# DrorT/demucs

Measured on AMD Instinct MI355X. Metric: real-time factor (audio-sec/wall-sec) htdemucs 4-stem 44.1kHz stereo, 1/8 GPU, higher is better.
Workload: dtype f32

## Files before the change

### demucs_amd/_lib.py

```python
from __future__ import annotations

import ctypes as C
import os
import threading

_HERE = os.path.dirname(os.path.abspath(__file__))
LIB_PATH = os.environ.get("DEMUCS_AMD_LIB") or os.path.join(_HERE, "libdemucs_amd.so")

MI_OK = 0


class MiTensorDesc(C.Structure):
    _fields_ = [("name", C.c_char_p), ("data", C.c_void_p), ("numel", C.c_int64)]


class MiConfig(C.Structure):
    _fields_ = [("n_sources", C.c_int32), ("segment_length", C.c_int32), ("max_batch", C.c_int32),
                ("dtype", C.c_int32)]


class MiProfileRow(C.Structure):
    _fields_ = [("name", C.c_char * 48), ("launches", C.c_int64), ("ms", C.c_double), ("flops", C.c_double),
                ("bytes", C.c_double)]

# ... 16 lines not shown
        ("xh", C.c_void_p), ("xh_n", C.c_int64), ("yh", C.c_void_p), ("yh_n", C.c_int64),
        ("wtap", C.c_void_p), ("ntaps", C.c_int32), ("tap_k2", C.c_int32), ("tap_pad1", C.c_int32), ("tap_pad2", C.c_int32),
        ("tap_dil1", C.c_int32), ("tap_dil2", C.c_int32), ("yh_pq", C.c_int64),
        ("dma_rows", C.c_int32), ("dma_rows_pad", C.c_int32),
    ]


SIGNATURES = {
    "mi_model_create": (C.c_int, [C.POINTER(MiConfig), C.POINTER(MiTensorDesc), C.c_size_t, C.POINTER(C.c_void_p)]),
    "mi_model_destroy": (None, [C.c_void_p]),
    "mi_model_forward": (C.c_int, [C.c_void_p, C.c_void_p, C.c_void_p, C.c_int32, C.c_void_p]),
    "mi_model_forward_core": (C.c_int, [C.c_void_p, C.c_void_p, C.c_void_p, C.c_void_p, C.c_void_p, C.c_int32, C.c_void_p]),
    "mi_model_tap": (C.c_int, [C.c_void_p, C.c_char_p, C.c_void_p, C.c_int32, C.POINTER(C.c_int64), C.c_void_p]),
    "mi_hmodel_create": (C.c_int, [C.POINTER(MiConfig), C.POINTER(MiTensorDesc), C.c_size_t, C.POINTER(C.c_void_p)]),
    "mi_hmodel_destroy": (None, [C.c_void_p]),
    "mi_hmodel_forward": (C.c_int, [C.c_void_p, C.c_void_p, C.c_void_p, C.c_int32, C.c_int32, C.c_void_p]),
    "mi_hmodel_tap": (C.c_int, [C.c_void_p, C.c_char_p, C.c_void_p, C.c_int32, C.POINTER(C.c_int64), C.c_void_p]),
    "mi_hmodel_device_bytes": (C.c_int64, [C.c_void_p]),
    "mi_hmodel_status": (C.c_int, [C.c_void_p, C.c_void_p]),
    "mi_set_two_streams": (C.c_int, [C.c_int32]),
    "mi_set_split_bf16": (C.c_int, [C.c_int32]),
    "mi_set_istft_fused": (C.c_int, [C.c_int32]),
    "mi_set_transpose_tiles": (C.c_int, [C.c_int32]),
    "mi_profile_begin": (C.c_int, [C.c_void_p]),
    "mi_profile_end": (C.c_int, [C.c_void_p, C.POINTER(MiProfileRow), C.c_int32, C.POINTER(C.c_int32), C.c_void_p]),
    "mi_model_device_bytes": (C.c_int64, [C.c_void_p]),
    "mi_segments_gather": (C.c_int, [C.c_void_p, C.c_int64, C.c_int32, C.c_void_p, C.c_int32, C.c_int32, C.c_void_p,
                                     C.c_int64, C.c_void_p]),
    "mi_ola_accumulate": (C.c_int, [C.c_void_p, C.c_int64, C.c_int32, C.c_void_p, C.c_int32, C.c_int64, C.c_void_p, C.c_void_p,
                                    C.c_void_p, C.c_int32, C.c_int64, C.c_int64, C.c_void_p, C.c_int32, C.c_void_p]),
    "mi_ola_finish": (C.c_int, [C.c_void_p, C.c_int64, C.c_int32, C.c_int64, C.c_void_p, C.c_void_p, C.c_int32,
                                C.c_int32, C.c_void_p, C.c_void_p]),
    "mi_segments_gather_packed": (C.c_int, [C.c_void_p, C.c_int64, C.c_int32, C.c_void_p, C.c_int32, C.c_int32, C.c_void_p,
                                            C.c_int64, C.c_void_p]),
    "mi_ola_accumulate_packed": (C.c_int, [C.c_void_p, C.c_int64, C.c_int32, C.c_void_p, C.c_int32, C.c_int64, C.c_void_p, C.c_int32,
                                           C.c_void_p, C.c_int32, C.c_void_p, C.c_int64, C.c_void_p]),
    "mi_ola_finish_packed": (C.c_int, [C.c_void_p, C.c_int64, C.c_int32, C.c_void_p, C.c_int32, C.c_void_p, C.c_int32, C.c_void_p,
                                       C.c_int64, C.c_void_p]),
    "mi_stream_emit": (C.c_int, [C.c_void_p, C.c_int64, C.c_int32, C.c_int32, C.c_void_p, C.c_int32, C.c_void_p, C.c_int32,
                                 C.c_void_p, C.c_int64, C.c_void_p, C.c_int32, C.c_int32, C.c_int32, C.c_void_p, C.c_int64,
                                 C.c_void_p, C.c_int64, C.c_void_p]),
    "mi_streams_emit": (C.c_int, [C.c_void_p, C.c_int64, C.c_int32, C.c_int32, C.c_void_p, C.c_int32, C.c_int64, C.c_void_p,
                                  C.c_int32, C.c_void_p, C.c_int32, C.c_void_p, C.c_int64, C.c_void_p, C.c_int32, C.c_int32,
                                  C.c_int32, C.c_void_p, C.c_int32, C.c_void_p, C.c_int64, C.c_void_p]),
    "mi_streams_append": (C.c_int, [C.c_void_p, C.c_int64, C.c_int32, C.c_void_p, C.c_int32, C.c_int64, C.c_void_p, C.c_int32,
                                    C.c_void_p]),
    "mi_streams_convert_append": (C.c_int, [C.c_void_p, C.c_int64, C.c_int32, C.c_void_p, C.c_int32, C.c_int64, C.c_void_p, C.c_int64,
                                            C.c_void_p, C.c_int64, C.c_void_p, C.c_int32, C.c_int32, C.c_void_p]),
    "mi_streams_compact": (C.c_int, [C.c_void_p, C.c_int64, C.c_void_p, C.c_int64, C.c_void_p, C.c_int32, C.c_int64, C.c_void_p]),
    "mi_mono_stats_scratch_bytes": (C.c_int32, []),
    "mi_mono_stats": (C.c_int, [C.c_void_p, C.c_int32, C.c_int64, C.c_void_p, C.c_void_p, C.c_void_p]),
    "mi_track_affine": (C.c_int, [C.c_void_p, C.c_int64, C.c_void_p, C.c_int32, C.c_void_p]),
    "mi_prevent_clip": (C.c_int, [C.c_void_p, C.c_int64, C.c_int32, C.c_void_p, C.c_void_p, C.c_void_p]),
    "mi_two_stems": (C.c_int, [C.c_void_p, C.c_int32, C.c_int32, C.c_void_p, C.c_int32, C.c_int64, C.c_void_p, C.c_void_p]),
    "mi_stft_cac": (C.c_int, [C.c_void_p, C.c_int32, C.c_int32, C.c_void_p, C.c_void_p]),
    "mi_istft_cac": (C.c_int, [C.c_void_p, C.c_int32, C.c_int32, C.c_int32, C.c_void_p, C.c_void_p]),
    "mi_conv_forward": (C.c_int, [C.POINTER(MiConvDesc), C.c_void_p]),
    "mi_resample_frac": (C.c_int, [C.c_void_p, C.c_int32, C.c_int64, C.c_void_p, C.c_int32, C.c_int32, C.c_int32, C.c_void_p, C.c_int64,
                                   C.c_void_p]),
    "mi_conv_pack_split": (C.c_int, [C.c_void_p, C.c_int32, C.c_int32, C.c_int32, C.c_void_p, C.c_void_p]),
    "mi_conv_pack_half": (C.c_int, [C.c_void_p, C.c_int32, C.c_int32, C.c_int32, C.c_void_p, C.c_void_p]),
    "mi_f32_to_image": (C.c_int, [C.c_void_p, C.c_int32, C.c_int32, C.c_int64, C.c_int32, C.c_void_p, C.c_void_p]),
    "mi_conv_pack_tap": (C.c_int, [C.c_void_p, C.c_int32, C.c_int32, C.c_int32, C.c_int32, C.c_void_p, C.c_void_p]),
    "mi_attention": (C.c_int, [C.c_void_p, C.c_void_p, C.c_void_p, C.c_void_p, C.c_int32, C.c_int32, C.c_int32,
                               C.c_int32, C.c_int64, C.c_int64, C.c_int64, C.c_int32, C.c_void_p]),
    "mi_attention_split": (C.c_int, [C.c_void_p, C.c_void_p, C.c_void_p, C.c_void_p, C.c_int32, C.c_int32, C.c_int32,
                                     C.c_int32, C.c_int64, C.c_int64, C.c_int64, C.c_void_p]),
    "mi_attention_heads": (C.c_int, [C.c_void_p, C.c_void_p, C.c_void_p, C.c_void_p, C.c_int32, C.c_int32, C.c_int32, C.c_int32,
                                     C.c_int32, C.c_int32, C.c_int32, C.c_void_p]),
    "mi_attention_image": (C.c_int, [C.c_void_p, C.c_void_p, C.c_void_p, C.c_void_p, C.c_int64, C.c_int32, C.c_int32, C.c_int32,
                                     C.c_int32, C.c_int64, C.c_int64, C.c_int32, C.c_void_p]),
    "mi_lstm_seq": (C.c_int, [C.c_void_p, C.c_void_p, C.c_int32, C.c_int32, C.c_int32, C.c_void_p, C.c_int32, C.c_void_p]),
    "mi_gn_gelu": (C.c_int, [C.c_void_p, C.c_int32, C.c_int32, C.c_int32, C.c_int32, C.c_int32, C.c_int32, C.c_void_p, C.c_void_p,
                             C.c_void_p, C.c_void_p]),
    "mi_gram_order": (C.c_int32, [C.c_int32]),
    "mi_gn_gelu_gram": (C.c_int, [C.c_void_p, C.c_int32, C.c_int32, C.c_int32, C.c_int32, C.c_int32, C.c_int32, C.c_int32, C.c_void_p,
                                  C.c_void_p, C.c_void_p, C.c_void_p, C.c_int32, C.c_void_p]),
    "mi_dconv_gn_gelu_gram": (C.c_int, [C.c_void_p, C.c_int32, C.c_int32, C.c_int32, C.c_int32, C.c_int32, C.c_int32, C.c_int32,
                                        C.c_void_p, C.c_void_p, C.c_void_p, C.c_void_p, C.c_int32, C.c_void_p]),
    "mi_gram_finalize": (C.c_int, [C.c_void_p, C.c_int32, C.c_int32, C.c_int32, C.c_void_p, C.c_void_p, C.c_double, C.c_double,
                                   C.c_double, C.c_double, C.c_float, C.c_void_p, C.c_void_p]),
    "mi_layernorm_cf": (C.c_int, [C.c_void_p, C.c_int32, C.c_int32, C.c_int32, C.c_void_p, C.c_void_p, C.c_void_p,
                                  C.c_void_p, C.c_void_p]),
    "mi_debug_set_post_launch_hook": (None, [C.c_void_p]),
    "mi_debug_last_conv_route": (C.c_int, []),
    "mi_last_error": (C.c_char_p, []),
    "mi_version": (C.c_char_p, []),
}

_lib = None
_lock = threading.Lock()


class EngineError(RuntimeError):
    """A libdemucs_amd call returned a non-zero status (the reference convention for this path
    is "exceptions propagate", demucs/apply.py:289-293)."""


def load() -> C.CDLL:
    global _lib
    with _lock:
        if _lib is None:
            if not os.path.exists(LIB_PATH):
                raise EngineError(
                    f"{LIB_PATH} not found: build it with `python -c 'import __graft_entry__ as g; g.build()'` "
                    "(hipcc --offload-arch=gfx950).  demucs_amd has no CPU / eager fallback.")
            lib = C.CDLL(LIB_PATH)
            for name, (res, args) in SIGNATURES.items():
                fn = getattr(lib, name)
                fn.restype = res
                fn.argtypes = args
            _lib = lib
    return _lib


def check(status: int, what: str) -> None:
    if status != MI_OK:
        msg = load().mi_last_error().decode(errors="replace")
        raise EngineError(f"{what} failed ({status}): {msg}")


def current_stream_ptr() -> int:
    import torch
    return torch.cuda.current_stream().cuda_stream
```

### demucs_amd/csrc/api.hip

```cpp
#include <new>

#include "common.h"
#include "gemm_conv.h"
#include "kernels.h"
#include "hmodel.h"
#include "model.h"

namespace mi {

post_launch_hook_t g_post_launch_hook = nullptr;
int g_last_conv_route = -1;

char *last_error_buf() {
    static thread_local char buf[1024] = "";
    return buf;
}

int set_error(int code, const char *fmt, ...) {
    va_list ap;
    va_start(ap, fmt);
    vsnprintf(last_error_buf(), 1024, fmt, ap);
    va_end(ap);
    return code;
}
// ... 414 lines not shown
                       void *stream) {
    MI_REQUIRE(q_dev && k_dev && v_dev && img_dev && B > 0 && heads > 0 && Tq > 0 && Tk > 0, "mi_attention_image: bad argument");
    MI_REQUIRE(dtype == MI_DTYPE_BF16 || dtype == MI_DTYPE_F16, "mi_attention_image: dtype %d is not a half mode", dtype);
    return launch_attention(q_dev, k_dev, v_dev, nullptr, B, heads, Tq, Tk, q_batch_stride, kv_batch_stride, 0, dtype,
                            (hipStream_t)stream, img_dev, n_img);
}

int mi_gn_gelu(float *x_dev, int32_t B, int32_t C, int32_t C_alloc, int32_t D1, int32_t D2, int32_t row_mode, const float *stats_dev,
               const float *w_dev, const float *b_dev, void *stream) {
    MI_REQUIRE(x_dev && stats_dev && w_dev && b_dev && B > 0 && C > 0 && D1 > 0 && D2 > 0, "mi_gn_gelu: bad argument");
    MI_REQUIRE(C_alloc >= C, "mi_gn_gelu: C_alloc < C");
    return launch_gn_gelu(x_dev, B, C, C_alloc, D1, D2, row_mode, (const float2 *)stats_dev, w_dev, b_dev, (hipStream_t)stream);
}

int32_t mi_gram_order(int32_t h) { return gram_hp(h); }

int mi_lstm_seq(const float *gx_dev, const float *whh_host, int32_t N, int32_t H, int32_t W, float *out_dev, int32_t mode, void *stream) {
    MI_REQUIRE(gx_dev && whh_host && out_dev && N > 0 && W > 0 && (H == 192 || H == 384), "mi_lstm_seq: bad argument (H must be 192 or 384)");
    MI_REQUIRE(mode == 0 || mode == 1, "mi_lstm_seq: mode 0 (one launch per step) or 1 (persistent kernel)");
    hipStream_t st = (hipStream_t)stream;
    std::vector<float> packed((size_t)2 * 4 * H * H);
    pack_lstm_whh(whh_host, H, packed.data());
    float *wd = nullptr, *state = nullptr;
    void *scratch = nullptr;
    unsigned *flag = nullptr;
    int r = MI_OK;
    auto fail = [&](hipError_t e, const char *what) { if (e != hipSuccess && r == MI_OK) r = set_error(MI_EHIP, "mi_lstm_seq: %s: %s", what, hipGetErrorString(e)); };
    fail(hipMalloc((void **)&wd, packed.size() * sizeof(float)), "hipMalloc");
    fail(hipMalloc((void **)&state, (size_t)6 * N * H * sizeof(float)), "hipMalloc");
    fail(hipMalloc(&scratch, lstm_persist_scratch_bytes()), "hipMalloc");
    fail(hipHostMalloc((void **)&flag, 64, hipHostMallocMapped), "hipHostMalloc");
    if (r == MI_OK) {
        *flag = 0;
        fail(hipMemcpyAsync(wd, packed.data(), packed.size() * sizeof(float), hipMemcpyHostToDevice, st), "hipMemcpyAsync");
        if (r == MI_OK) r = mode ? launch_lstm_persist(gx_dev, wd, N, H, W, out_dev, scratch, flag, st) : launch_lstm_seq(gx_dev, wd, N, H, W, out_dev, state, st);
        fail(hipStreamSynchronize(st), "hipStreamSynchronize");
        if (r == MI_OK && *(volatile unsigned *)flag) r = set_error(MI_EHIP, "mi_lstm_seq: the persistent kernel timed out waiting for its hidden-state exchange");
        if (r == MI_OK && mode && getenv("MI_LSTM_DEBUG")) {
                        unsigned dbg[16] = {};
            (void)hipMemcpy(dbg, (char *)scratch + lstm_persist_ctl_offset(), sizeof(dbg), hipMemcpyDeviceToHost);
            fprintf(stderr, "[lstm] H %d N %d W %d: block 0 / wave 1 spent %.1f us gathering h in %u poll passes (%.2f us, %.2f passes per step); "
                    "%s stores\n", H, N, W, dbg[2] * 0.01, dbg[3], dbg[2] * 0.01 / std::max(1, W - 1), (double)dbg[3] / std::max(1, W - 1),
                    dbg[4] ? "same-XCD plain" : "write-through");
            fprintf(stderr, "[lstm]   shader cycles per step: gather %.0f, issue + products %.0f, LDS write + barrier %.0f, gate stage %.0f; whole step %.0f\n",
                    (double)dbg[8] / W, (double)dbg[9] / W, (double)dbg[10] / W, (double)dbg[11] / W, (double)dbg[12] / W);
        }
    }
    if (wd) (void)hipFree(wd);
    if (state) (void)hipFree(state);
    if (scratch) (void)hipFree(scratch);
    if (flag) (void)hipHostFree(flag);
    return r;
}

int mi_gn_gelu_gram(float *x_dev, int32_t B, int32_t h, int32_t C_alloc, int32_t D1, int32_t D2, int32_t pitch, int32_t row_mode,
                    const float *stats_dev, const float *w_dev, const float *b_dev, double *gram_dev, int32_t slots, void *stream) {
    MI_REQUIRE(x_dev && stats_dev && w_dev && b_dev && gram_dev && B > 0 && h > 0 && D1 > 0 && D2 > 0 && slots > 0, "mi_gn_gelu_gram: bad argument");
    MI_REQUIRE(C_alloc >= h && pitch >= D2, "mi_gn_gelu_gram: C_alloc < h or pitch < D2");
    return launch_gn_gelu_gram(x_dev, B, h, C_alloc, D1, D2, pitch, row_mode, (const float2 *)stats_dev, w_dev, b_dev, gram_dev, slots,
                               false, (hipStream_t)stream);
}

int mi_dconv_gn_gelu_gram(float *x_dev, int32_t B, int32_t h, int32_t C_alloc, int32_t D1, int32_t D2, int32_t pitch, int32_t row_mode,
                          const float *stats_dev, const float *w_dev, const float *b_dev, double *gram_dev, int32_t slots, void *stream) {
    MI_REQUIRE(x_dev && stats_dev && w_dev && b_dev && gram_dev && B > 0 && h > 0 && D1 > 0 && D2 > 0 && slots > 0, "mi_dconv_gn_gelu_gram: bad argument");
    MI_REQUIRE(C_alloc >= h && C_alloc <= gram_hp(h) && pitch >= D2, "mi_dconv_gn_gelu_gram: C_alloc outside [h, mi_gram_order(h)] or pitch < D2");
    return launch_gn_gelu_gram(x_dev, B, h, C_alloc, D1, D2, pitch, row_mode, (const float2 *)stats_dev, w_dev, b_dev, gram_dev, slots,
                               true, (hipStream_t)stream);
}

int mi_gram_finalize(double *gram_dev, int32_t rows, int32_t h, int32_t slots, const double *wt_dev, const double *ct_dev, double sum_b,
                     double sum_bsq, double cols, double count, float eps, float *stats_out_dev, void *stream) {
    MI_REQUIRE(gram_dev && wt_dev && ct_dev && stats_out_dev && rows > 0 && h > 0 && slots > 0 && count > 0.0, "mi_gram_finalize: bad argument");
    return launch_gram_finalize(gram_dev, rows, h, slots, wt_dev, ct_dev, sum_b, sum_bsq, cols, count, eps, (float2 *)stats_out_dev,
                                (hipStream_t)stream);
}

int mi_layernorm_cf(const float *x_dev, int32_t B, int32_t C, int32_t T, const float *w_dev, const float *b_dev,
                    const float *add_dev, float *y_dev, void *stream) {
    MI_REQUIRE(x_dev && w_dev && b_dev && y_dev, "mi_layernorm_cf: null argument");
    return launch_layernorm_cf(x_dev, B, C, T, w_dev, b_dev, add_dev, y_dev, nullptr, (hipStream_t)stream);
}

}
```

### demucs_amd/csrc/attention_x6.hip

```cpp
#include "common.h"
#include "kernels.h"
#include "split_bf16.h"

namespace mi {

namespace {

typedef float f32x16 __attribute__((ext_vector_type(16)));
typedef unsigned u32x4 __attribute__((ext_vector_type(4)));
constexpr int HD = 64;
constexpr int KT = 64;

__device__ __forceinline__ f32x16 mfma6(const u32x4 (&a)[3], const u32x4 (&b)[3], f32x16 acc) {
    constexpr int PA[6] = {2, 0, 1, 1, 0, 0}, PB[6] = {0, 2, 1, 0, 1, 0};
#pragma unroll
    for (int q = 0; q < 6; ++q)
        acc = __builtin_amdgcn_mfma_f32_32x32x16_bf16(__builtin_bit_cast(bf16x8, a[PA[q]]), __builtin_bit_cast(bf16x8, b[PB[q]]), acc, 0,
                                                      0, 0);
    return acc;
}

__device__ __forceinline__ void split8(const float (&x)[8], u32x4 (&out)[3]) {
    unsigned h[4], m[4], l[4];
#pragma unroll
    for (int j = 0; j < 4; ++j) split3(x[2 * j], x[2 * j + 1], h[j], m[j], l[j]);
    out[0] = u32x4{h[0], h[1], h[2], h[3]};
    out[1] = u32x4{m[0], m[1], m[2], m[3]};
    out[2] = u32x4{l[0], l[1], l[2], l[3]};
}

}

__global__ __launch_bounds__(256, 2) void attention_x6_kernel(const float *__restrict__ q, const float *__restrict__ k,
                                                              const float *__restrict__ v, float *__restrict__ o, int Tq, int Tk,
                                                              int64_t q_bs, int64_t kv_bs, int64_t o_bs, int planes, int heads) {
    __shared__ u32x4 Kx[3 * 8 * KT];
    __shared__ u32x4 Vx[3 * 8 * HD];
    {
        float agpr_anchor = 0.f;
        asm volatile("; accumulators in AGPRs %0" : "+a"(agpr_anchor));
    }
    const int tid = threadIdx.x, lane = tid & 63;
    const int wave = __builtin_amdgcn_readfirstlane(tid >> 6);
    const int li = lane & 31, lh = lane >> 5;
    const int nqb = (Tq + 127) / 128;
    const int xj = blockIdx.x >> 3;
    const int pl = (xj / nqb) * 8 + (blockIdx.x & 7);
    if (pl >= planes) return;
    const int head = pl % heads, b = pl / heads;
    const int q0 = (xj % nqb) * 128 + wave * 32;
    const float *qp = q + (size_t)b * q_bs + (size_t)head * HD * Tq;
    const float *kp = k + (size_t)b * kv_bs + (size_t)head * HD * Tk;
    const float *vp = v + (size_t)b * kv_bs + (size_t)head * HD * Tk;

    const int qi = q0 + li;
    const bool qok = qi < Tq;
    const int qic = qok ? qi : Tq - 1;
    u32x4 qx[4][3];
#pragma unroll
    for (int t = 0; t < 4; ++t) {
        float x[8];
#pragma unroll
        for (int j = 0; j < 8; ++j) {
            const float qv = qp[(size_t)(16 * t + 8 * lh + j) * Tq + qic];
            x[j] = qok ? qv * 0.125f : 0.f;
        }
        split8(x, qx[t]);
    }

    f32x16 oacc[2];
#pragma unroll
    for (int r = 0; r < 16; ++r) { oacc[0][r] = 0.f; oacc[1][r] = 0.f; }
    float mrun = -INFINITY, lrun = 0.f;

    const int ve = lane >> 3, vd = (lane & 7) + 8 * wave, vc = 16 * (ve >> 1) + 4 * (ve & 1);
    float kst[2][8];
    float4 vst[2][2];
    auto stage_load = [&](int k0) {
        const bool kok = k0 + lane < Tk;
        const int kc = kok ? k0 + lane : Tk - 1;
#pragma unroll
        for (int i = 0; i < 2; ++i)
#pragma unroll
            for (int j = 0; j < 8; ++j) kst[i][j] = kp[(size_t)(8 * (wave + 4 * i) + j) * Tk + kc];
#pragma unroll
        for (int i = 0; i < 2; ++i)
#pragma unroll
            for (int c = 0; c < 2; ++c) {
                const int key = k0 + vc + 8 * c;
                vst[i][c] = *reinterpret_cast<const float4 *>(vp + (size_t)(vd + 32 * i) * Tk + (key < Tk ? key : Tk - 4));
            }
    };
    auto stage_mask = [&](int k0) {
        if (k0 + KT <= Tk) return;
        if (k0 + lane >= Tk) {
#pragma unroll
            for (int i = 0; i < 2; ++i)
#pragma unroll
                for (int j = 0; j < 8; ++j) kst[i][j] = 0.f;
        }
#pragma unroll
        for (int c = 0; c < 2; ++c)
            if (k0 + vc + 8 * c >= Tk)
#pragma unroll
                for (int i = 0; i < 2; ++i) vst[i][c] = make_float4(0.f, 0.f, 0.f, 0.f);
    };
    auto stage_store = [&]() {
#pragma unroll
        for (int i = 0; i < 2; ++i) {
            u32x4 t[3];
            split8(kst[i], t);
#pragma unroll
            for (int p = 0; p < 3; ++p) Kx[(p * 8 + wave + 4 * i) * KT + lane] = t[p];
        }
#pragma unroll
        for (int i = 0; i < 2; ++i) {
            const float x[8] = {vst[i][0].x, vst[i][0].y, vst[i][0].z, vst[i][0].w, vst[i][1].x, vst[i][1].y, vst[i][1].z, vst[i][1].w};
            u32x4 t[3];
            split8(x, t);
#pragma unroll
            for (int p = 0; p < 3; ++p) Vx[(p * 8 + ve) * HD + vd + 32 * i] = t[p];
        }
    };

    stage_load(0);
    for (int k0 = 0; k0 < Tk; k0 += KT) {
        __syncthreads();
        stage_mask(k0);
        stage_store();
        __syncthreads();
        if (k0 + KT < Tk) stage_load(k0 + KT);
#pragma unroll
        for (int sub = 0; sub < 2; ++sub) {
            const int kb = sub * 32;
            if (k0 + kb >= Tk) break;
            f32x16 sacc;
#pragma unroll
            for (int r = 0; r < 16; ++r) sacc[r] = 0.f;
#pragma unroll
            for (int t = 0; t < 4; ++t) {
                u32x4 kf[3];
#pragma unroll
                for (int p = 0; p < 3; ++p) kf[p] = Kx[(p * 8 + 2 * t + lh) * KT + kb + li];
                sacc = mfma6(kf, qx[t], sacc);
            }
            float s[16];
#pragma unroll
            for (int r = 0; r < 16; ++r) s[r] = sacc[r];
            float mloc = -INFINITY;
            if (k0 + kb + 32 > Tk) {
#pragma unroll
                for (int r = 0; r < 16; ++r)
                    if (k0 + kb + (r & 3) + 8 * (r >> 2) + 4 * lh >= Tk) s[r] = -INFINITY;
            }
#pragma unroll
            for (int r = 0; r < 16; ++r) mloc = fmaxf(mloc, s[r]);
            mloc = fmaxf(mloc, __shfl_xor(mloc, 32));
            const float mnew = fmaxf(mrun, mloc);
            float psum = 0.f;
#pragma unroll
            for (int r = 0; r < 16; ++r) {
                const float p = __expf(s[r] - mnew);
                s[r] = p;
                psum += p;
            }
            if (__any(mnew != mrun)) {
                const float alpha = __expf(mrun - mnew);
                lrun *= alpha;
#pragma unroll
                for (int r = 0; r < 16; ++r) { oacc[0][r] *= alpha; oacc[1][r] *= alpha; }
                mrun = mnew;
            }
            lrun += psum;
#pragma unroll
            for (int m = 0; m < 2; ++m) {
                float x[8];
#pragma unroll
                for (int j = 0; j < 8; ++j) x[j] = s[8 * m + j];
                u32x4 px[3];
                split8(x, px);
#pragma unroll
                for (int dt = 0; dt < 2; ++dt) {
                    u32x4 vf[3];
#pragma unroll
                    for (int p = 0; p < 3; ++p) vf[p] = Vx[(p * 8 + 2 * (2 * sub + m) + lh) * HD + dt * 32 + li];
                    oacc[dt] = mfma6(vf, px, oacc[dt]);
                }
            }
        }
    }
    const float ltot = lrun + __shfl_xor(lrun, 32);
    const float inv = 1.0f / ltot;
    if (qok) {
        float *op = o + (size_t)b * o_bs + (size_t)head * HD * Tq + qi;
#pragma unroll
        for (int dt = 0; dt < 2; ++dt)
#pragma unroll
            for (int r = 0; r < 16; ++r) {
                const int dd = dt * 32 + (r & 3) + 8 * (r >> 2) + 4 * lh;
                op[(size_t)dd * Tq] = oacc[dt][r] * inv;
            }
    }
}

int launch_attention_x6(const float *q, const float *k, const float *v, float *o, int B, int heads, int Tq, int Tk, int64_t q_bs,
                        int64_t kv_bs, int64_t o_bs, hipStream_t st) {
    MI_REQUIRE(Tk % 4 == 0, "attention x6: Tk %% 4 != 0 (%d)", Tk);
    MI_REQUIRE(((uintptr_t)k & 15) == 0 && ((uintptr_t)v & 15) == 0 && kv_bs % 4 == 0, "attention x6: k/v must be 16-byte aligned");
    const int planes = B * heads;
    hipLaunchKernelGGL(attention_x6_kernel, dim3((unsigned)(ceil_div(Tq, 128) * ((planes + 7) / 8) * 8)), dim3(256), 0, st, q, k, v, o,
                       Tq, Tk, q_bs, kv_bs, o_bs, planes, heads);
    MI_CHECK_LAUNCH();
    return MI_OK;
}

}
```

### demucs_amd/csrc/gemm_conv.hip

```cpp
#include <vector>

#include "gemm_tile.h"

namespace mi {

template <int WM, int WN, int TM, int TN, int EPI, int LFLAGS, bool PLAIN>
__global__ __launch_bounds__(256, (TM * TN == 4 ? 3 : 4)) void conv_gemm_kernel(const mi_conv_desc d, const int N, const int MT, const int Gm) {
    constexpr int BM = WM * TM * 32;
    static_assert(WN * TN * 32 == BN, "block N tile is 128");
    static_assert(WM * WN == 4, "4 waves");
    __shared__ float As[2][BK][BM];
    __shared__ float Bs[2][BK][BN];

    const int tid = threadIdx.x;
    const int lane = tid & 63;
    const int wave = __builtin_amdgcn_readfirstlane(tid >> 6);
    const int wm = wave / WN, wn = wave % WN;
    int mt, nt;
    if (!tile_of_block(MT, Gm, N, mt, nt)) return;
    const int m0 = mt * BM, n0 = nt * BN;
    const int P = d.O1 * d.O2;

    constexpr int A_F4 = BK * BM / 4, A_FULL = A_F4 / 256, A_REM = A_F4 % 256;
    constexpr int A_SLOTS = A_FULL + (A_REM ? 1 : 0);
// ... 562 lines not shown
            atomicMax(&rec->maxdiff_bits, __float_as_uint(dlt == dlt ? dlt : 3.0e38f));
            const int bb = (int)(i / ybs), m = (int)((i % ybs) / ycs), p = (int)(i % ycs);
            atomicMin(&rec->bmin, bb); atomicMax(&rec->bmax, bb);
            atomicMin(&rec->mmin, m); atomicMax(&rec->mmax, m);
            atomicMin(&rec->pmin, p); atomicMax(&rec->pmax, p);
        }
    }
}

static void x6_verify_dump() {
    if (!g_vlog || g_vinfo.empty()) return;
    (void)hipDeviceSynchronize();
    std::vector<X6VerifyRec> h(g_vinfo.size());
    if (hipMemcpy(h.data(), g_vlog, h.size() * sizeof(X6VerifyRec), hipMemcpyDeviceToHost) != hipSuccess) return;
    size_t nbad = 0;
    for (size_t i = 0; i < h.size(); ++i) {
        if (!h[i].bad) continue;
        const X6VerifyInfo &f = g_vinfo[i];
        if (++nbad <= 40)
            fprintf(stderr, "[x6 verify] launch %zu: M %d K %d N %d epi %d flags %d tile %d plain %d B %d O1 %d O2 %d o2v %d | %u bad, max %.3e, "
                    "b %d-%d  m %d-%d  p %d-%d (col tiles %d-%d)\n", i, f.M, f.K, f.N, f.epi, f.flags, f.tile, f.plain, f.B, f.O1, f.O2, f.o2v,
                    h[i].bad, __builtin_bit_cast(float, h[i].maxdiff_bits), h[i].bmin, h[i].bmax, h[i].mmin, h[i].mmax, h[i].pmin, h[i].pmax,
                    h[i].pmin / BN, h[i].pmax / BN);
    }
    fprintf(stderr, "[x6 verify] %zu launches checked, %zu with mismatches\n", h.size(), nbad);
}

static int launch_conv_fp32_only(const mi_conv_desc &d, hipStream_t st);

static int x6_verified_launch(const mi_conv_desc &d, int tile, bool plain, hipStream_t st, int loader = 0) {
    auto launch_x6 = [&]() {
        return loader == 1 ? launch_conv_tap_x6(d, tile, st) : loader == 2 ? launch_conv_rows_x6(d, tile, st) : launch_conv_x6(d, tile, plain, st);
    };
    const bool checkable = d.epi != MI_EPI_STATS_ONLY && d.epi != MI_EPI_BIAS_STATS && d.res != d.y && (int)g_vinfo.size() < kVerifyMax;
    if (!checkable) return launch_x6();
    if (!g_vlog) {
        MI_HIP(hipMalloc((void **)&g_vlog, kVerifyMax * sizeof(X6VerifyRec)));
        std::vector<X6VerifyRec> init(kVerifyMax, X6VerifyRec{0, 0, 1 << 30, -1, 1 << 30, -1, 1 << 30, -1});
        MI_HIP(hipMemcpy(g_vlog, init.data(), init.size() * sizeof(X6VerifyRec), hipMemcpyHostToDevice));
        atexit(x6_verify_dump);
    }
    const size_t elems = (size_t)d.B * (size_t)d.y_bstride;
    if (elems > g_vscratch_elems) {
        MI_HIP(hipStreamSynchronize(st));
        if (g_vscratch) (void)hipFree(g_vscratch);
        MI_HIP(hipMalloc((void **)&g_vscratch, elems * sizeof(float)));
        g_vscratch_elems = elems;
    }
    MI_HIP(hipMemcpyAsync(g_vscratch, d.y, elems * sizeof(float), hipMemcpyDeviceToDevice, st));
    MI_TRY(launch_x6());
    mi_conv_desc e = d;
    e.wx = nullptr; e.y = g_vscratch;
    MI_TRY(launch_conv_fp32_only(e, st));
    const int id = (int)g_vinfo.size();
    g_vinfo.push_back(X6VerifyInfo{d.M, d.K, d.B * d.O1 * d.O2, d.epi, d.flags, tile, plain ? 1 : 0, d.B, d.O1, d.O2, d.o2_valid, d.y_bstride, d.y_cstride});
    hipLaunchKernelGGL(x6_verify_kernel, dim3(1024), dim3(256), 0, st, d.y, g_vscratch, (long long)elems, (long long)d.y_bstride, (long long)d.y_cstride, g_vlog + id);
    MI_CHECK_LAUNCH();
    return MI_OK;
}

int g_split_bf16 = 1;

int launch_conv(const mi_conv_desc &din, hipStream_t st) {
    mi_conv_desc d = din;
    if (!d.sink) d.sink = conv_sink();
    MI_REQUIRE(d.sink, "conv: could not allocate the store sink");
    MI_REQUIRE((int64_t)d.Mpad * d.y_cstride < (1ll << 31), "conv: output channel stride too large for 32-bit row offsets");
    MI_REQUIRE(d.Kpad % BK == 0 && d.Kpad >= BK, "conv: Kpad %d must be a positive multiple of %d", d.Kpad, BK);
    MI_REQUIRE(d.Mpad % 4 == 0, "conv: Mpad %d must be a multiple of 4", d.Mpad);
    MI_REQUIRE(d.O2 >= 32 || d.row_mode == 0 || (d.epi != MI_EPI_BIAS_STATS && d.epi != MI_EPI_STATS_ONLY),
               "conv: statistics epilogue needs O2 >= 32");
    const int tile = d.tile_m ? d.tile_m : conv_pick_tile(d.M);
    MI_REQUIRE(d.pro == 0, "conv: the fused GroupNorm+GELU prologue was replaced by launch_gn_gelu");
    MI_REQUIRE(!(d.flags & MI_FLAG_IMG4) || (d.epi == MI_EPI_GLU && d.half && d.yh && d.yh_pq > 0 && d.yh_n >= (int64_t)d.B * d.yh_pq && d.M % 32 == 0 &&
                                             ((uintptr_t)d.yh & 15) == 0),
               "conv: MI_FLAG_IMG4 needs a half-mode GLU layer with M %% 32 == 0 and an aligned phase image of >= B * yh_pq positions per plane");
    MI_REQUIRE(!(d.flags & MI_FLAG_STATS) || (d.epi == MI_EPI_LINEAR && d.stats && d.O2 >= 32 && d.row_mode == 0),
               "conv: MI_FLAG_STATS needs a LINEAR layer, a statistics buffer and O2 >= 32");
    if (!g_split_bf16) d.wx = nullptr;
    MI_REQUIRE(!(d.flags & MI_FLAG_LN) || (d.pro_stats && d.scale && d.epi == MI_EPI_LINEAR), "conv: MI_FLAG_LN needs pro_stats and scale");
    const int64_t P = (int64_t)d.O1 * d.O2;
    const bool plain = d.plain && d.K == d.Kpad && P % 4 == 0 && d.x_bstride % 4 == 0 && ((uintptr_t)d.x & 15) == 0 &&
                       d.S1 == 1 && d.S2 == 1 && d.D1 == d.O1 && (d.x_ld ? d.x_ld : d.D2) == d.O2;
    MI_REQUIRE(!(d.flags & MI_FLAG_IMG) || d.epi == MI_EPI_CONVTR ||
               (d.half && d.yh && d.epi == MI_EPI_LINEAR && d.M % 8 == 0 && d.yh_n >= (int64_t)d.B * P && ((uintptr_t)d.yh & 15) == 0) ||
               (d.half && d.yh && d.epi == MI_EPI_GLU && d.M % 32 == 0 && !(d.flags & (MI_FLAG_IMG4 | MI_FLAG_EMB)) && d.yh_n >= (int64_t)d.B * P &&
                ((uintptr_t)d.yh & 15) == 0),
               "conv: MI_FLAG_IMG needs a half-precision LINEAR layer with M %% 8 == 0 (or GLU layer with M %% 32 == 0) and an aligned "
               "output image of >= B * P columns");
    MI_REQUIRE(d.epi != MI_EPI_CONVTR || ((int64_t)d.Mpad * d.y_cstride < (1ll << 30) && (d.tr_stride == 0 || d.tr_stride == 2 || d.tr_stride == 4) &&
                                          d.M % (d.tr_stride == 2 ? 2 : 4) == 0),
               "conv: transposed conv needs stride 2 or 4, M a multiple of it and 30-bit output offsets per item");
    {
        const int f = d.flags & (MI_FLAG_GELU | MI_FLAG_RES | MI_FLAG_IMG);
        MI_REQUIRE(d.epi != MI_EPI_CONVTR || f == 0 || (d.tr_stride != 2 && (f == (MI_FLAG_GELU | MI_FLAG_RES) || f == (MI_FLAG_GELU | MI_FLAG_RES | MI_FLAG_IMG))),
                   "conv: transposed conv epilogue supports no flags, GELU|RES or GELU|RES|IMG (stride 2: no flags), got %d", d.flags);
    }
    MI_REQUIRE(!(d.flags & MI_FLAG_IMG) || d.epi != MI_EPI_CONVTR ||
               (d.half && d.yh && d.yh_n >= (int64_t)d.B * d.y_cstride && ((uintptr_t)d.yh & 15) == 0),
               "conv: MI_FLAG_IMG on a transposed conv needs a half mode and an output image of >= B * y_cstride positions");
    if (d.wtap) { MI_REQUIRE(d.half && d.xh, "conv: tap-ordered weights need a half mode and an operand-image input"); g_last_conv_route = 6; return launch_conv_tap(d, tile, st); }
    MI_REQUIRE(!(d.flags & MI_FLAG_HEADS) || (d.half && d.yh && d.epi == MI_EPI_LINEAR && d.M % 512 == 0 && d.O1 == 1 && d.yh_n >= d.O2 &&
                                              ((uintptr_t)d.yh & 15) == 0 && !(d.flags & MI_FLAG_IMG)),
               "conv: MI_FLAG_HEADS needs a half-precision LINEAR layer on tokens (O1 = 1) with M %% 512 == 0 and an aligned output");
    MI_REQUIRE(!d.xh || d.half, "conv: an operand-image input needs a half-precision layer");
    if (d.half) { g_last_conv_route = 5; return launch_conv_half(d, tile, plain, st); }
    static const int x6_mode = getenv("MI_X6_MODE") ? atoi(getenv("MI_X6_MODE")) : 0;
    static const int x6_class = getenv("MI_X6_CLASS") ? atoi(getenv("MI_X6_CLASS")) : -1;
    const bool x6_class_ok = x6_class < 0 || x6_class == d.epi * 8 + (tile == 32 ? 0 : tile == 64 ? 1 : tile == 96 ? 2 : 3) * 2 + (plain ? 1 : 0);
    static const bool x6_verify = getenv("MI_X6_VERIFY") != nullptr;
    if (!plain && x6_mode == 0 && x6_class_ok && dmatap_eligible(d, tile, true))
        return x6_verify ? x6_verified_launch(d, tile, false, st, 1) : launch_conv_tap_x6(d, tile, st);
    if (x6_mode == 0 && x6_class_ok && dmarow_eligible(d, tile, plain, true))
        return x6_verify ? x6_verified_launch(d, tile, false, st, 2) : launch_conv_rows_x6(d, tile, st);
    static const int small_tile = getenv("MI_SMALL_TILE") ? atoi(getenv("MI_SMALL_TILE")) : 1;
    int ktile = tile;
    if (small_tile && !plain && d.epi == MI_EPI_GLU && tile == 128 && d.Mpad % 96 == 0 &&
        (int64_t)(d.Mpad / 128) * ceil_div((int64_t)d.B * d.O1 * d.O2, BN) < 200)
        ktile = 96;
    if (!plain && dmatap_eligible(d, ktile))
        return d.epi == MI_EPI_GLU ? launch_dmatap<MI_EPI_GLU>(d, ktile, st) : launch_dmatap<MI_EPI_BIAS_STATS>(d, ktile, st);
    if (dmarow_eligible(d, tile, plain)) {
        switch (d.epi) {
            case MI_EPI_LINEAR: return launch_dmarow<MI_EPI_LINEAR, MI_FLAG_GELU>(d, tile, st);
            case MI_EPI_CONVTR: return launch_dmarow<MI_EPI_CONVTR, 0>(d, tile, st);
            case MI_EPI_GLU: return launch_dmarow<MI_EPI_GLU, 0>(d, tile, st);
            case MI_EPI_GN_GLU: return launch_dmarow<MI_EPI_GN_GLU, 0>(d, tile, st);
        }
    }
    if (!x6_class_ok) d.wx = nullptr;
    if (d.wx && conv_x6_supported(tile) && x6_mode == 3) return launch_conv_x6(d, tile, false, st);
    if (d.wx && conv_x6_supported(tile) && (x6_mode == 0 || (x6_mode == 1) == plain))
        return x6_verify ? x6_verified_launch(d, tile, plain, st) : launch_conv_x6(d, tile, plain, st);
#define MI_DISPATCH(E)                                              \
    case E: return plain ? launch_tile<E, 0, true>(d, tile, st) : launch_tile<E, 0, false>(d, tile, st)
#define MI_LINEAR(F)                                                \
    case F: return plain ? launch_tile<MI_EPI_LINEAR, F, true>(d, tile, st) : launch_tile<MI_EPI_LINEAR, F, false>(d, tile, st)
    if (d.epi == MI_EPI_LINEAR) {
        switch (d.flags & (MI_FLAG_GELU | MI_FLAG_SCALE | MI_FLAG_RES | MI_FLAG_LN | MI_FLAG_STATS)) {
            MI_LINEAR(0);
            MI_LINEAR(MI_FLAG_GELU);
            MI_LINEAR(MI_FLAG_RES);
            MI_LINEAR(MI_FLAG_SCALE | MI_FLAG_RES);
            MI_LINEAR(MI_FLAG_SCALE | MI_FLAG_RES | MI_FLAG_STATS);
            MI_LINEAR(MI_FLAG_LN);
            MI_LINEAR(MI_FLAG_LN | MI_FLAG_GELU);
        }
        return set_error(MI_EINVAL, "conv: unsupported LINEAR flag combination %d", d.flags);
    }
#undef MI_LINEAR
    switch (d.epi) {
        MI_DISPATCH(MI_EPI_GLU);
        MI_DISPATCH(MI_EPI_BIAS_STATS);
        MI_DISPATCH(MI_EPI_STATS_ONLY);
        MI_DISPATCH(MI_EPI_GN_GLU);
        MI_DISPATCH(MI_EPI_CONVTR);
    }
#undef MI_DISPATCH
    return set_error(MI_EINVAL, "conv: unsupported epilogue %d", d.epi);
}

static int launch_conv_fp32_only(const mi_conv_desc &d, hipStream_t st) {
    mi_conv_desc e = d;
    e.wx = nullptr;
    return launch_conv(e, st);
}

}
```

### demucs_amd/csrc/gemm_tile.h

```cpp
#pragma once
#include "common.h"
#include "gemm_conv.h"
#include "kernels.h"

namespace mi {

typedef float f32x16 __attribute__((ext_vector_type(16)));

constexpr int BK = 16;
constexpr int BN = 128;

struct ColInfo {
    int b, o1, o2, p;
    bool valid;
};

__device__ __forceinline__ ColInfo decompose(int n, int N, int P, int O2, int o2v) {
    ColInfo c;
    c.valid = n < N;
    const int nn = c.valid ? n : 0;
    c.b = nn / P;
    c.p = nn - c.b * P;
    c.o1 = c.p / O2;
    c.o2 = c.p - c.o1 * O2;
    c.valid = c.valid && c.o2 < o2v;
    return c;
}

__device__ __forceinline__ void load_rows16(const float *p, int mbase, float (&out)[16]) {
#pragma unroll
    for (int g = 0; g < 4; ++g) {
        const float4 v = *reinterpret_cast<const float4 *>(p + mbase + 8 * g);
        out[4 * g] = v.x; out[4 * g + 1] = v.y; out[4 * g + 2] = v.z; out[4 * g + 3] = v.w;
    }
}

__device__ __forceinline__ float gather_b(const mi_conv_desc &d, const mi_ktab_entry e, const float *xcol, int i1b, int i2b,
                                          bool colvalid, bool &ok) {
    const int i1 = i1b + e.d1, i2 = i2b + e.d2;
    ok = colvalid && (unsigned)i1 < (unsigned)d.D1 && (unsigned)i2 < (unsigned)d.D2;
    const float *p = ok ? xcol + e.off : d.x;
    return *p;
}

struct TrCol {
    int po[4];
    size_t colbase;
    size_t imgbase;
};
constexpr int kTrBad = -(1 << 30);

template <int LG>
__device__ __forceinline__ TrCol convtr_column(const mi_conv_desc &d, const ColInfo &c) {
    const bool trf = d.flags & MI_FLAG_TR_FREQ;
    const int tpad = d.tr_stride ? d.tr_pad : 2, ostep = trf ? d.O2 : 1;
    const int oq = ((trf ? c.o1 : c.o2) << LG) - tpad;
    TrCol t;
#pragma unroll
    for (int ph = 0; ph < (1 << LG); ++ph) {
        const int o = oq + ph;
        t.po[ph] = (c.valid && (unsigned)o < (unsigned)d.out_len) ? o * ostep : kTrBad;
    }
    const int o2 = trf ? c.o2 : 0;
    t.colbase = c.valid ? (size_t)c.b * d.y_bstride + o2 : 0;
    t.imgbase = ((size_t)c.b * d.y_cstride + o2) * 8;
    return t;
}

template <int LG, int F>
__device__ __forceinline__ void convtr_tile(const mi_conv_desc &d, const f32x16 &acc, const float (&biasr)[16], const TrCol &t, int mbase,
                                            float *sink) {
    const int cs = (int)d.y_cstride;
    constexpr bool gelu = F & MI_FLAG_GELU, resf = F & MI_FLAG_RES, imgf = F & MI_FLAG_IMG;
    const int co0 = mbase >> LG, cout = d.M >> LG;
    float *const ycol = d.y + t.colbase;
    const float *const rcol = d.res + t.colbase;
    unsigned short *const yimg = reinterpret_cast<unsigned short *>(d.yh) + t.imgbase;
#pragma unroll
    for (int h = 0; h < 2; ++h) {
        int off[8];
        float resv[8];
#pragma unroll
        for (int q = 0; q < 8; ++q) {
            const int r = 8 * h + q, j = (r & 3) + 8 * (r >> 2), co = co0 + (j >> LG);
            const int rowoff = co < cout ? co * cs : kTrBad;
            off[q] = rowoff + t.po[j & ((1 << LG) - 1)];
        }
        if (resf) {
#pragma unroll
            for (int q = 0; q < 8; ++q) resv[q] = rcol[max(off[q], 0)];
        }
#pragma unroll
        for (int q = 0; q < 8; ++q) {
            const int r = 8 * h + q;
            float v = acc[r] + biasr[r];
            if (gelu) v = gelu_exact(v);
            if (resf) v += resv[q];
            if (imgf) {
                const int j = (r & 3) + 8 * (r >> 2), co = co0 + (j >> LG);
                const size_t chan = (size_t)(co >> 3) * d.yh_n * 8 + (co & 7);
                const int pos8 = (off[q] - co * cs) * 8;
                if (off[q] >= 0) yimg[chan + pos8] = (unsigned short)(pack_half2(d.half, v, 0.f) & 0xffffu);
            } else {
                *(off[q] >= 0 ? ycol + off[q] : sink) = v;
            }
        }
        __builtin_amdgcn_sched_barrier(0);
    }
}

template <int TM, int TN, int EPI, int LFLAGS>
__device__ __forceinline__ void conv_epilogue(const mi_conv_desc &d, f32x16 (&acc)[TM][TN], int m0, int n0, int wm, int wn, int N,
                                              int P, int o2v) {
    const int tid = threadIdx.x, lane = tid & 63, li = lane & 31, lh = lane >> 5;
    const int slot = blockIdx.x % kStatSlots;
    float *const sink = d.sink + tid;
#pragma unroll
    for (int b = 0; b < TN; ++b) {
        const int n = n0 + (wn * TN + b) * 32 + li;
        const ColInfo c = decompose(n, N, P, d.O2, o2v);
        const int row = d.row_mode ? c.b * d.O1 + c.o1 : c.b;
        float s1 = 0.f, s2 = 0.f;
        float2 lnstat = make_float2(0.f, 1.f);
        if (EPI == MI_EPI_LINEAR && (LFLAGS & MI_FLAG_LN))
            lnstat = reinterpret_cast<const float2 *>(d.pro_stats)[c.valid ? n : 0];
        float gmean = 0.f, grstd = 0.f;
        if (EPI == MI_EPI_GN_GLU) {
            const float2 st = reinterpret_cast<const float2 *>(d.gn_stats)[row];
            gmean = st.x; grstd = st.y;
        }
        const int tr_lg = d.tr_stride == 2 ? 1 : 2;
        TrCol trc;
        if (EPI == MI_EPI_CONVTR) trc = tr_lg == 2 ? convtr_column<2>(d, c) : convtr_column<1>(d, c);
#pragma unroll
        for (int a = 0; a < TM; ++a) {
            __builtin_amdgcn_sched_barrier(0);
            int mbase = m0 + (wm * TM + a) * 32 + 4 * lh;
            asm volatile("" : "+v"(mbase));
            const f32x16 &tacc = acc[a][b];
            float biasr[16], auxr[16], aux2r[16];
            load_rows16(d.bias, mbase, biasr);
            if (EPI == MI_EPI_LINEAR && (LFLAGS & (MI_FLAG_SCALE | MI_FLAG_LN))) load_rows16(d.scale, mbase, auxr);
            if (EPI == MI_EPI_GN_GLU) { load_rows16(d.gn_w, mbase, auxr); load_rows16(d.gn_b, mbase, aux2r); }
            if (EPI == MI_EPI_LINEAR) {
                const size_t colbase = c.valid ? (size_t)c.b * d.y_bstride + c.p : 0;
                float *const ycol = d.y + colbase;
                const int cs = (int)d.y_cstride;
                float resv[16], vq[4];
                if (LFLAGS & MI_FLAG_RES) {
                    const float *const rcol = d.res + colbase;
#pragma unroll
                    for (int r = 0; r < 16; ++r) {
                        const int m = mbase + (r & 3) + 8 * (r >> 2);
                        resv[r] = rcol[(c.valid && m < d.M) ? m * cs : 0];
                    }
                }
#pragma unroll
                for (int r = 0; r < 16; ++r) {
                    const int m = mbase + (r & 3) + 8 * (r >> 2);
                    float v;
                    if (LFLAGS & MI_FLAG_LN) v = lnstat.y * (tacc[r] - lnstat.x * auxr[r]) + biasr[r];
                    else v = tacc[r] + biasr[r];
                    if (LFLAGS & MI_FLAG_GELU) v = gelu_exact(v);
                    if (LFLAGS & MI_FLAG_SCALE) v *= auxr[r];
                    if (LFLAGS & MI_FLAG_RES) v += resv[r];
                    if (LFLAGS & MI_FLAG_STATS) { const bool ok = c.valid && m < d.M; s1 += ok ? v : 0.f; s2 += ok ? v * v : 0.f; }
                    if (LFLAGS & MI_FLAG_HEADS) {
                        vq[r & 3] = v;
                        if ((r & 3) == 3) {
                            const int mo = mbase + 8 * (r >> 2);
                            const size_t plane = ((size_t)(mo >> 9) * d.B + c.b) * 8 + ((mo >> 6) & 7);
                            uint2 *dst = reinterpret_cast<uint2 *>(d.yh) + ((plane * d.yh_n + c.p) * 64 + (mo & 63)) / 4;
                            if (c.valid && mo < d.M) *dst = make_uint2(pack_half2(d.half, vq[0], vq[1]), pack_half2(d.half, vq[2], vq[3]));
                        }
                        continue;
                    }
                    if (LFLAGS & MI_FLAG_IMG) {
                        vq[r & 3] = v;
                        if ((r & 3) == 3) {
                            const int mo = mbase + 8 * (r >> 2);
                            uint2 *dst = reinterpret_cast<uint2 *>(d.yh) + ((size_t)(mo >> 3) * d.yh_n + n) * 2 + lh;
                            if (c.valid && mo < d.M) *dst = make_uint2(pack_half2(d.half, vq[0], vq[1]), pack_half2(d.half, vq[2], vq[3]));
                        }
                        continue;
                    }
                    *((c.valid && m < d.M) ? ycol + m * cs : sink) = v;
                }
            } else if (EPI == MI_EPI_GLU || EPI == MI_EPI_GN_GLU) {
                const size_t colbase = c.valid ? (size_t)c.b * d.y_bstride + c.p : 0;
                float *const ycol = d.y + colbase;
                const int cs = (int)d.y_cstride;
                const bool emb = EPI == MI_EPI_GLU && (d.flags & MI_FLAG_EMB);
                const bool imgp = EPI == MI_EPI_GLU && (d.flags & MI_FLAG_IMG);
                const bool img4 = (EPI == MI_EPI_GLU && (d.flags & MI_FLAG_IMG4)) || imgp;
                unsigned *img4p = nullptr;
                size_t oct_step = 0;
                if (imgp) {
                    img4p = reinterpret_cast<unsigned *>(d.yh) + (size_t)(c.valid ? n : 0) * 4;
                    oct_step = (size_t)4 * d.yh_n;
                } else if (img4) {
                    const bool trf = d.flags & MI_FLAG_TR_FREQ;
                    const int idx = trf ? c.o1 : c.o2, rho = idx & 3, q = (idx >> 2) + (rho >> 1);
                    const size_t pos = (size_t)c.b * d.yh_pq + (trf ? (size_t)q * d.O2 + c.o2 : (size_t)q);
                    img4p = reinterpret_cast<unsigned *>(d.yh) + ((size_t)rho * d.yh_n + pos) * 4;
                    oct_step = (size_t)16 * d.yh_n;
                }
                float resv[8], scv[8], vprev = 0.f;
                unsigned pk4[4] = {0u, 0u, 0u, 0u};
#pragma unroll
                for (int r = 0; r < 16; r += 2) {
                    const int m = mbase + (r & 3) + 8 * (r >> 2), ch = m >> 1;
                    const bool ok = c.valid && m < d.M;
                    if (EPI == MI_EPI_GN_GLU) { resv[r >> 1] = d.res[colbase + (ok ? ch * cs : 0)]; scv[r >> 1] = d.scale[ok ? ch : 0]; }
                    else if (emb) resv[r >> 1] = d.emb[ok ? ch * d.O1 + c.o1 : 0];
                }
#pragma unroll
                for (int r = 0; r < 16; r += 2) {
                    const int m = mbase + (r & 3) + 8 * (r >> 2);
                    float va = tacc[r] + biasr[r], vg = tacc[r + 1] + biasr[r + 1];
                    if (EPI == MI_EPI_GN_GLU) {
                        va = (va - gmean) * grstd * auxr[r] + aux2r[r];
                        vg = (vg - gmean) * grstd * auxr[r + 1] + aux2r[r + 1];
                    }
                    float v = va * sigmoid_f(vg);
                    if (EPI == MI_EPI_GN_GLU) v = resv[r >> 1] + scv[r >> 1] * v;
                    else if (emb) v += resv[r >> 1];
                    *((c.valid && m < d.M && !imgp) ? ycol + (m >> 1) * cs : sink) = v;
                    if (img4) {
                        if (r & 2) pk4[r >> 2] = pack_half2(d.half, vprev, v);
                        else vprev = v;
                    }
                }
                if (img4) {
                    typedef unsigned u2 __attribute__((ext_vector_type(2)));
                    const u2 s02 = __builtin_amdgcn_permlane32_swap(pk4[0], pk4[2], false, false);
                    const u2 s13 = __builtin_amdgcn_permlane32_swap(pk4[1], pk4[3], false, false);
                    const int oct = ((mbase - 4 * lh) >> 4) + lh;
                    if (c.valid && mbase - 4 * lh + 31 < d.M)
                        *reinterpret_cast<uint4 *>(img4p + (size_t)oct * oct_step) = make_uint4(s02[0], s02[1], s13[0], s13[1]);
                }
            } else if (EPI == MI_EPI_BIAS_STATS || EPI == MI_EPI_STATS_ONLY) {
#pragma unroll
                for (int r = 0; r < 16; ++r) {
                    const int m = mbase + (r & 3) + 8 * (r >> 2);
                    const float v = tacc[r] + biasr[r];
                    const bool ok = c.valid && m < d.M;
                    if (EPI == MI_EPI_BIAS_STATS)
                        *(ok ? d.y + ((size_t)c.b * d.y_bstride + (size_t)m * d.y_cstride + c.p) : sink) = v;
                    s1 += ok ? v : 0.f; s2 += ok ? v * v : 0.f;
                }
            } else if (EPI == MI_EPI_CONVTR) {
                if (tr_lg == 1) convtr_tile<1, 0>(d, tacc, biasr, trc, mbase, sink);
                else if (!(d.flags & MI_FLAG_GELU)) convtr_tile<2, 0>(d, tacc, biasr, trc, mbase, sink);
                else if (!(d.flags & MI_FLAG_IMG)) convtr_tile<2, MI_FLAG_GELU | MI_FLAG_RES>(d, tacc, biasr, trc, mbase, sink);
                else convtr_tile<2, MI_FLAG_GELU | MI_FLAG_RES | MI_FLAG_IMG>(d, tacc, biasr, trc, mbase, sink);
            }
        }
        if (EPI == MI_EPI_BIAS_STATS || EPI == MI_EPI_STATS_ONLY || (EPI == MI_EPI_LINEAR && (LFLAGS & MI_FLAG_STATS))) {
            double t1 = (double)s1, t2 = (double)s2;
// ... 40 lines not shown
```

### demucs_amd/csrc/gemm_x6.hip

```cpp
#include "gemm_tile.h"
#include "split_bf16.h"

namespace mi {

typedef __attribute__((address_space(1))) const void gvoid_t;
typedef __attribute__((address_space(3))) void lvoid_t;

__global__ void pack_split_kernel(const float *__restrict__ wt, int Kpad, int Mpad, int BM, __bf16 *__restrict__ wx) {
    const size_t idx = blockIdx.x * (size_t)blockDim.x + threadIdx.x;
    if (idx >= (size_t)Kpad * Mpad) return;
    const int k = (int)(idx / Mpad), m = (int)(idx % Mpad);
    const int mt = m / BM, mi = m % BM, kt = k / BK, h = (k % BK) / 8, j = k % 8, nk = Kpad / BK;
    const float x = wt[idx];
    const __bf16 a = (__bf16)x;
    const float r = x - (float)a;
    const __bf16 b = (__bf16)r;
    const __bf16 c = (__bf16)(r - (float)b);
    __bf16 *img = wx + ((size_t)mt * nk + kt) * ((size_t)BM * 48);
    img[((0 * 2 + h) * BM + mi) * 8 + j] = a;
    img[((1 * 2 + h) * BM + mi) * 8 + j] = b;
    img[((2 * 2 + h) * BM + mi) * 8 + j] = c;
}

int launch_pack_split(const float *wt, int Kpad, int Mpad, int tile_m, void *wx, hipStream_t st) {
    MI_REQUIRE(Kpad % BK == 0 && Mpad % tile_m == 0, "pack_split: Kpad %d / Mpad %d do not fit tile %d", Kpad, Mpad, tile_m);
    const size_t n = (size_t)Kpad * Mpad;
    hipLaunchKernelGGL(pack_split_kernel, dim3((unsigned)((n + 255) / 256)), dim3(256), 0, st, wt, Kpad, Mpad, tile_m, (__bf16 *)wx);
    MI_CHECK_LAUNCH();
    return MI_OK;
}

#ifndef MI_X6_ABL
#define MI_X6_ABL 0
#endif
constexpr int kRowTaps = -1;
template <int WM, int WN, int TM, int TN, int EPI, int LFLAGS, bool PLAIN, bool HALF_IMG, int NT>
__device__ __forceinline__ void conv_x6_body(const mi_conv_desc &d, const int N, const int MT, const int Gm) {
    constexpr int BM = WM * TM * 32;
    constexpr bool RAW = PLAIN || NT != 0;
    constexpr bool ROWS = NT == kRowTaps;
    static_assert(NT <= 0 || (!PLAIN && EPI == MI_EPI_GLU), "tap loader: GLU rewrite convs");
    static_assert(!ROWS || (!PLAIN && (EPI == MI_EPI_LINEAR || EPI == MI_EPI_CONVTR || EPI == MI_EPI_GLU)),
                  "row-tap loader: encoder / transposed convs, 1 x 1 + GLU rewrites");
    static_assert(NT >= kRowTaps, "NT: taps, 0 or kRowTaps");
    static_assert(WN * TN * 32 == BN, "block N tile is 128");
    static_assert(WM * WN == 4, "4 waves");
    constexpr int A_BYTES = BM * 96, B_BYTES = BN * 96, STAGE = A_BYTES + B_BYTES;
    constexpr int A_CHUNKS = A_BYTES / 1024;
    static_assert(!HALF_IMG || BM == 64, "HALF_IMG: 64-row tile of a 128-row image");
    constexpr int A_KSTEP = HALF_IMG ? 2 * A_BYTES : A_BYTES, A_CHUNK_STRIDE = HALF_IMG ? 2048 : 1024;
    __shared__ __attribute__((aligned(16))) unsigned char smem[2 * STAGE];
    __shared__ __attribute__((aligned(16))) float braw[RAW ? 2 * BK * BN : 4];

    {
        float agpr_anchor = 0.f;
        asm volatile("; accumulators in AGPRs %0" : "+a"(agpr_anchor));
    }
    const int tid = threadIdx.x, lane = tid & 63;
    const int wave = __builtin_amdgcn_readfirstlane(tid >> 6);
    const int wm = wave / WN, wn = wave % WN;
    int mt, nt;
    if (!tile_of_block(MT, Gm, N, mt, nt)) return;
    const int m0 = mt * BM, n0 = nt * BN;
    const int P = d.O1 * d.O2;
    const int o2v = d.o2_valid ? d.o2_valid : d.O2;
    const int nk = d.Kpad / BK;

    const unsigned char *aimg = reinterpret_cast<const unsigned char *>(d.wx) + (size_t)(HALF_IMG ? mt >> 1 : mt) * nk * A_KSTEP +
                                (HALF_IMG ? (mt & 1) * 1024 : 0) + lane * 16;
#define MI_A_DMA(kt, stage)                                                                                         \
    do {                                                                                                            \
        _Pragma("unroll") for (int c = 0; c < (A_CHUNKS + 3) / 4; ++c) {                                             \
            const int chunk = c * 4 + wave;                                                                         \
            if (chunk < A_CHUNKS)                                                                                   \
                __builtin_amdgcn_global_load_lds((gvoid_t *)(aimg + (size_t)(kt) * A_KSTEP + chunk * A_CHUNK_STRIDE), \
                                                 (lvoid_t *)(smem + (stage) * STAGE + chunk * 1024), 16, 0, 0);     \
        }                                                                                                           \
    } while (0)

    const int bn = tid & 127;
    const int bh = __builtin_amdgcn_readfirstlane(tid >> 7);
    const ColInfo lc = decompose(n0 + bn, N, P, d.O2, PLAIN ? d.O2 : o2v);
    const int i1b = lc.o1 * d.S1, i2b = lc.o2 * d.S2;
    const float *xcol = d.x + (size_t)lc.b * d.x_bstride + (PLAIN ? (size_t)lc.p : (size_t)i1b * (d.x_ld ? d.x_ld : d.D2) + i2b);
    const float *bp = lc.valid ? xcol + (size_t)(8 * bh) * P : d.sink + 256;
    const size_t b_row = lc.valid ? (size_t)P : 0, b_step = lc.valid ? (size_t)BK * P : 0;
    float breg[8];
    const int li = lane & 31, lh = lane >> 5;
    const int rc4 = li * 4, rrow = 4 * wave + lh;
    const ColInfo rcol = decompose(n0 + rc4, N, P, d.O2, NT ? o2v : d.O2);
    const int x_ld = d.x_ld ? d.x_ld : d.D2;
    const int ri1 = rcol.o1 * d.S1;
    const float *rsrc = !rcol.valid ? d.sink + 256
                        : d.x + (size_t)rcol.b * d.x_bstride +
                              (ROWS ? (size_t)ri1 * x_ld + rcol.o2 : (size_t)rcol.p + (NT ? 0 : (size_t)rrow * P));
    const size_t r_row2 = rcol.valid ? (size_t)2 * P : 0, r_step = rcol.valid ? (size_t)BK * P : 0;
    const int4 *ktab4 = reinterpret_cast<const int4 *>(d.ktab) + 4 * wave;
    typedef int v2i __attribute__((ext_vector_type(2)));
    v2i e0, e1, e2, e3;
#define MI_ROW_LOADS "s_load_dwordx2 %0, %4, 0x0\n\ts_load_dwordx2 %1, %4, 0x10\n\ts_load_dwordx2 %2, %4, 0x20\n\t" \
                     "s_load_dwordx2 %3, %4, 0x30\n\t"
#define MI_ROW_ENTRIES(kt)                                                                                          \
    asm volatile(MI_ROW_LOADS "s_waitcnt lgkmcnt(0)"                                                               \
                 : "=&s"(e0), "=&s"(e1), "=&s"(e2), "=&s"(e3) : "s"(ktab4 + (kt) * BK) : "memory")
    constexpr int K2 = 3;
    const int fix_l = (NT && rcol.valid && rcol.o2 == 0) ? 0 : -1;
    const int fr = d.D2 - 1 - rcol.o2;
    const int fix_r = (NT && rcol.valid && fr >= 0 && fr < 4) ? fr : -1;
#define MI_BRAW_DMA(kt, rs)                                                                                         \
    do {                                                                                                            \
        float *dst = braw + (rs) * (BK * BN) + (4 * wave) * BN;                                                     \
        if constexpr (ROWS) {                                                                                       \
            _Pragma("unroll") for (int i = 0; i < 2; ++i) {                                                         \
                const int off = i ? (lh ? e3.x : e2.x) : (lh ? e1.x : e0.x);                                        \
                const int dd1 = i ? (lh ? e3.y : e2.y) : (lh ? e1.y : e0.y);                                        \
                const bool ok = rcol.valid && (unsigned)(ri1 + dd1) < (unsigned)d.D1;                               \
                __builtin_amdgcn_global_load_lds((gvoid_t *)(ok ? rsrc + off : d.sink + 256), (lvoid_t *)(dst + 2 * i * BN), 16, 0, 0); \
            }                                                                                                       \
        } else if constexpr (NT > 0) {                                                                              \
            _Pragma("unroll") for (int i = 0; i < 2; ++i) {                                                         \
                const int k = (kt) * BK + rrow + 2 * i, ci = k / NT, tap = k - ci * NT, t1 = tap / K2, t2 = tap - t1 * K2; \
                const int i1 = rcol.o1 + t1 - d.tap_pad1;                                                           \
                const bool ok = rcol.valid && k < d.K && (unsigned)i1 < (unsigned)d.D1;                             \
                const float *g = rsrc + (int64_t)ci * P + (int64_t)(t1 - d.tap_pad1) * x_ld + (t2 - d.tap_pad2);    \
                __builtin_amdgcn_global_load_lds((gvoid_t *)(ok ? g : d.sink + 256), (lvoid_t *)(dst + 2 * i * BN), 16, 0, 0); \
            }                                                                                                       \
        } else {                                                                                                    \
            const float *g = rsrc + (size_t)(kt) * r_step;                                                          \
            __builtin_amdgcn_global_load_lds((gvoid_t *)g, (lvoid_t *)dst, 16, 0, 0);                               \
            __builtin_amdgcn_global_load_lds((gvoid_t *)(g + r_row2), (lvoid_t *)(dst + 2 * BN), 16, 0, 0);         \
        }                                                                                                           \
    } while (0)
#define MI_BRAW_FIX(kt, rs)                                                                                         \
    do {                                                                                                            \
        if constexpr (NT > 0) {                                                                                     \
            float *row = braw + (rs) * (BK * BN) + rrow * BN + rc4;                                                 \
            _Pragma("unroll") for (int i = 0; i < 2; ++i) {                                                         \
                const int k = (kt) * BK + rrow + 2 * i, dd2 = (k % NT) % K2 - d.tap_pad2;                           \
                if (dd2 < 0 && fix_l >= 0) row[2 * i * BN + fix_l] = 0.f;                                           \
                if (dd2 > 0 && fix_r >= 0) row[2 * i * BN + fix_r] = 0.f;                                           \
            }                                                                                                       \
        }                                                                                                           \
    } while (0)
#define MI_BRAW_READ(rs)                                                                                            \
    do {                                                                                                            \
        _Pragma("unroll") for (int j = 0; j < 8; ++j) breg[j] = braw[(rs) * (BK * BN) + (8 * bh + j) * BN + bn];     \
    } while (0)

#define MI_B_LOAD(kt)                                                                                               \
    do {                                                                                                            \
        if (PLAIN) {                                                                                                \
            _Pragma("unroll") for (int j = 0; j < 8; ++j) breg[j] = bp[(size_t)(kt) * b_step + j * b_row];           \
        } else {                                                                                                    \
            mi_ktab_entry ke[8];                                                                                    \
            _Pragma("unroll") for (int j = 0; j < 8; ++j) ke[j] = d.ktab[(kt) * BK + 8 * bh + j];                    \
            _Pragma("unroll") for (int j = 0; j < 8; ++j) {                                                          \
                bool ok;                                                                                            \
                const float v = gather_b(d, ke[j], xcol, i1b, i2b, lc.valid, ok);                                   \
                breg[j] = ok ? v : 0.f;                                                                             \
            }                                                                                                       \
        }                                                                                                           \
    } while (0)

#define MI_B_STORE(stage)                                                                                           \
    do {                                                                                                            \
        unsigned ph[4], pm[4], pl[4];                                                                               \
        _Pragma("unroll") for (int j = 0; j < 4; ++j) split3(breg[2 * j], breg[2 * j + 1], ph[j], pm[j], pl[j]);    \
        unsigned char *bs = smem + (stage) * STAGE + A_BYTES + (bh * BN + bn) * 16;                                 \
        *reinterpret_cast<uint4 *>(bs) = make_uint4(ph[0], ph[1], ph[2], ph[3]);                                    \
        *reinterpret_cast<uint4 *>(bs + 2 * BN * 16) = make_uint4(pm[0], pm[1], pm[2], pm[3]);                      \
        *reinterpret_cast<uint4 *>(bs + 4 * BN * 16) = make_uint4(pl[0], pl[1], pl[2], pl[3]);                      \
    } while (0)

    f32x16 acc[TM][TN];
#pragma unroll
    for (int a = 0; a < TM; ++a)
#pragma unroll
        for (int b = 0; b < TN; ++b)
#pragma unroll
            for (int r = 0; r < 16; ++r) acc[a][b][r] = 0.f;

    constexpr int PA[6] = {2, 0, 1, 1, 0, 0}, PB[6] = {0, 2, 1, 0, 1, 0};
    MI_A_DMA(0, 0);
    if constexpr (RAW) {
        if constexpr (ROWS) MI_ROW_ENTRIES(0);
        MI_BRAW_DMA(0, 0);
        if (nk > 1) {
            if constexpr (ROWS) MI_ROW_ENTRIES(1);
            MI_BRAW_DMA(1, 1);
        }
        if constexpr (ROWS) { if (nk > 2) MI_ROW_ENTRIES(2); }
        asm volatile("s_waitcnt vmcnt(0)" ::: "memory");
        MI_BRAW_FIX(0, 0);
        if (nk > 1) MI_BRAW_FIX(1, 1);
        __syncthreads();
        MI_BRAW_READ(0);
    } else {
        MI_B_LOAD(0);
    }
    MI_B_STORE(0);
    asm volatile("s_waitcnt vmcnt(0)" ::: "memory");
    __syncthreads();
    int cur = 0;
    bf16x8 keepa[TM][3], keepb[TN][3];
    for (int kt = 0; kt < nk; ++kt) {
        const unsigned char *As = smem + cur * STAGE, *Bs = As + A_BYTES;
        bf16x8 af[TM][3], bf[TN][3];
        if ((MI_X6_ABL & 128) && kt > 0) {
#pragma unroll
            for (int p = 0; p < 3; ++p) {
#pragma unroll
                for (int a = 0; a < TM; ++a) af[a][p] = keepa[a][p];
#pragma unroll
                for (int b = 0; b < TN; ++b) bf[b][p] = keepb[b][p];
            }
        } else
#pragma unroll
        for (int p = 0; p < 3; ++p) {
#pragma unroll
            for (int a = 0; a < TM; ++a)
                af[a][p] = *reinterpret_cast<const bf16x8 *>(As + (((p * 2 + lh) * BM) + (wm * TM + a) * 32 + li) * 16);
#pragma unroll
            for (int b = 0; b < TN; ++b)
                bf[b][p] = *reinterpret_cast<const bf16x8 *>(Bs + (((p * 2 + lh) * BN) + (wn * TN + b) * 32 + li) * 16);
        }
        if (MI_X6_ABL & 128) {
#pragma unroll
            for (int p = 0; p < 3; ++p) {
#pragma unroll
                for (int a = 0; a < TM; ++a) keepa[a][p] = af[a][p];
#pragma unroll
                for (int b = 0; b < TN; ++b) keepb[b][p] = bf[b][p];
            }
        }
        if (MI_X6_ABL & 64) {
            typedef unsigned u32x4 __attribute__((ext_vector_type(4)));
#pragma unroll
            for (int p = 0; p < 3; ++p) {
#pragma unroll
                for (int a = 0; a < TM; ++a) { u32x4 z = __builtin_bit_cast(u32x4, af[a][p]); asm volatile("" : "+v"(z)); af[a][p] = __builtin_bit_cast(bf16x8, z); }
#pragma unroll
                for (int b = 0; b < TN; ++b) { u32x4 z = __builtin_bit_cast(u32x4, bf[b][p]); asm volatile("" : "+v"(z)); bf[b][p] = __builtin_bit_cast(bf16x8, z); }
            }
        }
        if (MI_X6_ABL & 8) {
            typedef unsigned u32x4 __attribute__((ext_vector_type(4)));
#pragma unroll
            for (int p = 0; p < 3; ++p) {
#pragma unroll
                for (int a = 0; a < TM; ++a) { u32x4 z = {0u, 0u, 0u, 0u}; asm volatile("" : "+v"(z)); af[a][p] = __builtin_bit_cast(bf16x8, z); }
#pragma unroll
                for (int b = 0; b < TN; ++b) { u32x4 z = {0u, 0u, 0u, 0u}; asm volatile("" : "+v"(z)); bf[b][p] = __builtin_bit_cast(bf16x8, z); }
            }
        }
        __builtin_amdgcn_sched_barrier(0);
        if (kt + 1 < nk) {
            MI_A_DMA(kt + 1, cur ^ 1);
            if constexpr (RAW) {
                if (kt + 2 < nk) MI_BRAW_DMA(kt + 2, kt & 1);
            } else {
                MI_B_LOAD(kt + 1);
            }
        }
        if constexpr (RAW) {
            MI_BRAW_READ((kt + 1) & 1);
        }
        __builtin_amdgcn_sched_barrier(0);
#pragma unroll
        for (int q = 0; q < 6; ++q)
#pragma unroll
            for (int a = 0; a < TM; ++a)
#pragma unroll
                for (int b = 0; b < TN; ++b)
                    if (!(MI_X6_ABL & 1) || (q == 0 && a == 0 && b == 0)) {
                        acc[a][b] = __builtin_amdgcn_mfma_f32_32x32x16_bf16(af[a][PA[q]], bf[b][PB[q]], acc[a][b], 0, 0, 0);
                        if (MI_X6_ABL & 16) asm volatile("s_nop 15\n\ts_nop 15");
                        if ((MI_X6_ABL & 32) && a == TM - 1 && b == TN - 1) asm volatile("s_nop 15\n\ts_nop 15\n\ts_nop 15\n\ts_nop 15");
                    }
        if (RAW || kt + 1 < nk) MI_B_STORE(cur ^ 1);
        if constexpr (RAW) {
#pragma unroll
            for (int i = 0; i < 6 * TM * TN; ++i) {
                __builtin_amdgcn_sched_group_barrier(0x008, 1, 0);
                __builtin_amdgcn_sched_group_barrier(0x002, (72 + 6 * TM * TN - 1) / (6 * TM * TN), 0);
            }
        }
        if (ROWS && kt + 3 < nk)
            asm volatile(MI_ROW_LOADS "s_waitcnt vmcnt(0) lgkmcnt(0)"
                         : "=&s"(e0), "=&s"(e1), "=&s"(e2), "=&s"(e3) : "s"(ktab4 + (kt + 3) * BK) : "memory");
        else
            asm volatile("s_waitcnt vmcnt(0)" ::: "memory");
        if (kt + 2 < nk) MI_BRAW_FIX(kt + 2, kt & 1);
        __syncthreads();
        cur ^= 1;
    }
#undef MI_A_DMA
#undef MI_B_LOAD
#undef MI_BRAW_DMA
#undef MI_BRAW_FIX
#undef MI_BRAW_READ
#undef MI_ROW_ENTRIES
#undef MI_ROW_LOADS
#undef MI_B_STORE

    if (MI_X6_ABL & 4) {
        float s = 0.f;
        for (int a = 0; a < TM; ++a) for (int b = 0; b < TN; ++b) for (int r = 0; r < 16; ++r) s += acc[a][b][r];
        d.sink[threadIdx.x] = s;
        return;
    }
    conv_epilogue<TM, TN, EPI, LFLAGS>(d, acc, m0, n0, wm, wn, N, P, o2v);
}

template <int WM, int WN, int TM, int TN, int EPI, int LFLAGS, bool PLAIN, bool HALF_IMG = false>
__global__ __launch_bounds__(256, 2) void conv_gemm_x6_kernel(const mi_conv_desc d, const int N, const int MT, const int Gm) {
    conv_x6_body<WM, WN, TM, TN, EPI, LFLAGS, PLAIN, HALF_IMG, 0>(d, N, MT, Gm);
}

template <int WM, int WN, int TM, int TN, bool HALF_IMG, int NT>
__global__ __launch_bounds__(256, 2) void conv_tap_x6_kernel(const mi_conv_desc d, const int N, const int MT, const int Gm) {
    conv_x6_body<WM, WN, TM, TN, MI_EPI_GLU, 0, false, HALF_IMG, NT>(d, N, MT, Gm);
}

template <int WM, int WN, int TM, int TN, int EPI, int LFLAGS, bool HALF_IMG>
__global__ __launch_bounds__(256, 2) void conv_rows_x6_kernel(const mi_conv_desc d, const int N, const int MT, const int Gm) {
    conv_x6_body<WM, WN, TM, TN, EPI, LFLAGS, false, HALF_IMG, kRowTaps>(d, N, MT, Gm);
}

template <int WM, int WN, int TM, int TN, int EPI, int LFLAGS, bool PLAIN, bool HALF_IMG = false, int NTAPS = 0>
static int launch_cfg_x6(const mi_conv_desc &d, hipStream_t st) {
    constexpr int BM = WM * TM * 32;
    const int64_t N64 = (int64_t)d.B * d.O1 * d.O2;
    MI_REQUIRE(N64 < (1ll << 31) - 256, "conv: too many output positions (%lld)", (long long)N64);
    MI_REQUIRE(d.Mpad % (HALF_IMG ? 2 * BM : BM) == 0, "conv: Mpad %d not a multiple of the %d-row tile", d.Mpad, BM);
    const int N = (int)N64, MT = d.Mpad / BM, NT = ceil_div(N, BN);
    const int Gm = pick_m_groups(MT, (size_t)d.Kpad * d.Mpad * 6);
    const unsigned grid = grouped_grid(MT, NT, Gm);
    if constexpr (NTAPS > 0) hipLaunchKernelGGL((conv_tap_x6_kernel<WM, WN, TM, TN, HALF_IMG, NTAPS>), dim3(grid), dim3(256), 0, st, d, N, MT, Gm);
    else if constexpr (NTAPS == kRowTaps)
        hipLaunchKernelGGL((conv_rows_x6_kernel<WM, WN, TM, TN, EPI, LFLAGS, HALF_IMG>), dim3(grid), dim3(256), 0, st, d, N, MT, Gm);
    else hipLaunchKernelGGL((conv_gemm_x6_kernel<WM, WN, TM, TN, EPI, LFLAGS, PLAIN, HALF_IMG>), dim3(grid), dim3(256), 0, st, d, N, MT, Gm);
    MI_CHECK_LAUNCH();
    return MI_OK;
}

template <int EPI, int LFLAGS, bool PLAIN>
static int launch_tile_x6(const mi_conv_desc &d, int tile, hipStream_t st) {
    if constexpr (PLAIN && EPI == MI_EPI_LINEAR) {
        static const int small = getenv("MI_SMALL_TILE") ? atoi(getenv("MI_SMALL_TILE")) : 1;
        if (small && tile == 128 && (int64_t)(d.Mpad / 128) * ceil_div((int64_t)d.B * d.O1 * d.O2, BN) < 200)
            return launch_cfg_x6<1, 4, 2, 1, EPI, LFLAGS, PLAIN, true>(d, st);
    }
    switch (tile) {
        case 128: return launch_cfg_x6<2, 2, 2, 2, EPI, LFLAGS, PLAIN>(d, st);
        case 96: return launch_cfg_x6<1, 4, 3, 1, EPI, LFLAGS, PLAIN>(d, st);
        case 64: return launch_cfg_x6<1, 4, 2, 1, EPI, LFLAGS, PLAIN>(d, st);
    }
    return set_error(MI_EINVAL, "conv x6: unsupported tile_m %d", tile);
}

bool conv_x6_supported(int tile) { return tile == 128 || tile == 96 || tile == 64; }

template <int NT>
static int launch_tile_tap_x6(const mi_conv_desc &d, int tile, hipStream_t st) {
    static const int small = getenv("MI_SMALL_TILE") ? atoi(getenv("MI_SMALL_TILE")) : 1;
    if (small && tile == 128 && (int64_t)(d.Mpad / 128) * ceil_div((int64_t)d.B * d.O1 * d.O2, BN) < 200)
        return launch_cfg_x6<1, 4, 2, 1, MI_EPI_GLU, 0, false, true, NT>(d, st);
    if (tile == 128) return launch_cfg_x6<2, 2, 2, 2, MI_EPI_GLU, 0, false, false, NT>(d, st);
    return launch_cfg_x6<1, 4, 3, 1, MI_EPI_GLU, 0, false, false, NT>(d, st);
}

int launch_conv_tap_x6(const mi_conv_desc &d, int tile, hipStream_t st) {
    g_last_conv_route = 7;
    MI_REQUIRE(d.wx && ((uintptr_t)d.wx & 15) == 0, "conv tap x6: split weight image missing or misaligned");
    MI_REQUIRE(d.epi == MI_EPI_GLU && (tile == 96 || tile == 128) && (d.ntaps == 9 || d.ntaps == 3),
               "conv tap x6: GLU layer with 9 or 3 taps on a 96- or 128-row tile (epi %d, tile %d, ntaps %d)", d.epi, tile, d.ntaps);
    return d.ntaps == 9 ? launch_tile_tap_x6<9>(d, tile, st) : launch_tile_tap_x6<3>(d, tile, st);
}

template <int EPI, int LFLAGS>
static int launch_tile_rows_x6(const mi_conv_desc &d, int tile, hipStream_t st) {
    static const int small = getenv("MI_SMALL_TILE") ? atoi(getenv("MI_SMALL_TILE")) : 1;
    if (small && tile == 128 && (int64_t)(d.Mpad / 128) * ceil_div((int64_t)d.B * d.O1 * d.O2, BN) < 200)
        return launch_cfg_x6<1, 4, 2, 1, EPI, LFLAGS, false, true, kRowTaps>(d, st);
    if (tile == 128) return launch_cfg_x6<2, 2, 2, 2, EPI, LFLAGS, false, false, kRowTaps>(d, st);
    return launch_cfg_x6<1, 4, 3, 1, EPI, LFLAGS, false, false, kRowTaps>(d, st);
}

int launch_conv_rows_x6(const mi_conv_desc &d, int tile, hipStream_t st) {
    g_last_conv_route = 8;
    MI_REQUIRE(d.wx && ((uintptr_t)d.wx & 15) == 0, "conv rows x6: split weight image missing or misaligned");
    MI_REQUIRE(d.ktab && ((uintptr_t)d.ktab & 63) == 0, "conv rows x6: gather table missing or misaligned");
    MI_REQUIRE(tile == 96 || tile == 128, "conv rows x6: 96- or 128-row tile (tile %d)", tile);
    if (d.epi == MI_EPI_CONVTR) return launch_tile_rows_x6<MI_EPI_CONVTR, 0>(d, tile, st);
    if (d.epi == MI_EPI_GLU) {
        MI_REQUIRE(tile == 128, "conv rows x6: GLU on a 128-row tile (tile %d)", tile);
        return launch_tile_rows_x6<MI_EPI_GLU, 0>(d, tile, st);
    }
    MI_REQUIRE(d.epi == MI_EPI_LINEAR && (d.flags & (MI_FLAG_GELU | MI_FLAG_SCALE | MI_FLAG_RES | MI_FLAG_LN | MI_FLAG_STATS)) == MI_FLAG_GELU,
               "conv rows x6: LINEAR + GELU, CONVTR or GLU (epi %d, flags %d)", d.epi, d.flags);
    return launch_tile_rows_x6<MI_EPI_LINEAR, MI_FLAG_GELU>(d, tile, st);
}

int launch_conv_x6(const mi_conv_desc &d, int tile, bool plain, hipStream_t st) {
    g_last_conv_route = 4;
    MI_REQUIRE(d.wx && ((uintptr_t)d.wx & 15) == 0, "conv x6: split weight image missing or misaligned");
#define MI_DISPATCH(E)                                              \
    case E: return plain ? launch_tile_x6<E, 0, true>(d, tile, st) : launch_tile_x6<E, 0, false>(d, tile, st)
#define MI_LINEAR(F)                                                \
    case F: return plain ? launch_tile_x6<MI_EPI_LINEAR, F, true>(d, tile, st) : launch_tile_x6<MI_EPI_LINEAR, F, false>(d, tile, st)
    if (d.epi == MI_EPI_LINEAR) {
        switch (d.flags & (MI_FLAG_GELU | MI_FLAG_SCALE | MI_FLAG_RES | MI_FLAG_LN | MI_FLAG_STATS)) {
            MI_LINEAR(0);
            MI_LINEAR(MI_FLAG_GELU);
            MI_LINEAR(MI_FLAG_RES);
            MI_LINEAR(MI_FLAG_SCALE | MI_FLAG_RES);
            MI_LINEAR(MI_FLAG_SCALE | MI_FLAG_RES | MI_FLAG_STATS);
            MI_LINEAR(MI_FLAG_LN);
            MI_LINEAR(MI_FLAG_LN | MI_FLAG_GELU);
        }
        return set_error(MI_EINVAL, "conv: unsupported LINEAR flag combination %d", d.flags);
    }
#undef MI_LINEAR
    switch (d.epi) {
        MI_DISPATCH(MI_EPI_GLU);
        MI_DISPATCH(MI_EPI_BIAS_STATS);
        MI_DISPATCH(MI_EPI_STATS_ONLY);
        MI_DISPATCH(MI_EPI_GN_GLU);
        MI_DISPATCH(MI_EPI_CONVTR);
    }
#undef MI_DISPATCH
    return set_error(MI_EINVAL, "conv: unsupported epilogue %d", d.epi);
}

}
```

### demucs_amd/csrc/kernels.h

```cpp
#pragma once
#include <cmath>
#include <vector>
#include <hip/hip_runtime.h>
#include <stdint.h>

#include "gemm_conv.h"

namespace mi {

struct FftTables {
    const float *window;
    const float2 *twiddle;
    const float *envelope;
};
static inline std::vector<float2> fft_twiddle_table() {
    std::vector<float2> tw(2048);
    for (int i = 0; i < 2048; ++i) { const double a = -2.0 * M_PI * i / 4096.0; tw[i] = make_float2((float)cos(a), (float)sin(a)); }
    return tw;
}

int launch_stft_frames(const float *mix, int B, int L, const FftTables &tb, float *zt, double *stats, hipStream_t st);
int launch_cac_transpose(const float *zt, int B, int T, const float2 *norm, float *x, hipStream_t st, int x_pitch = 0 );
int launch_istft(const float *y, int B, int S, int L, const float2 *denorm, const float *xt, const float2 *denorm_t,
                 const FftTables &tb, float *yt, float *fr, float *out, hipStream_t st, int xt_pitch = 0 ,
// ... 5 lines not shown
int launch_row_stats(const float *x, int rows, int64_t count, int64_t row_stride, double *stats, hipStream_t st);
int launch_finalize_stats(double *stats, int rows, double count, float eps, int mode, float2 *out_a, float2 *out_b,
                          hipStream_t st);
int launch_row_affine(const float *x, int rows, int64_t count, const float2 *norm, float *y, hipStream_t st);
int launch_row_denorm(const float *x, int rows, int64_t count, const float2 *denorm, float *y, hipStream_t st);
int launch_layernorm_cf(const float *x, int B, int C, int T, const float *w, const float *b, const float *pe, float *y,
                        float2 *ostat, hipStream_t st, void *img = nullptr, int64_t img_n = 0, int img_dtype = 0);
int launch_token_stats(const float *x, int B, int C, int T, float2 *ostat, hipStream_t st, void *img = nullptr, int64_t img_n = 0,
                       int img_dtype = 0);
int launch_gn_apply_tokstats(const float *x, int B, int C, int T, const float2 *gstat, const float *w, const float *b, float *y,
                             float2 *ostat, hipStream_t st, void *img = nullptr, int64_t img_n = 0, int img_dtype = 0);

int gram_hp(int h);
int launch_gn_gelu_gram(float *x, int B, int h, int Cs, int D1, int D2 , int pitch, int row_mode, const float2 *stats, const float *w,
                        const float *b, double *gram , int slots, bool zero_pad, hipStream_t st);
int launch_gram_finalize(double *gram, int rows, int h, int slots, const double *wt , const double *ct , double sum_b,
                         double sum_bsq, double cols, double count, float eps, float2 *out, hipStream_t st);
int launch_gn_gelu(float *x, int B, int C, int Cs, int D1, int D2, int row_mode, const float2 *stats, const float *w, const float *b,
                   hipStream_t st);

struct DConvRowLayer {
    const float *w0;
    const float *b0;
    const float *g1w, *g1b;
    const float *w3;
    const float *b3, *g2w, *g2b;
    const float *ls;
};
struct DConvTimeLayer {
    DConvRowLayer w;
    const double *gram_a;
    const double *gram_v;
    const double *gram_c;
    const double *gram_e1, *gram_e2;
    double sum_b3, sum_b3sq;
};
struct DConvRowArgs {
    DConvTimeLayer l[2];
    const float *x;
    float *y;
    int Fr, T;
};
bool dconv_row_supported(int C, int T);
int launch_dconv_row(const DConvRowArgs &a, int C, int rows, hipStream_t st);

bool dconv_time_supported(int C, int Lp);
int launch_dconv_time_layer(const DConvTimeLayer &l, int C, int dil, int B, int Lv, int Lp, const float *x, float *y, float *hbuf,
                            double *stats, double *gram, float2 *st1, float2 *st2, hipStream_t st);

int launch_conv(const mi_conv_desc &d, hipStream_t st);
int conv_pick_tile(int M);
extern int g_split_bf16;
bool conv_x6_supported(int tile);
int launch_conv_x6(const mi_conv_desc &d, int tile, bool plain, hipStream_t st);
int launch_conv_tap_x6(const mi_conv_desc &d, int tile, hipStream_t st);
int launch_conv_rows_x6(const mi_conv_desc &d, int tile, hipStream_t st);
int launch_pack_split(const float *wt, int Kpad, int Mpad, int tile_m, void *wx, hipStream_t st);

int launch_conv_half(const mi_conv_desc &d, int tile, bool plain, hipStream_t st);
int launch_pack_half(const float *wt, int Kpad, int Mpad, int dtype, void *wh, hipStream_t st);
int conv_tap_pairs_pad(int Cin, int ntaps);
int launch_pack_tap(const float *wt, int Mpad, int Cin, int ntaps, int dtype, void *out, hipStream_t st);
int launch_conv_tap(const mi_conv_desc &d, int tile, hipStream_t st);
int launch_f32_to_image(const float *x, int B, int C, int64_t P, int dtype, void *img, hipStream_t st);

int launch_row_affine_pitch(const float *x, int B, int C, int L, int out_pitch, const float2 *norm, float *y, hipStream_t st);
int launch_gn_apply(const float *x, int B, int Cin, int G, int in_pitch, int off, const float2 *stats, const float *w, const float *bias,
                    int glu, int gelu, const float *scale, const float *res, int res_pitch, float *y, int Cout, int out_len,
                    int out_pitch, hipStream_t st, int chan_div = 1);
int launch_unfold_frames(const float *x, int B, int C, int T, int F, int W, int S, float *fr, hipStream_t st);
int launch_restitch_frames(const float *fr, int B, int C, int T, int F, int W, int S, const float *skip, float *y, hipStream_t st);
void pack_lstm_whh(const float *whh , int H, float *packed);
int launch_lstm_seq(const float *gx, const float *whh , int N, int H, int W, float *out, float *state , hipStream_t st);
size_t lstm_persist_scratch_bytes();
size_t lstm_persist_ctl_offset();
int launch_lstm_persist(const float *gx, const float *whh , int N, int H, int W, float *out, void *scratch, unsigned *ctl_host,
                        hipStream_t st);
int launch_lstm_small(const float *gx, const float *whh_natural , int N, int H, int W, float *out, hipStream_t st);
int launch_local_attn(const float *qkc, int B, int C, int T, int ld , float *out, int ld_o, hipStream_t st);

int launch_attention(const float *q, const float *k, const float *v, float *o, int B, int heads, int Tq, int Tk, int64_t q_bs,
                     int64_t kv_bs, int64_t o_bs, int dtype, hipStream_t st, void *oh = nullptr, int64_t oh_n = 0);
int launch_attention_x6(const float *q, const float *k, const float *v, float *o, int B, int heads, int Tq, int Tk, int64_t q_bs,
                        int64_t kv_bs, int64_t o_bs, hipStream_t st);

int launch_segments_gather(const float *track, int64_t track_len, int channels, const int64_t *starts_dev, int B, int valid,
                           float *seg, hipStream_t st);
int launch_ola_accumulate(float *acc, int64_t acc_len, int rows, const float *model_out, int valid, const int64_t *offs_dev,
                          const int32_t *lens_dev, const int32_t *trim_dev, int B, int64_t span_lo, int64_t span_hi,
                          const float *weight, int weight_len, hipStream_t st);
int launch_ola_finish(float *acc, int64_t acc_len, int rows, int64_t acc_off0, const int64_t *offs_dev, const int32_t *lens_dev,
                      int n_segments, int max_len, const float *weight, hipStream_t st);

int launch_segments_gather_packed(const float *tracks, int64_t tracks_cap, int channels, const int64_t *items_dev, int B, int valid,
                                  float *seg, hipStream_t st);
int launch_ola_accumulate_packed(float *acc, int64_t acc_cap, int rows, const float *model_out, int valid, const int64_t *items_dev,
                                 int B, const int64_t *tiles_dev, int n_tiles, const float *weights, int64_t weights_cap,
                                 hipStream_t st);
int launch_ola_finish_packed(float *acc, int64_t acc_cap, int rows, const int64_t *tiles_dev, int n_tiles, const int64_t *segs_dev,
                             int n_segs, const float *weights, int64_t weights_cap, hipStream_t st);

int launch_resample_frac(const float *x, int rows, int64_t L, const float *table, int old_sr, int new_sr, int width, float *y,
                         int64_t Lout, hipStream_t st);

int launch_streams_convert_append(float *win, int64_t win_cap, int channels, const int64_t *table, int n_streams, int64_t max_groups,
                                  const float *bank, int64_t bank_cap, float *hist, int64_t hist_cap, const float *stats, int n_stats,
                                  int lds_floats, hipStream_t st);

const void *conv_zero_page();
int launch_attention_heads(const void *q, const void *k, const void *v, const void *zero_page, int B, int heads, int Tq, int Tk, int Tq_pitch,
                           int Tk_pitch, int dtype, void *oh, int64_t oh_n, float *o, int64_t o_bs, hipStream_t st);

int post_stats_scratch_bytes();
int launch_mono_stats(const float *wav, int channels, int64_t length, double *scratch, float *stats, hipStream_t st);
int launch_stream_emit(const float *acc, int64_t acc_cap, int n_sources, int channels, const int64_t *passes, int n_passes,
                       const int64_t *segs, int n_segs, const float *weights, int64_t weights_cap, const float *scales, int n_members,
                       int shifts, int bag, const float *stats, int64_t n, float *out, hipStream_t st);
int launch_streams_emit(const float *acc, int64_t acc_cap, int n_sources, int channels, const int64_t *streams, int n_streams, int64_t max_n,
                        const int64_t *passes, int n_passes, const int64_t *segs, int n_segs, const float *weights, int64_t weights_cap,
                        const float *scales, int n_members, int shifts, int bag, const float *stats, int n_stats, float *out,
                        int64_t out_cap, hipStream_t st);
int launch_streams_append(float *win, int64_t win_cap, int channels, const int64_t *table, int n_streams, int64_t max_n,
                          const float *stats, int n_stats, hipStream_t st);
int launch_streams_compact(float *dst, int64_t dst_cap, const float *src, int64_t src_cap, const int64_t *table, int n_rows, int64_t max_len,
                           hipStream_t st);
int launch_track_affine(float *x, int64_t n, const float *stats, int mode, hipStream_t st);
int launch_prevent_clip(const float *x, int64_t n, int mode, unsigned *peak, float *y, hipStream_t st);
int launch_two_stems(const float *const *stems, int S, int sel, const float *origin, int mode, int64_t n, float *y, hipStream_t st);

}
```

### demucs_amd/csrc/model.hip

```cpp
#include <cmath>
#include <map>
#include <memory>
#include <mutex>
#include <string>
#include <vector>

#include "common.h"
#include "gemm_conv.h"
#include "kernels.h"
#include "model.h"
#include "model_internal.h"

namespace mi {

int Model::dev_alloc(void **p, size_t bytes) {
    bytes = (bytes + 255) & ~(size_t)255;
    hipError_t e = hipMalloc(p, bytes);
    if (e != hipSuccess) return set_error(MI_ENOMEM, "hipMalloc(%zu) failed: %s", bytes, hipGetErrorString(e));
    allocs.push_back(*p);
    device_bytes += (int64_t)bytes;
    return MI_OK;
}

template <typename T>
// ... 21 lines not shown
        int least = 0, greatest = 0;
        MI_HIP(hipDeviceGetStreamPriorityRange(&least, &greatest));
        MI_HIP(hipStreamCreateWithPriority(&side_st, hipStreamNonBlocking, prio[0] == 'l' ? least : greatest));
    } else
        MI_HIP(hipStreamCreateWithFlags(&side_st, hipStreamNonBlocking));
    MI_HIP(hipEventCreateWithFlags(&ev_main, hipEventDisableTiming));
    MI_HIP(hipEventCreateWithFlags(&ev_side, hipEventDisableTiming));
    return MI_OK;
}

hipEvent_t Profiler::get() {
    if (!pool.empty()) { hipEvent_t e = pool.back(); pool.pop_back(); return e; }
    hipEvent_t e;
    (void)hipEventCreate(&e);
    return e;
}
void Profiler::begin() {
    for (auto &r : rows) r = ProfRow();
    on = true;
}
int Profiler::end(hipStream_t st) {
    on = false;
    MI_HIP(hipStreamSynchronize(st));
    for (auto &p : pending) {
        float ms = 0.f;
        MI_HIP(hipEventElapsedTime(&ms, p.a, p.b));
        ProfRow &r = rows[p.cls];
        r.cls = p.cls; r.launches += p.launches; r.ms += ms; r.flops += p.flops; r.bytes += p.bytes;
        pool.push_back(p.a); pool.push_back(p.b);
    }
    pending.clear();
    return MI_OK;
}
Profiler::~Profiler() {
    for (auto &p : pending) { (void)hipEventDestroy(p.a); (void)hipEventDestroy(p.b); }
    for (auto e : pool) (void)hipEventDestroy(e);
}

static const char *kEpiNames[6] = {"linear", "glu", "bias_stats", "stats_only", "gn_glu", "convtr"};

static int conv_class(const mi_conv_desc &d, int tile) {
    const int ti = tile == 32 ? 0 : tile == 64 ? 1 : tile == 96 ? 2 : 3;
    const bool x6 = d.half || (d.wx && g_split_bf16 && conv_x6_supported(tile));
    return (x6 ? 48 : 0) + d.epi * 8 + ti * 2 + (d.plain ? 1 : 0);
}

int Model::conv(const mi_conv_desc &d, hipStream_t st) {
    if (!prof.on) return launch_conv(d, st);
    const int tile = d.tile_m ? d.tile_m : conv_pick_tile(d.M);
    const int cls = conv_class(d, tile);
    const double N = (double)d.B * d.O1 * d.O2;
    const double in_bytes = 4.0 * (double)d.B * (double)d.x_bstride;
    double out_rows = d.M;
    if (d.epi == MI_EPI_GLU || d.epi == MI_EPI_GN_GLU) out_rows = d.M / 2;
    if (d.epi == MI_EPI_CONVTR) out_rows = d.M;
    if (d.epi == MI_EPI_STATS_ONLY) out_rows = 0;
    double bytes = in_bytes + 4.0 * out_rows * N + 4.0 * (double)d.M * d.K;
    if (d.flags & MI_FLAG_RES || d.epi == MI_EPI_GN_GLU) bytes += 4.0 * out_rows * N;
    Profiler::Pending p{cls, prof.get(), prof.get(), 2.0 * d.M * (double)d.K * N, bytes};
    MI_HIP(hipEventRecord(p.a, st));
    const int r = launch_conv(d, st);
    MI_HIP(hipEventRecord(p.b, st));
    const bool tap_x6 = r == MI_OK && g_last_conv_route == 7, rows_x6 = r == MI_OK && g_last_conv_route == 8;
    if (tap_x6) p.cls = 105 + (d.ntaps == 9 ? 2 : 0) + (tile == 128 ? 1 : 0);
    if (rows_x6) p.cls = 109 + (d.epi == MI_EPI_CONVTR ? 4 : d.epi == MI_EPI_GLU ? 2 : 0) + (tile == 128 ? 1 : 0);
    prof.pending.push_back(p);
    ProfRow &row = prof.rows[p.cls];
    if (!row.name[0] && tap_x6)
        snprintf(row.name, sizeof(row.name), "conv_tap_x6<%s,tile%d,taps%d>", kEpiNames[d.epi], tile, d.ntaps);
    else if (!row.name[0] && rows_x6)
        snprintf(row.name, sizeof(row.name), "conv_rows_x6<%s,tile%d>", kEpiNames[d.epi], tile);
    else if (!row.name[0])
        snprintf(row.name, sizeof(row.name), "conv_gemm%s<%s,tile%d%s>", d.half == MI_DTYPE_BF16 ? "_bf16" : d.half == MI_DTYPE_F16 ? "_f16" : cls >= 48 ? "_x6" : "",
                 kEpiNames[d.epi], tile, d.plain ? ",1x1" : "");
    return r;
}

static int x6_scope() {
    static const char *env = getenv("MI_X6");
    static const int scope = env ? (atoi(env) != 0 ? 2 : 0) : 1;
    return scope;
}

int Model::attn(const float *q, const float *k, const float *v, float *o, int B, int Tq, int Tk, int64_t q_bs, int64_t kv_bs,
                int64_t o_bs, hipStream_t st, bool image) {
    void *oh = image ? (void *)o : nullptr;
    const int64_t oh_n = (int64_t)B * Tq;
    const bool x6 = cfg.dtype == MI_DTYPE_F32 && !image && g_split_bf16 && x6_scope() != 0;
    auto launch = [&]() {
        return x6 ? launch_attention_x6(q, k, v, o, B, 8, Tq, Tk, q_bs, kv_bs, o_bs, st)
                  : launch_attention(q, k, v, o, B, 8, Tq, Tk, q_bs, kv_bs, o_bs, cfg.dtype, st, oh, oh_n);
    };
    if (!prof.on) return launch();
    const int cls = x6 ? 104 : 100;
    Profiler::Pending p{cls, prof.get(), prof.get(), 4.0 * B * 8 * (double)Tq * Tk * 64.0,
                        4.0 * B * 512.0 * (2.0 * Tq + 2.0 * Tk)};
    MI_HIP(hipEventRecord(p.a, st));
    const int r = launch();
    MI_HIP(hipEventRecord(p.b, st));
    prof.pending.push_back(p);
    snprintf(prof.rows[cls].name, sizeof(prof.rows[cls].name), "attention%s_kernel",
             x6 ? "_x6" : cfg.dtype == MI_DTYPE_BF16 ? "_bf16" : cfg.dtype == MI_DTYPE_F16 ? "_f16" : "");
    return r;
}

int Model::attn_heads(const void *q, const void *k, const void *v, float *o, int B, int Tq, int Tk, hipStream_t st) {
    const int64_t oh_n = (int64_t)B * Tq;
    const void *zero = conv_zero_page();
    MI_REQUIRE(zero, "attention: could not allocate the zero page");
    if (!prof.on) return launch_attention_heads(q, k, v, zero, B, 8, Tq, Tk, Tq, Tk, cfg.dtype, o, oh_n, nullptr, 0, st);
    const int cls = 100;
    Profiler::Pending p{cls, prof.get(), prof.get(), 4.0 * B * 8 * (double)Tq * Tk * 64.0, 2.0 * B * 512.0 * (2.0 * Tq + 2.0 * Tk)};
    MI_HIP(hipEventRecord(p.a, st));
    const int r = launch_attention_heads(q, k, v, zero, B, 8, Tq, Tk, Tq, Tk, cfg.dtype, o, oh_n, nullptr, 0, st);
    MI_HIP(hipEventRecord(p.b, st));
    prof.pending.push_back(p);
    snprintf(prof.rows[cls].name, sizeof(prof.rows[cls].name), "attention_heads%s_kernel", cfg.dtype == MI_DTYPE_BF16 ? "_bf16" : "_f16");
    return r;
}

int Model::pack_split(PackedConv *pc) {
    const int scope = x6_scope();
    static const bool no_rows = getenv("MI_NO_DMA_ROWS") != nullptr;
    const bool want = scope == 2 || (scope == 1 && (split_linears || split_taps || (split_rows && !no_rows)) && cfg.dtype == MI_DTYPE_F32);
    if (!want || !conv_x6_supported(pc->tile)) return MI_OK;
    MI_TRY(dev_alloc(&pc->wx, (size_t)6 * pc->Kpad * pc->Mpad));
    MI_TRY(launch_pack_split(pc->wt, pc->Kpad, pc->Mpad, pc->tile, pc->wx, nullptr));
    MI_HIP(hipStreamSynchronize(nullptr));
    return MI_OK;
}

int Model::pack_half(PackedConv *pc) {
    if (cfg.dtype == MI_DTYPE_F32) return MI_OK;
    const int Kh = round_up(pc->Kpad, 32);
    MI_TRY(dev_alloc(&pc->wh, (size_t)2 * Kh * pc->Mpad));
    pc->half = cfg.dtype;
    MI_TRY(launch_pack_half(pc->wt, pc->Kpad, pc->Mpad, cfg.dtype, pc->wh, nullptr));
    MI_HIP(hipStreamSynchronize(nullptr));
    return MI_OK;
}

int Model::pack_tap(PackedConv *pc, int ntaps) {
    static const bool no_tap = getenv("MI_NO_TAP_IMAGE") != nullptr;
    if (cfg.dtype == MI_DTYPE_F32 || no_tap || ntaps < 2 || pc->K % ntaps || (pc->K / ntaps) % 8) return MI_OK;
    const int Cin = pc->K / ntaps;
    MI_TRY(dev_alloc(&pc->wtap, (size_t)16 * conv_tap_pairs_pad(Cin, ntaps) * pc->Mpad));
    pc->ntaps = ntaps;
    MI_TRY(launch_pack_tap(pc->wt, pc->Mpad, Cin, ntaps, cfg.dtype, pc->wtap, nullptr));
    MI_HIP(hipStreamSynchronize(nullptr));
    return MI_OK;
}

int Model::pack_enc_tap(const float *W , int Cin, PackedConv *pc) {
    static const bool off = getenv("MI_NO_ENC_IMAGE") != nullptr || getenv("MI_NO_TAP_IMAGE") != nullptr;
    if (cfg.dtype == MI_DTYPE_F32 || off || Cin % 8) return MI_OK;
    const int M = pc->M, K = 8 * Cin;
    std::vector<float> wt((size_t)K * pc->Mpad, 0.f);
    for (int m = 0; m < M; ++m)
        for (int ci = 0; ci < Cin; ++ci)
            for (int rho = 0; rho < 4; ++rho)
                for (int j = 0; j < 2; ++j) {
                    const int tau = 4 * (j - (rho >= 2)) + rho + 2, ce = ((ci >> 3) * 4 + rho) * 8 + (ci & 7);
                    wt[(size_t)(ce * 2 + j) * pc->Mpad + m] = W[((size_t)m * Cin + ci) * 8 + tau];
                }
    float *tmp = nullptr;
    MI_HIP(hipMalloc((void **)&tmp, wt.size() * sizeof(float)));
    MI_HIP(hipMemcpy(tmp, wt.data(), wt.size() * sizeof(float), hipMemcpyHostToDevice));
    int r = dev_alloc(&pc->wtap, (size_t)16 * conv_tap_pairs_pad(4 * Cin, 2) * pc->Mpad);
    if (r == MI_OK) r = launch_pack_tap(tmp, pc->Mpad, 4 * Cin, 2, cfg.dtype, pc->wtap, nullptr);
    (void)hipStreamSynchronize(nullptr);
    (void)hipFree(tmp);
    if (r == MI_OK) pc->ntaps = 2;
    return r;
// ... 348 lines not shown
                pe1[(size_t)(256 + i) * Tt + t2] = sinf(ph);
            }
        }
        MI_TRY(upload(pe2, &pos_emb[0])); MI_TRY(upload(pe1, &pos_emb[1]));
    }
    MI_TRY(alloc_workspace());
    MI_HIP(hipDeviceSynchronize());
    return MI_OK;
}

int Workspace::alloc(void **p, size_t n) {
    n = (n + 255) & ~(size_t)255;
    hipError_t e = hipMalloc(p, n);
    if (e != hipSuccess) return set_error(MI_ENOMEM, "hipMalloc(%zu) failed: %s", n, hipGetErrorString(e));
    allocs.push_back(*p);
    bytes += (int64_t)n;
    return MI_OK;
}
Workspace::~Workspace() {
    for (void *p : allocs) (void)hipFree(p);
}

static std::mutex g_ws_mutex;
static std::map<std::string, std::weak_ptr<Workspace>> g_ws;

int Model::alloc_workspace() {
    int dev = 0;
    MI_HIP(hipGetDevice(&dev));
    char key[128];
    snprintf(key, sizeof(key), "htdemucs dev%d S%d SL%d B%d %s", dev, S, SL, cfg.max_batch, cfg.dtype == MI_DTYPE_F32 ? "f32" : "half");
    std::lock_guard<std::mutex> lock(g_ws_mutex);
    auto it = g_ws.find(key);
    if (it != g_ws.end()) ws = it->second.lock();
    if (!ws) {
        auto w = std::make_shared<Workspace>();
        w->key = key;
        MI_TRY(fill_workspace(*w));
        g_ws[key] = w;
        ws = w;
    }
    static_cast<WorkspacePtrs &>(*this) = *ws;
    dconv_tap_dma = true;
    return MI_OK;
}

int Model::fill_workspace(Workspace &w) {
    const size_t B = cfg.max_batch;
    auto A = [&](float **p, size_t per_item) { return w.alloc((void **)p, per_item * B * sizeof(float)); };
    auto dev_alloc = [&](void **p, size_t n) { return w.alloc(p, n); };
    MI_TRY(A(&w.w_xt0, (size_t)2 * SL));
    MI_TRY(A(&w.w_zt, (size_t)4 * 2048 * T));
    MI_TRY(A(&w.w_x0, (size_t)4 * 2048 * T));
    size_t big = 0;
    for (int i = 0; i < 4; ++i) {
        const size_t nf = (size_t)kCh[i] * kFr[i + 1] * T, nt = (size_t)kCh[i] * Lp[i + 1];
        MI_TRY(A(&w.w_skip[i], nf)); MI_TRY(A(&w.w_skip_t[i], nt));
        big = std::max(big, std::max(nf, nt));
    }
    if (cfg.dtype != MI_DTYPE_F32)
        for (int i = 0; i < 3; ++i) {
            const size_t pqf = (size_t)(kFr[i + 1] / 4 + 1) * T, pqt = round_up(ceil_div(Lt[i + 1], 4) + 1, 4);
            float *pf = nullptr, *pt = nullptr;
            MI_TRY(A(&pf, 2 * kCh[i] * pqf)); MI_TRY(A(&pt, 2 * kCh[i] * pqt));
            MI_HIP(hipMemset(pf, 0, 2 * kCh[i] * pqf * B * sizeof(float)));
            MI_HIP(hipMemset(pt, 0, 2 * kCh[i] * pqt * B * sizeof(float)));
            w.w_eimg[0][i] = pf; w.w_eimg[1][i] = pt;
        }
    MI_TRY(A(&w.w_h, big / 2)); MI_TRY(A(&w.w_th, big / 2));
    for (float **p : {&w.w_a, &w.w_b, &w.w_ta, &w.w_tb, &w.w_c, &w.w_tc}) {
        MI_TRY(w.alloc((void **)p, (big * B + 64) * sizeof(float)));
        *p += 32;
    }
    MI_HIP(hipMemset(w.w_h, 0, (big / 2) * B * sizeof(float)));
    MI_HIP(hipMemset(w.w_th, 0, (big / 2) * B * sizeof(float)));
    const size_t Tf = 8 * (size_t)T, Tt = Lt[4];
    for (int br = 0; br < 2; ++br) {
        const size_t P = br ? Tt : Tf;
        MI_TRY(A(&w.w_tr_x[br][0], 512 * P)); MI_TRY(A(&w.w_tr_x[br][1], 512 * P));
        if (cfg.dtype != MI_DTYPE_F32) {
            MI_TRY(A(&w.w_tr_ximg[br][0], 256 * P)); MI_TRY(A(&w.w_tr_ximg[br][1], 256 * P)); MI_TRY(A(&w.w_tr_x1img[br], 256 * P));
        }
        for (int q = 0; q < 2; ++q) MI_TRY(dev_alloc((void **)&w.w_tr_stat[br][q], B * P * sizeof(float2)));
        MI_TRY(dev_alloc((void **)&w.w_tr_stat1[br], B * P * sizeof(float2)));
        MI_TRY(A(&w.w_tr_qkv[br], 1536 * Tf)) ; MI_TRY(A(&w.w_tr_att[br], 512 * P));
        MI_TRY(A(&w.w_tr_x1[br], 512 * P)); MI_TRY(A(&w.w_tr_x2[br], 512 * P)); MI_TRY(A(&w.w_tr_ffh[br], 2048 * P));
    }
    MI_TRY(A(&w.w_yspec, (size_t)4 * S * 2048 * T));
    MI_TRY(A(&w.w_ytime, (size_t)2 * S * SL));
    MI_TRY(A(&w.w_yt, (size_t)4 * S * 2048 * T));
    MI_TRY(A(&w.w_fr, (size_t)S * T * 2 * 4096));
    const size_t max_rows = B * 512;
    w.stats_bytes = max_rows * kStatSlots * 2 * sizeof(double);
    MI_TRY(dev_alloc((void **)&w.w_stats, w.stats_bytes));
    MI_TRY(dev_alloc((void **)&w.w_stats_t, w.stats_bytes));
    w.gram_bytes = B * kStatSlots * 96 * sizeof(double);
    MI_TRY(dev_alloc((void **)&w.w_gram, w.gram_bytes));
    MI_HIP(hipMemset(w.w_gram, 0, w.gram_bytes));
    w.gram2_bytes = B * ((size_t)4 << 20);
    MI_TRY(dev_alloc((void **)&w.w_gram2, w.gram2_bytes));
    MI_HIP(hipMemset(w.w_gram2, 0, w.gram2_bytes));
    w.gram2t_bytes = B * ((size_t)1 << 20);
    MI_TRY(dev_alloc((void **)&w.w_gram2_t, w.gram2t_bytes));
    MI_HIP(hipMemset(w.w_gram2_t, 0, w.gram2t_bytes));
    MI_HIP(hipMemset(w.w_stats, 0, w.stats_bytes));
    MI_HIP(hipMemset(w.w_stats_t, 0, w.stats_bytes));
    MI_TRY(dev_alloc((void **)&w.w_st1, max_rows * sizeof(float2)));
    MI_TRY(dev_alloc((void **)&w.w_st2, max_rows * sizeof(float2)));
    MI_TRY(dev_alloc((void **)&w.w_st1_t, max_rows * sizeof(float2)));
    MI_TRY(dev_alloc((void **)&w.w_st2_t, max_rows * sizeof(float2)));
    MI_TRY(dev_alloc((void **)&w.w_norm_f, B * sizeof(float2))); MI_TRY(dev_alloc((void **)&w.w_denorm_f, B * sizeof(float2)));
    MI_TRY(dev_alloc((void **)&w.w_norm_t, B * sizeof(float2))); MI_TRY(dev_alloc((void **)&w.w_denorm_t, B * sizeof(float2)));
    return MI_OK;
}

static bool debug_sync() {
    static const bool on = getenv("MI_DEBUG_SYNC") != nullptr;
    return on;
}
#define MI_STAGE(name)                                                                        \
    do {                                                                                      \
        if (debug_sync()) {                                                                   \
            hipError_t _e = hipStreamSynchronize(st);                                         \
            fprintf(stderr, "[mi] reached %s (%s)\n", name, hipGetErrorString(_e));          \
            fflush(stderr);                                                                   \
            if (_e != hipSuccess) return set_error(MI_EHIP, "stage before %s failed: %s", name, hipGetErrorString(_e)); \
        }                                                                                     \
    } while (0)

int Model::run_dconv(const DConvW &w, int C, const Geo &g, float *x, float *tmp, float *hidden, double *stats, float2 *st1,
                     float2 *st2, hipStream_t st, double *gram2, size_t gram2_cap) {
    if (!gram2) { gram2 = w_gram2; gram2_cap = gram2_bytes; }
    const int h = w.h, hp = round_up(h, 16);
    const int64_t P = (int64_t)g.D1 * g.pitch();
    const int rows = g.row_mode ? g.B * g.D1 : g.B;
    if (w.has_row && g.row_mode == 1) {
        DConvRowArgs a{{w.tl[0], w.tl[1]}, x, x, g.D1, g.D2};
        if (prof.on) {
            Profiler::Pending p{101, prof.get(), prof.get(), 2.0 * 2.0 * (3.0 * C * h + 2.0 * 2 * C * h) * (double)rows * g.D2,
                                2.0 * 4.0 * C * (double)rows * g.D2};
            MI_HIP(hipEventRecord(p.a, st));
            const int r = launch_dconv_row(a, C, rows, st);
            MI_HIP(hipEventRecord(p.b, st));
            prof.pending.push_back(p);
            snprintf(prof.rows[101].name, sizeof(prof.rows[101].name), "dconv_row_kernel");
            return r;
        }
        return launch_dconv_row(a, C, rows, st);
    }
    if (w.has_time && g.row_mode == 0 && g.D1 == 1) {
        const bool timed = prof.on;
        Profiler::Pending p{102, nullptr, nullptr, 2.0 * 2.0 * (3.0 * C * h + 2.0 * C * h) * (double)g.B * g.D2,
                            2.0 * 4.0 * C * (double)g.B * g.D2};
        if (timed) { p.a = prof.get(); p.b = prof.get(); MI_HIP(hipEventRecord(p.a, st)); }
        float *s = x, *dd = tmp;
        for (int dlayer = 0; dlayer < 2; ++dlayer) {
            MI_TRY(launch_dconv_time_layer(w.tl[dlayer], C, 1 << dlayer, g.B, g.D2, g.pitch(), s, dd, hidden, stats, w_gram, st1, st2, st));
            std::swap(s, dd);
        }
        if (timed) {
            MI_HIP(hipEventRecord(p.b, st));
            prof.pending.push_back(p);
            snprintf(prof.rows[102].name, sizeof(prof.rows[102].name), "dconv_time_kernels");
        }
        return MI_OK;
    }
    const double cnt_row = g.row_mode ? (double)g.D2 : (double)g.D1 * g.D2;
    float *src = x, *dst = tmp;
    for (int dlayer = 0; dlayer < 2; ++dlayer) {
        const DConvLayerW &l = w.l[dlayer];
        mi_conv_desc d = base_desc(l.conv3, l.ktab3, src, (int64_t)C * P, g);
        d.epi = MI_EPI_BIAS_STATS; d.y = hidden; d.y_bstride = (int64_t)hp * P; d.y_cstride = P; d.stats = stats;
        if (dconv_tap_dma) {
            d.ntaps = 3; d.tap_k2 = 3; d.tap_pad1 = 0; d.tap_pad2 = 1 << dlayer; d.tap_dil2 = 1 << dlayer;
        }
        MI_TRY(conv(d, st));
        MI_TRY(launch_finalize_stats(stats, rows, cnt_row * h, 1e-5f, 0, st1, nullptr, st));
        const int gslots = g.row_mode ? 1 : 8, HP = gram_hp(h);
        MI_REQUIRE((size_t)rows * gslots * HP * HP * sizeof(double) <= gram2_cap, "dconv: Gram accumulators need %zu bytes, workspace has %zu",
                   (size_t)rows * gslots * HP * HP * sizeof(double), gram2_cap);
        MI_TRY(launch_gn_gelu_gram(hidden, g.B, h, hp, g.D1, g.D2, g.pitch(), g.row_mode, st1, l.gn1_w, l.gn1_b, gram2, gslots, true, st));
        MI_TRY(launch_gram_finalize(gram2, rows, h, gslots, l.gram_wt, l.gram_ct, l.sum_b, l.sum_bsq, cnt_row, cnt_row * 2 * C, 1e-5f, st2, st));
        mi_conv_desc e = base_desc(l.conv1, l.ktab1, hidden, (int64_t)hp * P, g);
        e.plain = 1;
        e.epi = MI_EPI_GN_GLU; e.stats = nullptr; e.gn_stats = (const float *)st2; e.gn_w = l.gn2_w; e.gn_b = l.gn2_b;
        e.scale = l.ls; e.res = src; e.y = dst; e.y_bstride = (int64_t)C * P; e.y_cstride = P;
        MI_TRY(conv(e, st));
        std::swap(src, dst);
    }
    return MI_OK;
}

int Model::run_tr_layer(int br, int k, int B, const float *x, const float2 *xstat, const float *other, const float2 *ostat,
                        float *out, float2 *outstat, hipStream_t st, const void *ximg, const void *oimg, void *outimg) {
    const TrLayerW &l = tr[br][k];
    const bool cross = k & 1;
    const int Tf = 8 * T, Tt = Lt[4];
    const int Tq = br ? Tt : Tf, Tk = cross ? (br ? Tf : Tt) : Tq;
    const Geo gq{B, 1, Tq, 0}, gk{B, 1, Tk, 0};
    float *qkv = w_tr_qkv[br], *att = w_tr_att[br], *x1 = w_tr_x1[br], *x2 = w_tr_x2[br], *ffh = w_tr_ffh[br];
    double *stats = br ? w_stats_t : w_stats;
    float2 *st1 = br ? w_st1_t : w_st1;
    static const bool lin2_stats = getenv("MI_NO_LIN2_STATS") == nullptr;
    static const bool no_img = getenv("MI_NO_FFN_IMAGE") != nullptr;
    const bool img = cfg.dtype != MI_DTYPE_F32 && !no_img;
    static const bool no_heads = getenv("MI_NO_QKV_HEADS") != nullptr;
    const bool heads = img && !no_heads;
    unsigned short *qh = reinterpret_cast<unsigned short *>(qkv);
    const size_t plane_q = (size_t)B * 512 * Tq, plane_k = (size_t)B * 512 * Tk;
    if (!cross) {
        mi_conv_desc d = base_desc(l.qkv_proj, tr_ktab512[br], x, (int64_t)512 * Tq, gq);
        d.plain = 1; d.epi = MI_EPI_LINEAR; d.flags = MI_FLAG_LN; d.scale = l.qkv_c1; d.pro_stats = (const float *)xstat;
        d.y = qkv; d.y_bstride = (int64_t)1536 * Tq; d.y_cstride = Tq;
        if (heads) { d.flags |= MI_FLAG_HEADS; d.yh = qh; d.yh_n = Tq; }
        if (heads && ximg) { d.xh = ximg; d.xh_n = (int64_t)B * Tq; }
        MI_TRY(conv(d, st));
        if (heads) MI_TRY(attn_heads(qh, qh + plane_q, qh + 2 * plane_q, att, B, Tq, Tq, st));
        else MI_TRY(attn(qkv, qkv + (size_t)512 * Tq, qkv + (size_t)1024 * Tq, att, B, Tq, Tq, (int64_t)1536 * Tq, (int64_t)1536 * Tq,
                         (int64_t)512 * Tq, st, img));
    } else {
        mi_conv_desc d = base_desc(l.q_proj, tr_ktab512[br], x, (int64_t)512 * Tq, gq);
        d.plain = 1; d.epi = MI_EPI_LINEAR; d.flags = MI_FLAG_LN; d.scale = l.q_c1; d.pro_stats = (const float *)xstat;
        d.y = qkv; d.y_bstride = (int64_t)512 * Tq; d.y_cstride = Tq;
        if (heads) { d.flags |= MI_FLAG_HEADS; d.yh = qh; d.yh_n = Tq; }
        if (heads && ximg) { d.xh = ximg; d.xh_n = (int64_t)B * Tq; }
        MI_TRY(conv(d, st));
        float *kv = qkv + (size_t)B * 512 * Tq;
        unsigned short *kvh = qh + plane_q;
        mi_conv_desc e = base_desc(l.kv_proj, tr_ktab512[1 - br], other, (int64_t)512 * Tk, gk);
        e.plain = 1; e.epi = MI_EPI_LINEAR; e.flags = MI_FLAG_LN; e.scale = l.kv_c1; e.pro_stats = (const float *)ostat;
        e.y = kv; e.y_bstride = (int64_t)1024 * Tk; e.y_cstride = Tk;
        if (heads) { e.flags |= MI_FLAG_HEADS; e.yh = kvh; e.yh_n = Tk; }
        if (heads && oimg) { e.xh = oimg; e.xh_n = (int64_t)B * Tk; }
        MI_TRY(conv(e, st));
        if (heads) MI_TRY(attn_heads(qh, kvh, kvh + plane_k, att, B, Tq, Tk, st));
        else MI_TRY(attn(qkv, kv, kv + (size_t)512 * Tk, att, B, Tq, Tk, (int64_t)512 * Tq, (int64_t)1024 * Tk, (int64_t)512 * Tq, st, img));
    }
    {
        mi_conv_desc d = base_desc(l.out_proj, tr_ktab512[br], att, (int64_t)512 * Tq, gq);
        d.plain = 1; d.epi = MI_EPI_LINEAR; d.flags = MI_FLAG_SCALE | MI_FLAG_RES; d.scale = l.gamma1; d.res = x;
        d.y = x1; d.y_bstride = (int64_t)512 * Tq; d.y_cstride = Tq;
        if (img) { d.xh = att; d.xh_n = (int64_t)B * Tq; }
        MI_TRY(conv(d, st));
    }
    const bool in_img = heads && ximg != nullptr;
    MI_TRY(launch_token_stats(x1, B, 512, Tq, w_tr_stat1[br], st, in_img ? w_tr_x1img[br] : nullptr, (int64_t)B * Tq, cfg.dtype));
    {
        mi_conv_desc d = base_desc(l.lin1, tr_ktab512[br], x1, (int64_t)512 * Tq, gq);
        d.plain = 1; d.epi = MI_EPI_LINEAR; d.flags = MI_FLAG_LN | MI_FLAG_GELU; d.scale = l.lin1_c1;
        d.pro_stats = (const float *)w_tr_stat1[br];
        d.y = ffh; d.y_bstride = (int64_t)2048 * Tq; d.y_cstride = Tq;
        if (img) { d.flags |= MI_FLAG_IMG; d.yh = ffh; d.yh_n = (int64_t)B * Tq; }
        if (img && in_img) { d.xh = w_tr_x1img[br]; d.xh_n = (int64_t)B * Tq; }
        MI_TRY(conv(d, st));
        mi_conv_desc e = base_desc(l.lin2, tr_ktab2048[br], ffh, (int64_t)2048 * Tq, gq);
        if (img) { e.xh = ffh; e.xh_n = (int64_t)B * Tq; }
        e.plain = 1; e.epi = MI_EPI_LINEAR; e.flags = MI_FLAG_SCALE | MI_FLAG_RES; e.scale = l.gamma2; e.res = x1;
        if (lin2_stats) { e.flags |= MI_FLAG_STATS; e.stats = stats; }
        e.y = x2; e.y_bstride = (int64_t)512 * Tq; e.y_cstride = Tq;
        MI_TRY(conv(e, st));
    }
    if (!lin2_stats) MI_TRY(launch_row_stats(x2, B, (int64_t)512 * Tq, (int64_t)512 * Tq, stats, st));
    MI_TRY(launch_finalize_stats(stats, B, (double)512 * Tq, 1e-5f, 0, st1, nullptr, st));
    MI_TRY(launch_gn_apply_tokstats(x2, B, 512, Tq, st1, l.norm_w[3], l.norm_b[3], out, outstat, st, in_img ? outimg : nullptr,
                                    (int64_t)B * Tq, cfg.dtype));
    return MI_OK;
}

int Model::run_core(const float *mix, const float *mag, int B, hipStream_t st) {
    if (ws->dirty) {
        MI_HIP(hipMemsetAsync(w_stats, 0, ws->stats_bytes, st));
        MI_HIP(hipMemsetAsync(w_stats_t, 0, ws->stats_bytes, st));
        MI_HIP(hipMemsetAsync(w_gram, 0, ws->gram_bytes, st));
        MI_HIP(hipMemsetAsync(w_gram2, 0, gram2_bytes, st));
        MI_HIP(hipMemsetAsync(w_gram2_t, 0, gram2t_bytes, st));
        ws->dirty = false;
    }
    const int r = run_core_impl(mix, mag, B, st);
    if (r != MI_OK) {
        ws->dirty = true;
        if (side_st) (void)hipStreamSynchronize(side_st);
    }
    return r;
}

int Model::forward(const float *mix, float *out, int B, hipStream_t st) {
    MI_REQUIRE(mix && out, "forward: null buffer");
    MI_TRY(run_core(mix, nullptr, B, st));
    MI_TRY(launch_istft(w_yspec, B, S, SL, w_denorm_f, w_ytime, w_denorm_t, fft, w_yt, w_fr, out, st));
    MI_STAGE("istft done");
    return MI_OK;
}

int Model::forward_core(const float *mix, const float *mag, float *spec_out, float *time_out, int B, hipStream_t st) {
    MI_REQUIRE(mix && spec_out && time_out, "forward_core: null buffer");
    MI_TRY(run_core(mix, mag, B, st));
    MI_TRY(launch_row_denorm(w_yspec, B, (int64_t)4 * S * 2048 * T, w_denorm_f, spec_out, st));
    MI_TRY(launch_row_denorm(w_ytime, B, (int64_t)2 * S * SL, w_denorm_t, time_out, st));
    return MI_OK;
}

int Model::run_core_impl(const float *mix, const float *mag, int B, hipStream_t st) {
    MI_REQUIRE(B >= 1 && B <= cfg.max_batch, "forward: batch %d outside [1, %d]", B, cfg.max_batch);
    const int Tf = 8 * T, Tt = Lt[4];
    static const bool one_stream = getenv("MI_ONE_STREAM") != nullptr;
    const bool two = !one_stream && g_two_streams && !debug_sync() && side_streams() == MI_OK;
    hipStream_t stt = two ? side_st : st;
    auto fork = [&]() -> int {
        if (!two) return MI_OK;
        MI_HIP(hipEventRecord(ev_main, st));
        MI_HIP(hipStreamWaitEvent(side_st, ev_main, 0));
        return MI_OK;
    };
    auto join = [&]() -> int {
        if (!two) return MI_OK;
        MI_HIP(hipEventRecord(ev_side, side_st));
        MI_HIP(hipStreamWaitEvent(st, ev_side, 0));
        return MI_OK;
    };
    MI_TRY(fork());
    MI_TRY(launch_row_stats(mix, B, (int64_t)2 * SL, (int64_t)2 * SL, w_stats_t, stt));
    MI_TRY(launch_finalize_stats(w_stats_t, B, 2.0 * SL, 1e-5f, 1, w_norm_t, w_denorm_t, stt));
    MI_TRY(launch_row_affine(mix, B, (int64_t)2 * SL, w_norm_t, w_xt0, stt));
    MI_STAGE("time normalisation done");
    if (mag) {
        const int64_t cnt = (int64_t)4 * 2048 * T;
        MI_TRY(launch_row_stats(mag, B, cnt, cnt, w_stats, st));
        MI_TRY(launch_finalize_stats(w_stats, B, (double)cnt, 1e-5f, 1, w_norm_f, w_denorm_f, st));
        MI_TRY(launch_row_affine(mag, B, cnt, w_norm_f, w_x0, st));
    } else {
        MI_TRY(launch_stft_frames(mix, B, SL, fft, w_zt, w_stats, st));
        MI_TRY(launch_finalize_stats(w_stats, B, 4.0 * 2048 * T, 1e-5f, 1, w_norm_f, w_denorm_f, st));
        MI_TRY(launch_cac_transpose(w_zt, B, T, w_norm_f, w_x0, st));
    }
    MI_STAGE("stft done");

    const float *xf = w_x0, *xt = w_xt0;
    for (int i = 0; i < 4; ++i) {
        const int Cin = i ? kCh[i - 1] : 4, Cint = i ? kCh[i - 1] : 2, C = kCh[i];
        {
            const Geo gin{B, kFr[i], T, 1}, go{B, kFr[i + 1], T, 1};
            const int64_t Pin = (int64_t)kFr[i] * T, P = (int64_t)kFr[i + 1] * T;
            mi_conv_desc d = base_desc(enc[i].conv, enc[i].ktab_conv, xf, Cin * Pin, gin);
            d.O1 = kFr[i + 1]; d.S1 = 4; d.epi = MI_EPI_LINEAR; d.flags = MI_FLAG_GELU;
            d.y = w_a; d.y_bstride = C * P; d.y_cstride = P;
            d.dma_rows = 1;
            if (i && enc[i].conv.wtap && w_eimg[0][i - 1]) {
                const int Q = kFr[i] / 4 + 1;
                d.xh = w_eimg[0][i - 1]; d.xh_n = (int64_t)cfg.max_batch * Q * T; d.wtap = enc[i].conv.wtap; d.ntaps = 2; d.tap_k2 = 1;
                d.D1 = Q; d.S1 = 1;
            }
            MI_TRY(conv(d, st));
            MI_STAGE("enc conv done");
            MI_TRY(run_dconv(enc[i].dconv, C, go, w_a, w_b, w_h, w_stats, w_st1, w_st2, st));
            MI_STAGE("enc dconv done");
            mi_conv_desc r = base_desc(enc[i].rewrite, enc[i].ktab_rw, w_a, C * P, go);
            r.plain = 1; r.epi = MI_EPI_GLU; r.y = w_skip[i]; r.y_bstride = C * P; r.y_cstride = P;
            if (i == 0) { r.flags = MI_FLAG_EMB; r.emb = freq_emb; }
            if (i < 3 && enc[i + 1].conv.wtap && w_eimg[0][i]) {
                const int64_t pq = (int64_t)(kFr[i + 1] / 4 + 1) * T;
                r.flags |= MI_FLAG_IMG4 | MI_FLAG_TR_FREQ; r.yh = w_eimg[0][i]; r.yh_pq = pq; r.yh_n = (int64_t)cfg.max_batch * pq;
            }
            MI_TRY(conv(r, st));
            xf = w_skip[i];
            MI_STAGE("enc rewrite done");
        }
        {
            const Geo gin{B, 1, Lt[i], 0, Lp[i]}, go{B, 1, Lt[i + 1], 0, Lp[i + 1]};
            const int64_t P = Lp[i + 1];
            mi_conv_desc d = base_desc(tenc[i].conv, tenc[i].ktab_conv, xt, (int64_t)Cint * Lp[i], gin);
            d.O2 = Lp[i + 1]; d.o2_valid = Lt[i + 1]; d.S2 = 4; d.epi = MI_EPI_LINEAR; d.flags = MI_FLAG_GELU;
            d.y = w_ta; d.y_bstride = C * P; d.y_cstride = P;
            if (i && tenc[i].conv.wtap && w_eimg[1][i - 1]) {
                const int Qp = round_up(ceil_div(Lt[i], 4) + 1, 4);
                d.xh = w_eimg[1][i - 1]; d.xh_n = (int64_t)cfg.max_batch * Qp; d.wtap = tenc[i].conv.wtap; d.ntaps = 2; d.tap_k2 = 2;
                d.D2 = Qp; d.x_ld = Qp; d.S2 = 1;
            }
            MI_TRY(conv(d, stt));
            MI_TRY(run_dconv(tenc[i].dconv, C, go, w_ta, w_tb, w_th, w_stats_t, w_st1_t, w_st2_t, stt, w_gram2_t, gram2t_bytes));
            mi_conv_desc r = base_desc(tenc[i].rewrite, tenc[i].ktab_rw, w_ta, C * P, go);
            r.plain = 1; r.epi = MI_EPI_GLU; r.y = w_skip_t[i]; r.y_bstride = C * P; r.y_cstride = P;
            if (i < 3 && tenc[i + 1].conv.wtap && w_eimg[1][i]) {
                const int64_t pq = round_up(ceil_div(Lt[i + 1], 4) + 1, 4);
                r.flags |= MI_FLAG_IMG4; r.yh = w_eimg[1][i]; r.yh_pq = pq; r.yh_n = (int64_t)cfg.max_batch * pq;
            }
            MI_TRY(conv(r, stt));
            xt = w_skip_t[i];
            MI_STAGE("tenc layer done");
        }
    }
    int cur[2] = {0, 0};
    static const bool no_in_img = getenv("MI_NO_INPUT_IMAGE") != nullptr || getenv("MI_NO_QKV_HEADS") != nullptr || getenv("MI_NO_FFN_IMAGE") != nullptr;
    const bool in_img = cfg.dtype != MI_DTYPE_F32 && !no_in_img;
    for (int br = 0; br < 2; ++br) {
        const int P = br ? Tt : Tf;
        const Geo g{B, 1, P, 0};
        hipStream_t sb = br ? stt : st;
        mi_conv_desc d = base_desc(chan[br], chan_ktab[br], br ? xt : xf, (int64_t)384 * P, g);
        d.plain = 1; d.epi = MI_EPI_LINEAR; d.y = w_tr_x1[br]; d.y_bstride = (int64_t)512 * P; d.y_cstride = P;
        MI_TRY(conv(d, sb));
        MI_TRY(launch_layernorm_cf(w_tr_x1[br], B, 512, P, norm_in_w[br], norm_in_b[br], pos_emb[br], w_tr_x[br][0],
                                   w_tr_stat[br][0], sb, in_img ? w_tr_ximg[br][0] : nullptr, (int64_t)B * P, cfg.dtype));
    }
    MI_STAGE("upsample + norm_in done");
    for (int k = 0; k < 5; ++k) {
        const float *f_in = w_tr_x[0][cur[0]], *t_in = w_tr_x[1][cur[1]];
        const float2 *f_st = w_tr_stat[0][cur[0]], *t_st = w_tr_stat[1][cur[1]];
        const void *f_img = in_img ? w_tr_ximg[0][cur[0]] : nullptr, *t_img = in_img ? w_tr_ximg[1][cur[1]] : nullptr;
        MI_TRY(join());
        MI_TRY(fork());
        MI_TRY(run_tr_layer(0, k, B, f_in, f_st, t_in, t_st, w_tr_x[0][cur[0] ^ 1], w_tr_stat[0][cur[0] ^ 1], st, f_img, t_img,
                            w_tr_ximg[0][cur[0] ^ 1]));
        MI_TRY(run_tr_layer(1, k, B, t_in, t_st, f_in, f_st, w_tr_x[1][cur[1] ^ 1], w_tr_stat[1][cur[1] ^ 1], stt, t_img, f_img,
                            w_tr_ximg[1][cur[1] ^ 1]));
        cur[0] ^= 1; cur[1] ^= 1;
        MI_STAGE("transformer layer done");
    }
    float *din = w_c, *dtin = w_tc;
    const bool tapimg = cfg.dtype != MI_DTYPE_F32 && dec[0].rewrite.wtap && tdec[0].rewrite.wtap;
    for (int br = 0; br < 2; ++br) {
        const int P = br ? Tt : Tf;
        const Geo g{B, 1, P, 0};
        mi_conv_desc d = base_desc(chan[2 + br], chan_ktab[2 + br], w_tr_x[br][cur[br]], (int64_t)512 * P, g);
        d.plain = 1; d.epi = MI_EPI_LINEAR; d.flags = MI_FLAG_RES; d.res = br ? w_skip_t[3] : w_skip[3];
        d.y = br ? dtin : din; d.y_bstride = (int64_t)384 * P; d.y_cstride = P;
        if (tapimg) { d.flags |= MI_FLAG_IMG; d.yh = br ? dtin : din; d.yh_n = (int64_t)B * P; }
        MI_TRY(conv(d, br ? stt : st));
    }
    for (int j = 0; j < 4; ++j) {
        const int C = kCh[3 - j], Fr = kFr[4 - j];
        const bool last = j == 3;
        {
            const Geo g{B, Fr, T, 1};
            const int64_t P = (int64_t)Fr * T;
            mi_conv_desc r = base_desc(dec[j].rewrite, dec[j].ktab_rw, din, C * P, g);
            r.epi = MI_EPI_GLU; r.y = w_a; r.y_bstride = C * P; r.y_cstride = P;
            r.ntaps = 9; r.tap_k2 = 3; r.tap_pad1 = 1; r.tap_pad2 = 1;
            if (tapimg) { r.xh = din; r.xh_n = (int64_t)B * P; r.wtap = dec[j].rewrite.wtap; }
            MI_TRY(conv(r, st));
            MI_TRY(run_dconv(dec[j].dconv, C, g, w_a, w_b, w_h, w_stats, w_st1, w_st2, st));
            const int Cout = last ? 4 * S : kCh[2 - j];
            mi_conv_desc t = base_desc(dec[j].convtr, dec[j].ktab_tr, w_a, C * P, g);
            t.O1 = Fr + 1; t.epi = MI_EPI_CONVTR; t.flags = MI_FLAG_TR_FREQ; t.out_len = 4 * Fr;
            t.y_cstride = (int64_t)4 * Fr * T; t.y_bstride = Cout * t.y_cstride;
            t.dma_rows = 1;
            if (last) t.y = w_yspec;
            else { t.flags |= MI_FLAG_GELU | MI_FLAG_RES; t.res = w_skip[2 - j]; t.y = din; }
            if (!last && tapimg) { t.flags |= MI_FLAG_IMG; t.yh = din; t.yh_n = (int64_t)B * t.y_cstride; }
            if (tapimg && dec[j].convtr.wtap && !last) {
                MI_TRY(launch_f32_to_image(w_a, B, C, P, cfg.dtype, w_b, st));
                t.xh = w_b; t.xh_n = (int64_t)B * P; t.wtap = dec[j].convtr.wtap; t.ntaps = 2; t.tap_k2 = 1; t.tap_dil1 = -1;
            }
            MI_TRY(conv(t, st));
            MI_STAGE("dec freq layer done");
        }
        {
            const int Lv = Lt[4 - j], L = Lp[4 - j], Lout = Lt[3 - j], Lpo = Lp[3 - j];
            const Geo g{B, 1, Lv, 0, L};
            mi_conv_desc r = base_desc(tdec[j].rewrite, tdec[j].ktab_rw, dtin, (int64_t)C * L, g);
            r.epi = MI_EPI_GLU; r.y = w_ta; r.y_bstride = (int64_t)C * L; r.y_cstride = L;
            r.ntaps = 3; r.tap_k2 = 3; r.tap_pad1 = 0; r.tap_pad2 = 1;
            if (tapimg) { r.xh = dtin; r.xh_n = (int64_t)B * L; r.wtap = tdec[j].rewrite.wtap; }
            MI_TRY(conv(r, stt));
            MI_TRY(run_dconv(tdec[j].dconv, C, g, w_ta, w_tb, w_th, w_stats_t, w_st1_t, w_st2_t, stt, w_gram2_t, gram2t_bytes));
            const int Cout = last ? 2 * S : kCh[2 - j];
            mi_conv_desc t = base_desc(tdec[j].convtr, tdec[j].ktab_tr, w_ta, (int64_t)C * L, g);
            t.O2 = Lv + 1; t.o2_valid = 0; t.epi = MI_EPI_CONVTR; t.out_len = Lout;
            t.y_cstride = Lpo; t.y_bstride = (int64_t)Cout * Lpo;
            if (last) t.y = w_ytime;
            else { t.flags |= MI_FLAG_GELU | MI_FLAG_RES; t.res = w_skip_t[2 - j]; t.y = dtin; }
            if (!last && tapimg) { t.flags |= MI_FLAG_IMG; t.yh = dtin; t.yh_n = (int64_t)B * t.y_cstride; }
            if (tapimg && tdec[j].convtr.wtap && !last) {
                MI_TRY(launch_f32_to_image(w_ta, B, C, L, cfg.dtype, w_tb, stt));
                t.xh = w_tb; t.xh_n = (int64_t)B * L; t.wtap = tdec[j].convtr.wtap; t.ntaps = 2; t.tap_k2 = 2; t.tap_dil2 = -1;
            }
            MI_TRY(conv(t, stt));
        }
    }
    MI_TRY(join());
    MI_STAGE("decoders done");
    return MI_OK;
}

}
```

### demucs_amd/csrc/norms.hip

```cpp
#include "common.h"
#include "kernels.h"

namespace mi {

__device__ __forceinline__ double wave_sum(double v) {
#pragma unroll
    for (int off = 32; off > 0; off >>= 1) v += __shfl_xor(v, off);
    return v;
}

__device__ __forceinline__ void block_sum2(double &a, double &b, double *red ) {
    a = wave_sum(a); b = wave_sum(b);
    const int w = threadIdx.x >> 6;
    if ((threadIdx.x & 63) == 0) { red[2 * w] = a; red[2 * w + 1] = b; }
    __syncthreads();
    if (threadIdx.x == 0) { a = red[0] + red[2] + red[4] + red[6]; b = red[1] + red[3] + red[5] + red[7]; }
}

__global__ __launch_bounds__(256) void row_stats_kernel(const float *__restrict__ x, int64_t count, int64_t row_stride,
                                                        double *__restrict__ stats) {
    __shared__ double red[8];
    const float *p = x + (size_t)blockIdx.y * row_stride;
    const int64_t per = (count + gridDim.x - 1) / gridDim.x;
    const int64_t lo = (int64_t)blockIdx.x * per, hi = min(count, lo + per);
    double s1 = 0.0, s2 = 0.0;
    for (int64_t base = lo; base < hi; base += 256 * 16) {
        float a = 0.f, q = 0.f;
#pragma unroll
        for (int j = 0; j < 16; ++j) {
            const int64_t i = base + threadIdx.x + 256 * j;
            if (i < hi) { const float v = p[i]; a += v; q += v * v; }
        }
        s1 += a; s2 += q;
    }
    block_sum2(s1, s2, red);
    if (threadIdx.x == 0) {
        double *dst = stats + ((size_t)blockIdx.y * kStatSlots + (blockIdx.x % kStatSlots)) * 2;
        atomicAdd(dst, s1); atomicAdd(dst + 1, s2);
    }
}

__global__ void finalize_stats_kernel(double *__restrict__ stats, int rows, double count, float eps, int mode,
                                      float2 *__restrict__ out_a, float2 *__restrict__ out_b) {
    const int row = blockIdx.x * blockDim.x + threadIdx.x;
    if (row >= rows) return;
    double s1 = 0.0, s2 = 0.0;
    for (int s = 0; s < kStatSlots; ++s) {
        double *p = stats + ((size_t)row * kStatSlots + s) * 2;
        s1 += p[0]; s2 += p[1];
        p[0] = 0.0; p[1] = 0.0;
    }
    const double mean = s1 / count;
    double m2 = s2 - s1 * mean;
    if (m2 < 0.0) m2 = 0.0;
    if (mode == 0) {
        const float var = (float)(m2 / count);
        out_a[row] = make_float2((float)mean, 1.0f / sqrtf(var + eps));
    } else {
        const float sd = (float)sqrt(m2 / (count - 1.0));
        out_a[row] = make_float2((float)mean, 1.0f / (eps + sd));
        if (out_b) out_b[row] = make_float2((float)mean, sd);
    }
}

__global__ __launch_bounds__(256) void row_affine_kernel(const float *__restrict__ x, int64_t count, const float2 *__restrict__ norm,
                                                         float *__restrict__ y) {
    const float2 nm = norm[blockIdx.y];
    const size_t base = (size_t)blockIdx.y * count;
    for (int64_t i = (int64_t)blockIdx.x * 256 + threadIdx.x; i < count; i += (int64_t)gridDim.x * 256)
        y[base + i] = (x[base + i] - nm.x) * nm.y;
}

template <int MODE>
__global__ __launch_bounds__(256) void token_tile_kernel(const float *__restrict__ x, int C, int T, const float *__restrict__ w,
                                                         const float *__restrict__ bvec, const float *__restrict__ pe,
                                                         const float2 *__restrict__ gstat, float eps, float *__restrict__ y,
                                                         float2 *__restrict__ ostat, uint4 *__restrict__ img, int64_t img_n, int img_dtype) {
    __shared__ float red[4][64][2];
    const int lane = threadIdx.x & 63, wv = __builtin_amdgcn_readfirstlane(threadIdx.x >> 6);
    const int t = blockIdx.x * 64 + lane;
    const bool ok = t < T;
    const size_t base = (size_t)blockIdx.y * C * T + (ok ? t : 0);
    const int cw = C / 4, c0 = wv * cw;
    const float inv_c = 1.0f / (float)C;
    float mean = 0.f, rstd = 1.f;
    if (MODE == 0 || MODE == 1) {
        const float x0 = x[base];
        float s1 = 0.f, s2 = 0.f;
        if (MODE == 1 && img) {
            for (int c = c0; c < c0 + cw; c += 8) {
                float q[8];
#pragma unroll
                for (int e = 0; e < 8; ++e) {
                    q[e] = x[base + (size_t)(c + e) * T];
                    const float v = q[e] - x0;
                    s1 += v; s2 += v * v;
                }
                if (ok) img[(size_t)(c >> 3) * img_n + (size_t)blockIdx.y * T + t] =
                    make_uint4(pack_half2(img_dtype, q[0], q[1]), pack_half2(img_dtype, q[2], q[3]), pack_half2(img_dtype, q[4], q[5]),
                               pack_half2(img_dtype, q[6], q[7]));
            }
        } else
        for (int c = c0; c < c0 + cw; ++c) {
            const float v = x[base + (size_t)c * T] - x0;
            s1 += v; s2 += v * v;
        }
        red[wv][lane][0] = s1; red[wv][lane][1] = s2;
        __syncthreads();
        s1 = red[0][lane][0] + red[1][lane][0] + red[2][lane][0] + red[3][lane][0];
        s2 = red[0][lane][1] + red[1][lane][1] + red[2][lane][1] + red[3][lane][1];
        const float dm = s1 * inv_c;
        mean = x0 + dm;
        rstd = 1.0f / sqrtf(fmaxf(s2 * inv_c - dm * dm, 0.f) + eps);
        if (MODE == 1) {
            if (ok && wv == 0) ostat[(size_t)blockIdx.y * T + t] = make_float2(mean, rstd);
            return;
        }
        __syncthreads();
    } else {
        const float2 g = gstat[blockIdx.y];
        mean = g.x; rstd = g.y;
    }
    float y0;
    {
        float v = (x[base] - mean) * rstd * w[0] + bvec[0];
        if (MODE == 0 && pe) v += pe[ok ? t : 0];
        y0 = v;
    }
    float s1 = 0.f, s2 = 0.f;
    int c = c0;
    for (; c + 8 <= c0 + cw; c += 8) {
        float xv[8], pv[8], q8[8];
#pragma unroll
        for (int e = 0; e < 8; ++e) xv[e] = x[base + (size_t)(c + e) * T];
        if (MODE == 0 && pe) {
#pragma unroll
            for (int e = 0; e < 8; ++e) pv[e] = pe[(size_t)(c + e) * T + (ok ? t : 0)];
        }
#pragma unroll
        for (int e = 0; e < 8; ++e) {
            float v = (xv[e] - mean) * rstd * w[c + e] + bvec[c + e];
            if (MODE == 0 && pe) v += pv[e];
            if (ok) y[base + (size_t)(c + e) * T] = v;
            const float dv = v - y0;
            s1 += dv; s2 += dv * dv;
            q8[e] = v;
        }
        if (img && ok)
            img[(size_t)(c >> 3) * img_n + (size_t)blockIdx.y * T + t] =
                make_uint4(pack_half2(img_dtype, q8[0], q8[1]), pack_half2(img_dtype, q8[2], q8[3]), pack_half2(img_dtype, q8[4], q8[5]),
                           pack_half2(img_dtype, q8[6], q8[7]));
    }
    for (; c < c0 + cw; ++c) {
        float v = (x[base + (size_t)c * T] - mean) * rstd * w[c] + bvec[c];
        if (MODE == 0 && pe) v += pe[(size_t)c * T + (ok ? t : 0)];
        if (ok) y[base + (size_t)c * T] = v;
        const float dv = v - y0;
        s1 += dv; s2 += dv * dv;
    }
    if (!ostat) return;
    red[wv][lane][0] = s1; red[wv][lane][1] = s2;
    __syncthreads();
    if (ok && wv == 0) {
        s1 = red[0][lane][0] + red[1][lane][0] + red[2][lane][0] + red[3][lane][0];
        s2 = red[0][lane][1] + red[1][lane][1] + red[2][lane][1] + red[3][lane][1];
        const float dm = s1 * inv_c;
        ostat[(size_t)blockIdx.y * T + t] = make_float2(y0 + dm, 1.0f / sqrtf(fmaxf(s2 * inv_c - dm * dm, 0.f) + eps));
    }
}

__global__ __launch_bounds__(256) void gn_gelu_kernel(float *__restrict__ x, int C, int Cs, int D1, int D2, int row_mode,
                                                      const float2 *__restrict__ st, const float *__restrict__ w,
                                                      const float *__restrict__ bvec) {
    const int p = blockIdx.x * 256 + threadIdx.x;
    if (p >= D1 * D2) return;
    const int c = blockIdx.y, b = blockIdx.z;
    const float2 s = st[row_mode ? b * D1 + p / D2 : b];
    const size_t i = ((size_t)b * Cs + c) * D1 * D2 + p;
    x[i] = gelu_exact((x[i] - s.x) * s.y * w[c] + bvec[c]);
}

int launch_gn_gelu(float *x, int B, int C, int Cs, int D1, int D2, int row_mode, const float2 *stats, const float *w, const float *b,
                   hipStream_t st) {
    hipLaunchKernelGGL(gn_gelu_kernel, dim3(ceil_div((int64_t)D1 * D2, 256), C, B), dim3(256), 0, st, x, C, Cs, D1, D2, row_mode, stats, w, b);
    MI_CHECK_LAUNCH();
    return MI_OK;
}

typedef float gram_f32x16 __attribute__((ext_vector_type(16)));
template <int HP>
__global__ __launch_bounds__(256) void gn_gelu_gram_kernel(float *__restrict__ x, int h, int Cs, int D1, int D2, int pitch, int row_mode,
                                                           const float2 *__restrict__ st, const float *__restrict__ w,
                                                           const float *__restrict__ bvec, double *__restrict__ gram, int slots,
                                                           int zero_pad) {
    constexpr int CT = HP > 96 ? 64 : 128, CG = 256 / CT, LDG = CT + 1, NT = HP / 32;
    __shared__ float Gs[HP][LDG];
    const int tid = threadIdx.x, row = blockIdx.y, col = tid & (CT - 1), cg = tid / CT;
    const int b = row_mode ? row / D1 : row, d1 = row_mode ? row % D1 : 0;
    const int cols = row_mode ? D2 : D1 * D2;
    const int q = blockIdx.x * CT + col;
    const bool ok = q < cols;
    const float2 s = st[row];
    float *xp = x + (size_t)b * Cs * D1 * pitch + (size_t)d1 * pitch + q;
    float v[HP / CG];
#pragma unroll
    for (int k = 0; k < HP / CG; ++k) {
        const int c = cg + k * CG;
        v[k] = (c < h && ok) ? xp[(size_t)c * D1 * pitch] : 0.f;
    }
#pragma unroll
    for (int k = 0; k < HP / CG; ++k) {
        const int c = cg + k * CG;
        float g = 0.f;
        if (c < h && ok) {
            g = gelu_exact((v[k] - s.x) * s.y * w[c] + bvec[c]);
            xp[(size_t)c * D1 * pitch] = g;
        } else if (ok) {
            if (c == h) g = 1.f;
            if (zero_pad && c < Cs) xp[(size_t)c * D1 * pitch] = 0.f;
        }
        Gs[c][col] = g;
    }
    __syncthreads();
    const int lane = tid & 63, wave = tid >> 6, li = lane & 31, lh = lane >> 5;
    double *gout = gram + ((size_t)row * slots + blockIdx.x % slots) * HP * HP;
    int t = 0;
    for (int ti = 0; ti < NT; ++ti)
        for (int tj = ti; tj < NT; ++tj, ++t) {
            if (t % 4 != wave) continue;
            if (ti * 32 > h) continue;
            gram_f32x16 acc;
#pragma unroll
            for (int r = 0; r < 16; ++r) acc[r] = 0.f;
            const float *ga = &Gs[ti * 32 + li][lh], *gb = &Gs[tj * 32 + li][lh];
// ... 22 lines not shown
        for (int sl = 0; sl < 8; ++sl) v[sl] = sl < slots ? p[(size_t)sl * HP * HP] : 0.0;
#pragma unroll
        for (int sl = 0; sl < 8; ++sl)
            if (sl < slots) p[(size_t)sl * HP * HP] = 0.0;
        const double acc = ((v[0] + v[1]) + (v[2] + v[3])) + ((v[4] + v[5]) + (v[6] + v[7]));
        s2 += wt[e] * acc;
        if (j == h) s1 += ct[i] * acc;
    }
    for (int off = 32; off > 0; off >>= 1) { s1 += __shfl_down(s1, off); s2 += __shfl_down(s2, off); }
    if ((tid & 63) == 0) { red[0][tid >> 6] = s1; red[1][tid >> 6] = s2; }
    __syncthreads();
    if (tid == 0) {
        s1 = red[0][0] + red[0][1] + red[0][2] + red[0][3] + cols * sum_b;
        s2 = red[1][0] + red[1][1] + red[1][2] + red[1][3] + cols * sum_bsq;
        const double mean = s1 / count;
        double m2 = s2 - s1 * mean;
        if (m2 < 0.0) m2 = 0.0;
        out[row] = make_float2((float)mean, 1.0f / sqrtf((float)(m2 / count) + eps));
    }
}

int gram_hp(int h) { return (h + 1 + 31) / 32 * 32; }

int launch_gn_gelu_gram(float *x, int B, int h, int Cs, int D1, int D2, int pitch, int row_mode, const float2 *stats, const float *w,
                        const float *b, double *gram, int slots, bool zero_pad, hipStream_t st) {
    const int HP = gram_hp(h), rows = row_mode ? B * D1 : B, cols = row_mode ? D2 : D1 * D2;
    MI_REQUIRE(HP <= 128, "gn_gelu_gram: %d hidden channels not instantiated", h);
    MI_REQUIRE(!zero_pad || Cs <= HP, "gn_gelu_gram: %d allocated channels, the pass zeroes padding up to %d", Cs, HP);
    MI_REQUIRE(row_mode || D1 == 1 || pitch == D2, "gn_gelu_gram: a per-item row needs contiguous positions");
    const dim3 grid(ceil_div(cols, HP > 96 ? 64 : 128), rows);
    if (HP == 32) hipLaunchKernelGGL(gn_gelu_gram_kernel<32>, grid, dim3(256), 0, st, x, h, Cs, D1, D2, pitch, row_mode, stats, w, b, gram, slots, (int)zero_pad);
    else if (HP == 64) hipLaunchKernelGGL(gn_gelu_gram_kernel<64>, grid, dim3(256), 0, st, x, h, Cs, D1, D2, pitch, row_mode, stats, w, b, gram, slots, (int)zero_pad);
    else if (HP == 96) hipLaunchKernelGGL(gn_gelu_gram_kernel<96>, grid, dim3(256), 0, st, x, h, Cs, D1, D2, pitch, row_mode, stats, w, b, gram, slots, (int)zero_pad);
    else hipLaunchKernelGGL(gn_gelu_gram_kernel<128>, grid, dim3(256), 0, st, x, h, Cs, D1, D2, pitch, row_mode, stats, w, b, gram, slots, (int)zero_pad);
    MI_CHECK_LAUNCH();
    return MI_OK;
}

int launch_gram_finalize(double *gram, int rows, int h, int slots, const double *wt, const double *ct, double sum_b, double sum_bsq,
                         double cols, double count, float eps, float2 *out, hipStream_t st) {
    MI_REQUIRE(slots >= 1 && slots <= 8, "gram_finalize: %d accumulator slots (1..8)", slots);
    hipLaunchKernelGGL(gram_finalize_kernel, dim3(rows), dim3(256), 0, st, gram, gram_hp(h), slots, h, wt, ct, sum_b, sum_bsq, cols, count, eps, out);
    MI_CHECK_LAUNCH();
    return MI_OK;
}

int launch_row_stats(const float *x, int rows, int64_t count, int64_t row_stride, double *stats, hipStream_t st) {
    const int nblk = (int)std::min<int64_t>(256, (count + 4095) / 4096);
    hipLaunchKernelGGL(row_stats_kernel, dim3(nblk, rows), dim3(256), 0, st, x, count, row_stride, stats);
    MI_CHECK_LAUNCH();
    return MI_OK;
}

int launch_finalize_stats(double *stats, int rows, double count, float eps, int mode, float2 *out_a, float2 *out_b,
                          hipStream_t st) {
    hipLaunchKernelGGL(finalize_stats_kernel, dim3(ceil_div(rows, 64)), dim3(64), 0, st, stats, rows, count, eps, mode, out_a, out_b);
    MI_CHECK_LAUNCH();
    return MI_OK;
}

__global__ __launch_bounds__(256) void row_denorm_kernel(const float *__restrict__ x, int64_t count, const float2 *__restrict__ denorm,
                                                         float *__restrict__ y) {
    const float2 d = denorm[blockIdx.y];
    const size_t base = (size_t)blockIdx.y * count;
    for (int64_t i = (int64_t)blockIdx.x * 256 + threadIdx.x; i < count; i += (int64_t)gridDim.x * 256)
        y[base + i] = x[base + i] * d.y + d.x;
}

int launch_row_denorm(const float *x, int rows, int64_t count, const float2 *denorm, float *y, hipStream_t st) {
    const int nblk = (int)std::min<int64_t>(2048, (count + 255) / 256);
    hipLaunchKernelGGL(row_denorm_kernel, dim3(nblk, rows), dim3(256), 0, st, x, count, denorm, y);
    MI_CHECK_LAUNCH();
    return MI_OK;
}

int launch_row_affine(const float *x, int rows, int64_t count, const float2 *norm, float *y, hipStream_t st) {
    const int nblk = (int)std::min<int64_t>(1024, (count + 255) / 256);
    hipLaunchKernelGGL(row_affine_kernel, dim3(nblk, rows), dim3(256), 0, st, x, count, norm, y);
    MI_CHECK_LAUNCH();
    return MI_OK;
}

static int check_img(int C, const void *img, int64_t img_n, int B, int T, int dtype) {
    MI_REQUIRE(!img || (C % 32 == 0 && img_n >= (int64_t)B * T && ((uintptr_t)img & 15) == 0 && (dtype == MI_DTYPE_BF16 || dtype == MI_DTYPE_F16)),
               "token kernel: operand image needs C %% 32 == 0, >= B * T columns, 16-byte alignment and a half dtype");
    return MI_OK;
}

int launch_layernorm_cf(const float *x, int B, int C, int T, const float *w, const float *b, const float *pe, float *y,
                        float2 *ostat, hipStream_t st, void *img, int64_t img_n, int img_dtype) {
    MI_REQUIRE(C % 4 == 0, "layernorm: C %% 4 != 0");
    MI_TRY(check_img(C, img, img_n, B, T, img_dtype));
    hipLaunchKernelGGL(token_tile_kernel<0>, dim3(ceil_div(T, 64), B), dim3(256), 0, st, x, C, T, w, b, pe, nullptr, 1e-5f, y, ostat,
                       (uint4 *)img, img_n, img_dtype);
    MI_CHECK_LAUNCH();
    return MI_OK;
}

int launch_token_stats(const float *x, int B, int C, int T, float2 *ostat, hipStream_t st, void *img, int64_t img_n, int img_dtype) {
    MI_REQUIRE(C % 4 == 0, "token_stats: C %% 4 != 0");
    MI_TRY(check_img(C, img, img_n, B, T, img_dtype));
    hipLaunchKernelGGL(token_tile_kernel<1>, dim3(ceil_div(T, 64), B), dim3(256), 0, st, x, C, T, nullptr, nullptr, nullptr, nullptr,
                       1e-5f, nullptr, ostat, (uint4 *)img, img_n, img_dtype);
    MI_CHECK_LAUNCH();
    return MI_OK;
}

int launch_gn_apply_tokstats(const float *x, int B, int C, int T, const float2 *gstat, const float *w, const float *b, float *y,
                             float2 *ostat, hipStream_t st, void *img, int64_t img_n, int img_dtype) {
    MI_REQUIRE(C % 4 == 0, "gn_apply: C %% 4 != 0");
    MI_TRY(check_img(C, img, img_n, B, T, img_dtype));
    hipLaunchKernelGGL(token_tile_kernel<2>, dim3(ceil_div(T, 64), B), dim3(256), 0, st, x, C, T, w, b, nullptr, gstat, 1e-5f, y, ostat,
                       (uint4 *)img, img_n, img_dtype);
    MI_CHECK_LAUNCH();
    return MI_OK;
}

}
```

### include/demucs_amd.h

```cpp
#ifndef DEMUCS_AMD_H
#define DEMUCS_AMD_H

#include <stddef.h>
#include <stdint.h>

#ifdef __cplusplus
extern "C" {
#endif

#define MI_OK 0
#define MI_EINVAL (-1)
#define MI_EHIP (-2)
#define MI_ENOMEM (-3)
#define MI_EWEIGHT (-4)

typedef struct mi_tensor_desc {
    const char *name;
    const float *data;
    int64_t numel;
} mi_tensor_desc;

typedef struct mi_config {
    int32_t n_sources;
    int32_t segment_length;
// ... 123 lines not shown
#define MI_CVT_SRC_CH 1
#define MI_CVT_N_IN 2
#define MI_CVT_BEFORE 3
#define MI_CVT_HIST_LEN 4
#define MI_CVT_HIST_RD 5
#define MI_CVT_HIST_WR 6
#define MI_CVT_HIST_START 7
#define MI_CVT_HIST_NEXT 8
#define MI_CVT_OUT0 9
#define MI_CVT_N_OUT 10
#define MI_CVT_TOTAL 11
#define MI_CVT_OLD 12
#define MI_CVT_NEW 13
#define MI_CVT_WIDTH 14
#define MI_CVT_BANK_OFF 15
#define MI_CVT_DST_OFF 16
#define MI_CVT_DST_LEN 17
#define MI_CVT_COL 18
#define MI_CVT_STATS 19
#define MI_CVT_COLS 20
#define MI_CVT_LDS_FLOATS 16384
int mi_streams_convert_append(float *win_dev, int64_t win_capacity, int32_t channels, const int64_t *table_dev, int32_t n_streams,
                              int64_t max_groups, const float *bank_dev, int64_t bank_capacity, float *hist_dev, int64_t hist_capacity,
                              const float *stats_dev, int32_t n_stats, int32_t lds_floats, void *stream);

int mi_resample_frac(const float *x_dev, int32_t rows, int64_t length, const float *table_dev, int32_t old_sr, int32_t new_sr,
                     int32_t width, float *y_dev, int64_t out_length, void *stream);

int32_t mi_mono_stats_scratch_bytes(void);
int mi_mono_stats(const float *wav_dev, int32_t channels, int64_t length, void *scratch_dev, float *stats_dev, void *stream);
int mi_track_affine(float *x_dev, int64_t numel, const float *stats_dev, int32_t inverse, void *stream);

#define MI_CLIP_RESCALE 1
#define MI_CLIP_CLAMP 2
#define MI_CLIP_TANH 3
int mi_prevent_clip(const float *x_dev, int64_t numel, int32_t mode, void *peak_dev, float *y_dev, void *stream);
int mi_two_stems(const float *const *stems_dev, int32_t n_stems, int32_t selected, const float *origin_dev, int32_t minus, int64_t numel,
                 float *y_dev, void *stream);

int mi_stft_cac(const float *mix_dev, int32_t B, int32_t L, float *cac_dev, void *stream);
int mi_istft_cac(const float *x_dev, int32_t B, int32_t S, int32_t L, float *wav_dev, void *stream);

struct mi_conv_desc;
int mi_conv_forward(const struct mi_conv_desc *desc, void *stream);

int mi_conv_pack_split(const float *wt_dev, int32_t Kpad, int32_t Mpad, int32_t tile_m, void *wx_dev, void *stream);

int mi_conv_pack_tap(const float *wt_dev, int32_t Mpad, int32_t Cin, int32_t ntaps, int32_t dtype, void *wtap_dev, void *stream);
int mi_f32_to_image(const float *x_dev, int32_t B, int32_t C, int64_t P, int32_t dtype, void *img_dev, void *stream);

int mi_conv_pack_half(const float *wt_dev, int32_t Kpad, int32_t Mpad, int32_t dtype, void *wh_dev, void *stream);

int mi_attention(const float *q_dev, const float *k_dev, const float *v_dev, float *o_dev, int32_t B, int32_t heads,
                 int32_t Tq, int32_t Tk, int64_t q_batch_stride, int64_t kv_batch_stride, int64_t o_batch_stride,
                 int32_t dtype, void *stream);

int mi_attention_split(const float *q_dev, const float *k_dev, const float *v_dev, float *o_dev, int32_t B, int32_t heads,
                       int32_t Tq, int32_t Tk, int64_t q_batch_stride, int64_t kv_batch_stride, int64_t o_batch_stride,
                       void *stream);

int mi_attention_heads(const void *q_dev, const void *k_dev, const void *v_dev, float *o_dev, int32_t B, int32_t heads, int32_t Tq, int32_t Tk,
                       int32_t Tq_pitch, int32_t Tk_pitch, int32_t dtype, void *stream);

int mi_attention_image(const float *q_dev, const float *k_dev, const float *v_dev, void *img_dev, int64_t n_img, int32_t B,
                       int32_t heads, int32_t Tq, int32_t Tk, int64_t q_batch_stride, int64_t kv_batch_stride, int32_t dtype,
                       void *stream);

int mi_gn_gelu(float *x_dev, int32_t B, int32_t C, int32_t C_alloc, int32_t D1, int32_t D2, int32_t row_mode, const float *stats_dev,
               const float *w_dev, const float *b_dev, void *stream);

int32_t mi_gram_order(int32_t h);
int mi_gn_gelu_gram(float *x_dev, int32_t B, int32_t h, int32_t C_alloc, int32_t D1, int32_t D2, int32_t pitch, int32_t row_mode,
                    const float *stats_dev, const float *w_dev, const float *b_dev, double *gram_dev, int32_t slots, void *stream);
int mi_dconv_gn_gelu_gram(float *x_dev, int32_t B, int32_t h, int32_t C_alloc, int32_t D1, int32_t D2, int32_t pitch, int32_t row_mode,
                          const float *stats_dev, const float *w_dev, const float *b_dev, double *gram_dev, int32_t slots, void *stream);
int mi_gram_finalize(double *gram_dev, int32_t rows, int32_t h, int32_t slots, const double *wt_dev, const double *ct_dev, double sum_b,
                     double sum_bsq, double cols, double count, float eps, float *stats_out_dev, void *stream);

int mi_lstm_seq(const float *gx_dev, const float *whh_host, int32_t N, int32_t H, int32_t W, float *out_dev, int32_t mode, void *stream);

int mi_layernorm_cf(const float *x_dev, int32_t B, int32_t C, int32_t T, const float *w_dev, const float *b_dev,
                    const float *add_dev, float *y_dev, void *stream);

void mi_debug_set_post_launch_hook(void (*hook)(void *stream));

int mi_debug_last_conv_route(void);

const char *mi_last_error(void);
const char *mi_version(void);

#ifdef __cplusplus
}
#endif
#endif
```

Measured before the change: 2313.

## Emit pre-split bf16x3 activation images from producers for float32 transformer linears

Producers (layernorm/token kernels, attention output, linear epilogues) now write their float32 outputs directly as a three-plane split-bf16 operand image. The consuming x6 GEMM DMAs the B operand from that image straight into LDS instead of loading raw floats and splitting them in the main loop. This moves the hi/mid/lo split work out of the GEMM inner loop and lets both operands be fed by async global-to-LDS copies. In exchange it writes three bf16 planes per activation, which costs extra memory traffic, and it needs image buffers and gating through env-controlled scopes.

Measured after the change: 2236. 3.3% lower.

```diff
diff --git a/demucs_amd/_lib.py b/demucs_amd/_lib.py
--- a/demucs_amd/_lib.py
+++ b/demucs_amd/_lib.py
@@ -122,6 +122,10 @@
                                    C.c_double, C.c_double, C.c_float, C.c_void_p, C.c_void_p]),
     "mi_layernorm_cf": (C.c_int, [C.c_void_p, C.c_int32, C.c_int32, C.c_int32, C.c_void_p, C.c_void_p, C.c_void_p,
                                   C.c_void_p, C.c_void_p]),
+    "mi_token_tile": (C.c_int, [C.c_int32, C.c_void_p, C.c_int32, C.c_int32, C.c_int32, C.c_void_p, C.c_void_p, C.c_void_p, C.c_void_p,
+                                C.c_void_p, C.c_void_p, C.c_void_p, C.c_int64, C.c_int32, C.c_void_p]),
+    "mi_attention_split_image": (C.c_int, [C.c_void_p, C.c_void_p, C.c_void_p, C.c_void_p, C.c_int64, C.c_int32, C.c_int32, C.c_int32,
+                                           C.c_int32, C.c_int64, C.c_int64, C.c_void_p]),
     "mi_debug_set_post_launch_hook": (None, [C.c_void_p]),
     "mi_debug_last_conv_route": (C.c_int, []),
     "mi_last_error": (C.c_char_p, []),
diff --git a/demucs_amd/csrc/api.hip b/demucs_amd/csrc/api.hip
--- a/demucs_amd/csrc/api.hip
+++ b/demucs_amd/csrc/api.hip
@@ -520,4 +520,24 @@
     return launch_layernorm_cf(x_dev, B, C, T, w_dev, b_dev, add_dev, y_dev, nullptr, (hipStream_t)stream);
 }
 
-}
+int mi_token_tile(int32_t mode, const float *x_dev, int32_t B, int32_t C, int32_t T, const float *w_dev, const float *b_dev,
+                  const float *add_dev, const float *gstat_dev, float *y_dev, float *stat_dev, void *img_dev, int64_t n_img,
+                  int32_t img_dtype, void *stream) {
+    MI_REQUIRE(x_dev && stat_dev && B > 0 && C > 0 && T > 0 && mode >= 0 && mode <= 2, "mi_token_tile: bad argument");
+    MI_REQUIRE(mode == 1 || (w_dev && b_dev && y_dev), "mi_token_tile: modes 0 and 2 need w, b and y");
+    MI_REQUIRE(mode != 2 || gstat_dev, "mi_token_tile: mode 2 needs the per-item statistics");
+    hipStream_t st = (hipStream_t)stream;
+    float2 *os = (float2 *)stat_dev;
+    if (mode == 0) return launch_layernorm_cf(x_dev, B, C, T, w_dev, b_dev, add_dev, y_dev, os, st, img_dev, n_img, img_dtype);
+    if (mode == 1) return launch_token_stats(x_dev, B, C, T, os, st, img_dev, n_img, img_dtype);
+    return launch_gn_apply_tokstats(x_dev, B, C, T, (const float2 *)gstat_dev, w_dev, b_dev, y_dev, os, st, img_dev, n_img, img_dtype);
+}
+
+int mi_attention_split_image(const float *q_dev, const float *k_dev, const float *v_dev, void *img_dev, int64_t n_img, int32_t B,
+                             int32_t heads, int32_t Tq, int32_t Tk, int64_t q_batch_stride, int64_t kv_batch_stride, void *stream) {
+    MI_REQUIRE(q_dev && k_dev && v_dev && img_dev && B > 0 && heads > 0 && Tq > 0 && Tk > 0, "mi_attention_split_image: bad argument");
+    return launch_attention_x6(q_dev, k_dev, v_dev, nullptr, B, heads, Tq, Tk, q_batch_stride, kv_batch_stride, 0, (hipStream_t)stream,
+                               img_dev, n_img);
+}
+
+}
diff --git a/demucs_amd/csrc/attention_x6.hip b/demucs_amd/csrc/attention_x6.hip
--- a/demucs_amd/csrc/attention_x6.hip
+++ b/demucs_amd/csrc/attention_x6.hip
@@ -33,7 +33,8 @@
 
 __global__ __launch_bounds__(256, 2) void attention_x6_kernel(const float *__restrict__ q, const float *__restrict__ k,
                                                               const float *__restrict__ v, float *__restrict__ o, int Tq, int Tk,
-                                                              int64_t q_bs, int64_t kv_bs, int64_t o_bs, int planes, int heads) {
+                                                              int64_t q_bs, int64_t kv_bs, int64_t o_bs, int planes, int heads,
+                                                              uint2 *__restrict__ oimg, int64_t img_n) {
     __shared__ u32x4 Kx[3 * 8 * KT];
     __shared__ u32x4 Vx[3 * 8 * HD];
     {
@@ -191,7 +192,23 @@
     }
     const float ltot = lrun + __shfl_xor(lrun, 32);
     const float inv = 1.0f / ltot;
-    if (qok) {
+    if (qok && oimg) {
+        const size_t plane = (size_t)heads * 8 * img_n * 2;
+        uint2 *ip = oimg + ((size_t)head * 8 * img_n + (size_t)b * Tq + qi) * 2 + lh;
+#pragma unroll
+        for (int dt = 0; dt < 2; ++dt)
+#pragma unroll
+            for (int g = 0; g < 4; ++g) {
+                unsigned h0, m0, l0, h1, m1, l1;
+                split3(oacc[dt][4 * g] * inv, oacc[dt][4 * g + 1] * inv, h0, m0, l0);
+                split3(oacc[dt][4 * g + 2] * inv, oacc[dt][4 * g + 3] * inv, h1, m1, l1);
+                uint2 *dst = ip + (size_t)(dt * 4 + g) * img_n * 2;
+                dst[0] = make_uint2(h0, h1);
+                dst[plane] = make_uint2(m0, m1);
+                dst[2 * plane] = make_uint2(l0, l1);
+            }
+    }
+    if (qok && o) {
         float *op = o + (size_t)b * o_bs + (size_t)head * HD * Tq + qi;
 #pragma unroll
         for (int dt = 0; dt < 2; ++dt)
@@ -204,12 +221,14 @@
 }
 
 int launch_attention_x6(const float *q, const float *k, const float *v, float *o, int B, int heads, int Tq, int Tk, int64_t q_bs,
-                        int64_t kv_bs, int64_t o_bs, hipStream_t st) {
+                        int64_t kv_bs, int64_t o_bs, hipStream_t st, void *oimg, int64_t img_n) {
     MI_REQUIRE(Tk % 4 == 0, "attention x6: Tk %% 4 != 0 (%d)", Tk);
+    MI_REQUIRE(o || oimg, "attention x6: no output");
+    MI_REQUIRE(!oimg || (((uintptr_t)oimg & 15) == 0 && img_n >= (int64_t)B * Tq), "attention x6: the split image needs 16-byte alignment and >= B * Tq columns");
     MI_REQUIRE(((uintptr_t)k & 15) == 0 && ((uintptr_t)v & 15) == 0 && kv_bs % 4 == 0, "attention x6: k/v must be 16-byte aligned");
     const int planes = B * heads;
     hipLaunchKernelGGL(attention_x6_kernel, dim3((unsigned)(ceil_div(Tq, 128) * ((planes + 7) / 8) * 8)), dim3(256), 0, st, q, k, v, o,
-                       Tq, Tk, q_bs, kv_bs, o_bs, planes, heads);
+                       Tq, Tk, q_bs, kv_bs, o_bs, planes, heads, (uint2 *)oimg, img_n);
     MI_CHECK_LAUNCH();
     return MI_OK;
 }
diff --git a/demucs_amd/csrc/gemm_conv.hip b/demucs_amd/csrc/gemm_conv.hip
--- a/demucs_amd/csrc/gemm_conv.hip
+++ b/demucs_amd/csrc/gemm_conv.hip
@@ -668,7 +668,8 @@
     const int64_t P = (int64_t)d.O1 * d.O2;
     const bool plain = d.plain && d.K == d.Kpad && P % 4 == 0 && d.x_bstride % 4 == 0 && ((uintptr_t)d.x & 15) == 0 &&
                        d.S1 == 1 && d.S2 == 1 && d.D1 == d.O1 && (d.x_ld ? d.x_ld : d.D2) == d.O2;
-    MI_REQUIRE(!(d.flags & MI_FLAG_IMG) || d.epi == MI_EPI_CONVTR ||
+    const bool split_img = !d.half && d.wx && d.epi == MI_EPI_LINEAR && plain && conv_x6_supported(tile);
+    MI_REQUIRE(!(d.flags & MI_FLAG_IMG) || d.epi == MI_EPI_CONVTR || (split_img && d.yh) ||
                (d.half && d.yh && d.epi == MI_EPI_LINEAR && d.M % 8 == 0 && d.yh_n >= (int64_t)d.B * P && ((uintptr_t)d.yh & 15) == 0) ||
                (d.half && d.yh && d.epi == MI_EPI_GLU && d.M % 32 == 0 && !(d.flags & (MI_FLAG_IMG4 | MI_FLAG_EMB)) && d.yh_n >= (int64_t)d.B * P &&
                 ((uintptr_t)d.yh & 15) == 0),
@@ -689,7 +690,8 @@
     MI_REQUIRE(!(d.flags & MI_FLAG_HEADS) || (d.half && d.yh && d.epi == MI_EPI_LINEAR && d.M % 512 == 0 && d.O1 == 1 && d.yh_n >= d.O2 &&
                                               ((uintptr_t)d.yh & 15) == 0 && !(d.flags & MI_FLAG_IMG)),
                "conv: MI_FLAG_HEADS needs a half-precision LINEAR layer on tokens (O1 = 1) with M %% 512 == 0 and an aligned output");
-    MI_REQUIRE(!d.xh || d.half, "conv: an operand-image input needs a half-precision layer");
+    MI_REQUIRE(!d.xh || d.half || split_img,
+               "conv: an operand-image input needs a half-precision layer, or a plain float32 LINEAR layer on the split-bf16 loop");
     if (d.half) { g_last_conv_route = 5; return launch_conv_half(d, tile, plain, st); }
     static const int x6_mode = getenv("MI_X6_MODE") ? atoi(getenv("MI_X6_MODE")) : 0;
     static const int x6_class = getenv("MI_X6_CLASS") ? atoi(getenv("MI_X6_CLASS")) : -1;
@@ -715,6 +717,8 @@
         }
     }
     if (!x6_class_ok) d.wx = nullptr;
+    MI_REQUIRE(!(split_img && (d.xh || (d.flags & MI_FLAG_IMG))) || (x6_class_ok && x6_mode == 0 && !x6_verify),
+               "conv: the split activation image does not combine with MI_X6_MODE / MI_X6_CLASS / MI_X6_VERIFY");
     if (d.wx && conv_x6_supported(tile) && x6_mode == 3) return launch_conv_x6(d, tile, false, st);
     if (d.wx && conv_x6_supported(tile) && (x6_mode == 0 || (x6_mode == 1) == plain))
         return x6_verify ? x6_verified_launch(d, tile, plain, st) : launch_conv_x6(d, tile, plain, st);
diff --git a/demucs_amd/csrc/gemm_tile.h b/demucs_amd/csrc/gemm_tile.h
--- a/demucs_amd/csrc/gemm_tile.h
+++ b/demucs_amd/csrc/gemm_tile.h
@@ -2,6 +2,7 @@
 #include "common.h"
 #include "gemm_conv.h"
 #include "kernels.h"
+#include "split_bf16.h"
 
 namespace mi {
 
@@ -9,6 +10,7 @@
 
 constexpr int BK = 16;
 constexpr int BN = 128;
+constexpr int kMiLflagImg3 = 1 << 16;
 
 struct ColInfo {
     int b, o1, o2, p;
@@ -175,6 +177,23 @@
                         }
                         continue;
                     }
+                    if (LFLAGS & kMiLflagImg3) {
+                        vq[r & 3] = v;
+                        if ((r & 3) == 3) {
+                            const int mo = mbase + 8 * (r >> 2);
+                            unsigned h0, m0_, l0, h1, m1, l1;
+                            split3(vq[0], vq[1], h0, m0_, l0);
+                            split3(vq[2], vq[3], h1, m1, l1);
+                            const size_t plane = (size_t)(d.M >> 3) * d.yh_n * 2;
+                            uint2 *dst = reinterpret_cast<uint2 *>(d.yh) + ((size_t)(mo >> 3) * d.yh_n + n) * 2 + lh;
+                            if (c.valid && mo < d.M) {
+                                dst[0] = make_uint2(h0, h1);
+                                dst[plane] = make_uint2(m0_, m1);
+                                dst[2 * plane] = make_uint2(l0, l1);
+                            }
+                        }
+                        continue;
+                    }
                     if (LFLAGS & MI_FLAG_IMG) {
                         vq[r & 3] = v;
                         if ((r & 3) == 3) {
diff --git a/demucs_amd/csrc/gemm_x6.hip b/demucs_amd/csrc/gemm_x6.hip
--- a/demucs_amd/csrc/gemm_x6.hip
+++ b/demucs_amd/csrc/gemm_x6.hip
@@ -34,10 +34,11 @@
 #define MI_X6_ABL 0
 #endif
 constexpr int kRowTaps = -1;
-template <int WM, int WN, int TM, int TN, int EPI, int LFLAGS, bool PLAIN, bool HALF_IMG, int NT>
+template <int WM, int WN, int TM, int TN, int EPI, int LFLAGS, bool PLAIN, bool HALF_IMG, int NT, bool BIMG = false>
 __device__ __forceinline__ void conv_x6_body(const mi_conv_desc &d, const int N, const int MT, const int Gm) {
     constexpr int BM = WM * TM * 32;
-    constexpr bool RAW = PLAIN || NT != 0;
+    constexpr bool RAW = (PLAIN || NT != 0) && !BIMG;
+    static_assert(!BIMG || (PLAIN && NT == 0 && EPI == MI_EPI_LINEAR), "split activation image: plain LINEAR layers");
     constexpr bool ROWS = NT == kRowTaps;
     static_assert(NT <= 0 || (!PLAIN && EPI == MI_EPI_GLU), "tap loader: GLU rewrite convs");
     static_assert(!ROWS || (!PLAIN && (EPI == MI_EPI_LINEAR || EPI == MI_EPI_CONVTR || EPI == MI_EPI_GLU)),
@@ -75,6 +76,18 @@
             if (chunk < A_CHUNKS)                                                                                   \
                 __builtin_amdgcn_global_load_lds((gvoid_t *)(aimg + (size_t)(kt) * A_KSTEP + chunk * A_CHUNK_STRIDE), \
                                                  (lvoid_t *)(smem + (stage) * STAGE + chunk * 1024), 16, 0, 0);     \
+        }                                                                                                           \
+    } while (0)
+
+    const unsigned char *bimg = reinterpret_cast<const unsigned char *>(d.xh) + ((size_t)n0 + lane) * 16;
+    const size_t bimg_row = (size_t)d.xh_n * 16, bimg_plane = (size_t)(d.Kpad / 8) * bimg_row;
+#define MI_BIMG_DMA(kt, stage)                                                                                      \
+    do {                                                                                                            \
+        _Pragma("unroll") for (int c = 0; c < 3; ++c) {                                                             \
+            const int chunk = c * 4 + wave, pk = chunk >> 1;                                                        \
+            __builtin_amdgcn_global_load_lds(                                                                       \
+                (gvoid_t *)(bimg + (pk >> 1) * bimg_plane + (size_t)(2 * (kt) + (pk & 1)) * bimg_row + (chunk & 1) * 1024), \
+                (lvoid_t *)(smem + (stage) * STAGE + A_BYTES + chunk * 1024), 16, 0, 0);                            \
         }                                                                                                           \
     } while (0)
 
@@ -182,7 +195,9 @@
 
     constexpr int PA[6] = {2, 0, 1, 1, 0, 0}, PB[6] = {0, 2, 1, 0, 1, 0};
     MI_A_DMA(0, 0);
-    if constexpr (RAW) {
+    if constexpr (BIMG) {
+        MI_BIMG_DMA(0, 0);
+    } else if constexpr (RAW) {
         if constexpr (ROWS) MI_ROW_ENTRIES(0);
         MI_BRAW_DMA(0, 0);
         if (nk > 1) {
@@ -198,7 +213,7 @@
     } else {
         MI_B_LOAD(0);
     }
-    MI_B_STORE(0);
+    if constexpr (!BIMG) MI_B_STORE(0);
     asm volatile("s_waitcnt vmcnt(0)" ::: "memory");
     __syncthreads();
     int cur = 0;
@@ -256,7 +271,9 @@
         __builtin_amdgcn_sched_barrier(0);
         if (kt + 1 < nk) {
             MI_A_DMA(kt + 1, cur ^ 1);
-            if constexpr (RAW) {
+            if constexpr (BIMG) {
+                MI_BIMG_DMA(kt + 1, cur ^ 1);
+            } else if constexpr (RAW) {
                 if (kt + 2 < nk) MI_BRAW_DMA(kt + 2, kt & 1);
             } else {
                 MI_B_LOAD(kt + 1);
@@ -277,7 +294,9 @@
                         if (MI_X6_ABL & 16) asm volatile("s_nop 15\n\ts_nop 15");
                         if ((MI_X6_ABL & 32) && a == TM - 1 && b == TN - 1) asm volatile("s_nop 15\n\ts_nop 15\n\ts_nop 15\n\ts_nop 15");
                     }
-        if (RAW || kt + 1 < nk) MI_B_STORE(cur ^ 1);
+        if constexpr (!BIMG) {
+            if (RAW || kt + 1 < nk) MI_B_STORE(cur ^ 1);
+        }
         if constexpr (RAW) {
 #pragma unroll
             for (int i = 0; i < 6 * TM * TN; ++i) {
@@ -295,6 +314,7 @@
         cur ^= 1;
     }
 #undef MI_A_DMA
+#undef MI_BIMG_DMA
 #undef MI_B_LOAD
 #undef MI_BRAW_DMA
 #undef MI_BRAW_FIX
@@ -317,6 +337,14 @@
     conv_x6_body<WM, WN, TM, TN, EPI, LFLAGS, PLAIN, HALF_IMG, 0>(d, N, MT, Gm);
 }
 
+#ifndef MI_X6_IMG_WGS
+#define MI_X6_IMG_WGS 2
+#endif
+template <int WM, int WN, int TM, int TN, int LFLAGS, bool HALF_IMG>
+__global__ __launch_bounds__(256, (LFLAGS & MI_FLAG_STATS) ? 2 : MI_X6_IMG_WGS) void conv_gemm_x6_img_kernel(const mi_conv_desc d, const int N, const int MT, const int Gm) {
+    conv_x6_body<WM, WN, TM, TN, MI_EPI_LINEAR, LFLAGS, true, HALF_IMG, 0, true>(d, N, MT, Gm);
+}
+
 template <int WM, int WN, int TM, int TN, bool HALF_IMG, int NT>
 __global__ __launch_bounds__(256, 2) void conv_tap_x6_kernel(const mi_conv_desc d, const int N, const int MT, const int Gm) {
     conv_x6_body<WM, WN, TM, TN, MI_EPI_GLU, 0, false, HALF_IMG, NT>(d, N, MT, Gm);
@@ -327,7 +355,7 @@
     conv_x6_body<WM, WN, TM, TN, EPI, LFLAGS, false, HALF_IMG, kRowTaps>(d, N, MT, Gm);
 }
 
-template <int WM, int WN, int TM, int TN, int EPI, int LFLAGS, bool PLAIN, bool HALF_IMG = false, int NTAPS = 0>
+template <int WM, int WN, int TM, int TN, int EPI, int LFLAGS, bool PLAIN, bool HALF_IMG = false, int NTAPS = 0, bool BIMG = false>
 static int launch_cfg_x6(const mi_conv_desc &d, hipStream_t st) {
     constexpr int BM = WM * TM * 32;
     const int64_t N64 = (int64_t)d.B * d.O1 * d.O2;
@@ -336,7 +364,8 @@
     const int N = (int)N64, MT = d.Mpad / BM, NT = ceil_div(N, BN);
     const int Gm = pick_m_groups(MT, (size_t)d.Kpad * d.Mpad * 6);
     const unsigned grid = grouped_grid(MT, NT, Gm);
-    if constexpr (NTAPS > 0) hipLaunchKernelGGL((conv_tap_x6_kernel<WM, WN, TM, TN, HALF_IMG, NTAPS>), dim3(grid), dim3(256), 0, st, d, N, MT, Gm);
+    if constexpr (BIMG) hipLaunchKernelGGL((conv_gemm_x6_img_kernel<WM, WN, TM, TN, LFLAGS, HALF_IMG>), dim3(grid), dim3(256), 0, st, d, N, MT, Gm);
+    else if constexpr (NTAPS > 0) hipLaunchKernelGGL((conv_tap_x6_kernel<WM, WN, TM, TN, HALF_IMG, NTAPS>), dim3(grid), dim3(256), 0, st, d, N, MT, Gm);
     else if constexpr (NTAPS == kRowTaps)
         hipLaunchKernelGGL((conv_rows_x6_kernel<WM, WN, TM, TN, EPI, LFLAGS, HALF_IMG>), dim3(grid), dim3(256), 0, st, d, N, MT, Gm);
     else hipLaunchKernelGGL((conv_gemm_x6_kernel<WM, WN, TM, TN, EPI, LFLAGS, PLAIN, HALF_IMG>), dim3(grid), dim3(256), 0, st, d, N, MT, Gm);
@@ -357,6 +386,14 @@
         case 64: return launch_cfg_x6<1, 4, 2, 1, EPI, LFLAGS, PLAIN>(d, st);
     }
     return set_error(MI_EINVAL, "conv x6: unsupported tile_m %d", tile);
+}
+
+template <int LFLAGS>
+static int launch_tile_x6_img(const mi_conv_desc &d, hipStream_t st) {
+    static const int small = getenv("MI_SMALL_TILE") ? atoi(getenv("MI_SMALL_TILE")) : 1;
+    if (small && (int64_t)(d.Mpad / 128) * ceil_div((int64_t)d.B * d.O1 * d.O2, BN) < 200)
+        return launch_cfg_x6<1, 4, 2, 1, MI_EPI_LINEAR, LFLAGS, true, true, 0, true>(d, st);
+    return launch_cfg_x6<2, 2, 2, 2, MI_EPI_LINEAR, LFLAGS, true, false, 0, true>(d, st);
 }
 
 bool conv_x6_supported(int tile) { return tile == 128 || tile == 96 || tile == 64; }
@@ -405,6 +442,28 @@
 int launch_conv_x6(const mi_conv_desc &d, int tile, bool plain, hipStream_t st) {
     g_last_conv_route = 4;
     MI_REQUIRE(d.wx && ((uintptr_t)d.wx & 15) == 0, "conv x6: split weight image missing or misaligned");
+    const int lf = d.flags & (MI_FLAG_GELU | MI_FLAG_SCALE | MI_FLAG_RES | MI_FLAG_LN | MI_FLAG_STATS | MI_FLAG_IMG);
+    if (d.flags & MI_FLAG_IMG)
+        MI_REQUIRE(plain && d.epi == MI_EPI_LINEAR && lf == (MI_FLAG_LN | MI_FLAG_GELU | MI_FLAG_IMG) && d.yh && ((uintptr_t)d.yh & 15) == 0 &&
+                       d.M % 8 == 0 && d.yh_n >= (int64_t)d.B * d.O1 * d.O2,
+                   "conv x6: a split output image needs a plain LINEAR layer with LN | GELU, M %% 8 == 0 and an aligned image of >= B * P columns");
+    if (d.xh) {
+        const int64_t N64 = (int64_t)d.B * d.O1 * d.O2;
+        MI_REQUIRE(plain && d.epi == MI_EPI_LINEAR && tile == 128 && ((uintptr_t)d.xh & 15) == 0 && d.xh_n % BN == 0 &&
+                       d.xh_n >= (N64 + BN - 1) / BN * BN,
+                   "conv x6: a split activation image needs a plain LINEAR layer on the 128-row tile and an aligned image whose column "
+                   "count is a multiple of %d covering B * P (tile %d, columns %lld)", BN, tile, (long long)d.xh_n);
+        g_last_conv_route = 9;
+        switch (lf) {
+            case MI_FLAG_LN: return launch_tile_x6_img<MI_FLAG_LN>(d, st);
+            case MI_FLAG_LN | MI_FLAG_GELU: return launch_tile_x6_img<MI_FLAG_LN | MI_FLAG_GELU>(d, st);
+            case MI_FLAG_LN | MI_FLAG_GELU | MI_FLAG_IMG: return launch_tile_x6_img<MI_FLAG_LN | MI_FLAG_GELU | kMiLflagImg3>(d, st);
+            case MI_FLAG_SCALE | MI_FLAG_RES: return launch_tile_x6_img<MI_FLAG_SCALE | MI_FLAG_RES>(d, st);
+            case MI_FLAG_SCALE | MI_FLAG_RES | MI_FLAG_STATS: return launch_tile_x6_img<MI_FLAG_SCALE | MI_FLAG_RES | MI_FLAG_STATS>(d, st);
+        }
+        return set_error(MI_EINVAL, "conv x6: no image-fed LINEAR kernel for flag combination %d", d.flags);
+    }
+    if (d.flags & MI_FLAG_IMG) return launch_tile_x6<MI_EPI_LINEAR, MI_FLAG_LN | MI_FLAG_GELU | kMiLflagImg3, true>(d, tile, st);
 #define MI_DISPATCH(E)                                              \
     case E: return plain ? launch_tile_x6<E, 0, true>(d, tile, st) : launch_tile_x6<E, 0, false>(d, tile, st)
 #define MI_LINEAR(F)                                                \
diff --git a/demucs_amd/csrc/kernels.h b/demucs_amd/csrc/kernels.h
--- a/demucs_amd/csrc/kernels.h
+++ b/demucs_amd/csrc/kernels.h
@@ -111,7 +111,7 @@
 int launch_attention(const float *q, const float *k, const float *v, float *o, int B, int heads, int Tq, int Tk, int64_t q_bs,
                      int64_t kv_bs, int64_t o_bs, int dtype, hipStream_t st, void *oh = nullptr, int64_t oh_n = 0);
 int launch_attention_x6(const float *q, const float *k, const float *v, float *o, int B, int heads, int Tq, int Tk, int64_t q_bs,
-                        int64_t kv_bs, int64_t o_bs, hipStream_t st);
+                        int64_t kv_bs, int64_t o_bs, hipStream_t st, void *oimg = nullptr, int64_t img_n = 0);
 
 int launch_segments_gather(const float *track, int64_t track_len, int channels, const int64_t *starts_dev, int B, int valid,
                            float *seg, hipStream_t st);
diff --git a/demucs_amd/csrc/model.hip b/demucs_amd/csrc/model.hip
--- a/demucs_amd/csrc/model.hip
+++ b/demucs_amd/csrc/model.hip
@@ -127,13 +127,21 @@
     return scope;
 }
 
+static bool x6_image() {
+    static const bool on = !(getenv("MI_X6_IMAGE") && atoi(getenv("MI_X6_IMAGE")) == 0) && !getenv("MI_X6_MODE") && !getenv("MI_X6_CLASS") &&
+                           !getenv("MI_X6_VERIFY");
+    return on;
+}
+static int64_t img_cols(int64_t n) { return (n + 127) / 128 * 128; }
+
 int Model::attn(const float *q, const float *k, const float *v, float *o, int B, int Tq, int Tk, int64_t q_bs, int64_t kv_bs,
                 int64_t o_bs, hipStream_t st, bool image) {
     void *oh = image ? (void *)o : nullptr;
-    const int64_t oh_n = (int64_t)B * Tq;
-    const bool x6 = cfg.dtype == MI_DTYPE_F32 && !image && g_split_bf16 && x6_scope() != 0;
+    const bool x6 = cfg.dtype == MI_DTYPE_F32 && g_split_bf16 && x6_scope() != 0;
+    MI_REQUIRE(!image || x6 || cfg.dtype != MI_DTYPE_F32, "attention: the split image exists on the split-bf16 kernel only");
+    const int64_t oh_n = x6 ? img_cols((int64_t)B * Tq) : (int64_t)B * Tq;
     auto launch = [&]() {
-        return x6 ? launch_attention_x6(q, k, v, o, B, 8, Tq, Tk, q_bs, kv_bs, o_bs, st)
+        return x6 ? launch_attention_x6(q, k, v, image ? nullptr : o, B, 8, Tq, Tk, q_bs, kv_bs, o_bs, st, oh, oh_n)
                   : launch_attention(q, k, v, o, B, 8, Tq, Tk, q_bs, kv_bs, o_bs, cfg.dtype, st, oh, oh_n);
     };
     if (!prof.on) return launch();
@@ -648,8 +656,19 @@
         }
         for (int q = 0; q < 2; ++q) MI_TRY(dev_alloc((void **)&w.w_tr_stat[br][q], B * P * sizeof(float2)));
         MI_TRY(dev_alloc((void **)&w.w_tr_stat1[br], B * P * sizeof(float2)));
-        MI_TRY(A(&w.w_tr_qkv[br], 1536 * Tf)) ; MI_TRY(A(&w.w_tr_att[br], 512 * P));
-        MI_TRY(A(&w.w_tr_x1[br], 512 * P)); MI_TRY(A(&w.w_tr_x2[br], 512 * P)); MI_TRY(A(&w.w_tr_ffh[br], 2048 * P));
+        MI_TRY(A(&w.w_tr_qkv[br], 1536 * Tf)) ;
+        MI_TRY(A(&w.w_tr_x1[br], 512 * P)); MI_TRY(A(&w.w_tr_x2[br], 512 * P));
+        if (cfg.dtype == MI_DTYPE_F32 && x6_scope() != 0 && x6_image()) {
+            const size_t n_img = (size_t)img_cols((int64_t)(B * P)), img512 = 6 * 512 * n_img;
+            for (float **p : {&w.w_tr_ximg[br][0], &w.w_tr_ximg[br][1], &w.w_tr_x1img[br], &w.w_tr_att[br]}) {
+                MI_TRY(dev_alloc((void **)p, img512));
+                MI_HIP(hipMemset(*p, 0, img512));
+            }
+            MI_TRY(dev_alloc((void **)&w.w_tr_ffh[br], 4 * img512));
+            MI_HIP(hipMemset(w.w_tr_ffh[br], 0, 4 * img512));
+        } else {
+            MI_TRY(A(&w.w_tr_att[br], 512 * P)); MI_TRY(A(&w.w_tr_ffh[br], 2048 * P));
+        }
     }
     MI_TRY(A(&w.w_yspec, (size_t)4 * S * 2048 * T));
     MI_TRY(A(&w.w_ytime, (size_t)2 * S * SL));
@@ -771,6 +790,8 @@
     const bool img = cfg.dtype != MI_DTYPE_F32 && !no_img;
     static const bool no_heads = getenv("MI_NO_QKV_HEADS") != nullptr;
     const bool heads = img && !no_heads;
+    const bool img3 = cfg.dtype == MI_DTYPE_F32 && ximg != nullptr;
+    const int64_t nq = img3 ? img_cols((int64_t)B * Tq) : (int64_t)B * Tq, nk = img3 ? img_cols((int64_t)B * Tk) : (int64_t)B * Tk;
     unsigned short *qh = reinterpret_cast<unsigned short *>(qkv);
     const size_t plane_q = (size_t)B * 512 * Tq, plane_k = (size_t)B * 512 * Tk;
     if (!cross) {
@@ -778,17 +799,17 @@
         d.plain = 1; d.epi = MI_EPI_LINEAR; d.flags = MI_FLAG_LN; d.scale = l.qkv_c1; d.pro_stats = (const float *)xstat;
         d.y = qkv; d.y_bstride = (int64_t)1536 * Tq; d.y_cstride = Tq;
         if (heads) { d.flags |= MI_FLAG_HEADS; d.yh = qh; d.yh_n = Tq; }
-        if (heads && ximg) { d.xh = ximg; d.xh_n = (int64_t)B * Tq; }
+        if ((heads || img3) && ximg) { d.xh = ximg; d.xh_n = nq; }
         MI_TRY(conv(d, st));
         if (heads) MI_TRY(attn_heads(qh, qh + plane_q, qh + 2 * plane_q, att, B, Tq, Tq, st));
         else MI_TRY(attn(qkv, qkv + (size_t)512 * Tq, qkv + (size_t)1024 * Tq, att, B, Tq, Tq, (int64_t)1536 * Tq, (int64_t)1536 * Tq,
-                         (int64_t)512 * Tq, st, img));
+                         (int64_t)512 * Tq, st, img || img3));
     } else {
         mi_conv_desc d = base_desc(l.q_proj, tr_ktab512[br], x, (int64_t)512 * Tq, gq);
         d.plain = 1; d.epi = MI_EPI_LINEAR; d.flags = MI_FLAG_LN; d.scale = l.q_c1; d.pro_stats = (const float *)xstat;
         d.y = qkv; d.y_bstride = (int64_t)512 * Tq; d.y_cstride = Tq;
         if (heads) { d.flags |= MI_FLAG_HEADS; d.yh = qh; d.yh_n = Tq; }
-        if (heads && ximg) { d.xh = ximg; d.xh_n = (int64_t)B * Tq; }
+        if ((heads || img3) && ximg) { d.xh = ximg; d.xh_n = nq; }
         MI_TRY(conv(d, st));
         float *kv = qkv + (size_t)B * 512 * Tq;
         unsigned short *kvh = qh + plane_q;
@@ -796,30 +817,30 @@
         e.plain = 1; e.epi = MI_EPI_LINEAR; e.flags = MI_FLAG_LN; e.scale = l.kv_c1; e.pro_stats = (const float *)ostat;
         e.y = kv; e.y_bstride = (int64_t)1024 * Tk; e.y_cstride = Tk;
         if (heads) { e.flags |= MI_FLAG_HEADS; e.yh = kvh; e.yh_n = Tk; }
-        if (heads && oimg) { e.xh = oimg; e.xh_n = (int64_t)B * Tk; }
+        if ((heads || img3) && oimg) { e.xh = oimg; e.xh_n = nk; }
         MI_TRY(conv(e, st));
         if (heads) MI_TRY(attn_heads(qh, kvh, kvh + plane_k, att, B, Tq, Tk, st));
-        else MI_TRY(attn(qkv, kv, kv + (size_t)512 * Tk, att, B, Tq, Tk, (int64_t)512 * Tq, (int64_t)1024 * Tk, (int64_t)512 * Tq, st, img));
+        else MI_TRY(attn(qkv, kv, kv + (size_t)512 * Tk, att, B, Tq, Tk, (int64_t)512 * Tq, (int64_t)1024 * Tk, (int64_t)512 * Tq, st, img || img3));
     }
     {
         mi_conv_desc d = base_desc(l.out_proj, tr_ktab512[br], att, (int64_t)512 * Tq, gq);
         d.plain = 1; d.epi = MI_EPI_LINEAR; d.flags = MI_FLAG_SCALE | MI_FLAG_RES; d.scale = l.gamma1; d.res = x;
         d.y = x1; d.y_bstride = (int64_t)512 * Tq; d.y_cstride = Tq;
-        if (img) { d.xh = att; d.xh_n = (int64_t)B * Tq; }
+        if (img || img3) { d.xh = att; d.xh_n = nq; }
         MI_TRY(conv(d, st));
     }
-    const bool in_img = heads && ximg != nullptr;
-    MI_TRY(launch_token_stats(x1, B, 512, Tq, w_tr_stat1[br], st, in_img ? w_tr_x1img[br] : nullptr, (int64_t)B * Tq, cfg.dtype));
+    const bool in_img = (heads || img3) && ximg != nullptr;
+    MI_TRY(launch_token_stats(x1, B, 512, Tq, w_tr_stat1[br], st, in_img ? w_tr_x1img[br] : nullptr, nq, cfg.dtype));
     {
         mi_conv_desc d = base_desc(l.lin1, tr_ktab512[br], x1, (int64_t)512 * Tq, gq);
         d.plain = 1; d.epi = MI_EPI_LINEAR; d.flags = MI_FLAG_LN | MI_FLAG_GELU; d.scale = l.lin1_c1;
         d.pro_stats = (const float *)w_tr_stat1[br];
         d.y = ffh; d.y_bstride = (int64_t)2048 * Tq; d.y_cstride = Tq;
-        if (img) { d.flags |= MI_FLAG_IMG; d.yh = ffh; d.yh_n = (int64_t)B * Tq; }
-        if (img && in_img) { d.xh = w_tr_x1img[br]; d.xh_n = (int64_t)B * Tq; }
+        if (img || img3) { d.flags |= MI_FLAG_IMG; d.yh = ffh; d.yh_n = nq; }
+        if ((img || img3) && in_img) { d.xh = w_tr_x1img[br]; d.xh_n = nq; }
         MI_TRY(conv(d, st));
         mi_conv_desc e = base_desc(l.lin2, tr_ktab2048[br], ffh, (int64_t)2048 * Tq, gq);
-        if (img) { e.xh = ffh; e.xh_n = (int64_t)B * Tq; }
+        if (img || img3) { e.xh = ffh; e.xh_n = nq; }
         e.plain = 1; e.epi = MI_EPI_LINEAR; e.flags = MI_FLAG_SCALE | MI_FLAG_RES; e.scale = l.gamma2; e.res = x1;
         if (lin2_stats) { e.flags |= MI_FLAG_STATS; e.stats = stats; }
         e.y = x2; e.y_bstride = (int64_t)512 * Tq; e.y_cstride = Tq;
@@ -828,7 +849,7 @@
     if (!lin2_stats) MI_TRY(launch_row_stats(x2, B, (int64_t)512 * Tq, (int64_t)512 * Tq, stats, st));
     MI_TRY(launch_finalize_stats(stats, B, (double)512 * Tq, 1e-5f, 0, st1, nullptr, st));
     MI_TRY(launch_gn_apply_tokstats(x2, B, 512, Tq, st1, l.norm_w[3], l.norm_b[3], out, outstat, st, in_img ? outimg : nullptr,
-                                    (int64_t)B * Tq, cfg.dtype));
+                                    nq, cfg.dtype));
     return MI_OK;
 }
 
@@ -956,7 +977,8 @@
     }
     int cur[2] = {0, 0};
     static const bool no_in_img = getenv("MI_NO_INPUT_IMAGE") != nullptr || getenv("MI_NO_QKV_HEADS") != nullptr || getenv("MI_NO_FFN_IMAGE") != nullptr;
-    const bool in_img = cfg.dtype != MI_DTYPE_F32 && !no_in_img;
+    const bool img3 = cfg.dtype == MI_DTYPE_F32 && g_split_bf16 && x6_scope() != 0 && x6_image() && w_tr_ximg[0][0] && tr[0][0].lin1.wx;
+    const bool in_img = (cfg.dtype != MI_DTYPE_F32 && !no_in_img) || img3;
     for (int br = 0; br < 2; ++br) {
         const int P = br ? Tt : Tf;
         const Geo g{B, 1, P, 0};
@@ -965,7 +987,8 @@
         d.plain = 1; d.epi = MI_EPI_LINEAR; d.y = w_tr_x1[br]; d.y_bstride = (int64_t)512 * P; d.y_cstride = P;
         MI_TRY(conv(d, sb));
         MI_TRY(launch_layernorm_cf(w_tr_x1[br], B, 512, P, norm_in_w[br], norm_in_b[br], pos_emb[br], w_tr_x[br][0],
-                                   w_tr_stat[br][0], sb, in_img ? w_tr_ximg[br][0] : nullptr, (int64_t)B * P, cfg.dtype));
+                                   w_tr_stat[br][0], sb, in_img ? w_tr_ximg[br][0] : nullptr,
+                                   img3 ? img_cols((int64_t)B * P) : (int64_t)B * P, cfg.dtype));
     }
     MI_STAGE("upsample + norm_in done");
     for (int k = 0; k < 5; ++k) {
diff --git a/demucs_amd/csrc/norms.hip b/demucs_amd/csrc/norms.hip
--- a/demucs_amd/csrc/norms.hip
+++ b/demucs_amd/csrc/norms.hip
@@ -1,5 +1,6 @@
 #include "common.h"
 #include "kernels.h"
+#include "split_bf16.h"
 
 namespace mi {
 
@@ -71,7 +72,22 @@
         y[base + i] = (x[base + i] - nm.x) * nm.y;
 }
 
-template <int MODE>
+template <bool SPLIT>
+__device__ __forceinline__ void store_img8(uint4 *__restrict__ img, size_t idx, size_t plane, int dtype, const float (&q)[8]) {
+    if constexpr (SPLIT) {
+        unsigned h[4], m[4], l[4];
+#pragma unroll
+        for (int j = 0; j < 4; ++j) split3(q[2 * j], q[2 * j + 1], h[j], m[j], l[j]);
+        img[idx] = make_uint4(h[0], h[1], h[2], h[3]);
+        img[idx + plane] = make_uint4(m[0], m[1], m[2], m[3]);
+        img[idx + 2 * plane] = make_uint4(l[0], l[1], l[2], l[3]);
+    } else {
+        img[idx] = make_uint4(pack_half2(dtype, q[0], q[1]), pack_half2(dtype, q[2], q[3]), pack_half2(dtype, q[4], q[5]),
+                              pack_half2(dtype, q[6], q[7]));
+    }
+}
+
+template <int MODE, bool SPLIT = false>
 __global__ __launch_bounds__(256) void token_tile_kernel(const float *__restrict__ x, int C, int T, const float *__restrict__ w,
                                                          const float *__restrict__ bvec, const float *__restrict__ pe,
                                                          const float2 *__restrict__ gstat, float eps, float *__restrict__ y,
@@ -83,6 +99,7 @@
     const size_t base = (size_t)blockIdx.y * C * T + (ok ? t : 0);
     const int cw = C / 4, c0 = wv * cw;
     const float inv_c = 1.0f / (float)C;
+    const size_t img_plane = (size_t)(C >> 3) * img_n;
     float mean = 0.f, rstd = 1.f;
     if (MODE == 0 || MODE == 1) {
         const float x0 = x[base];
@@ -96,9 +113,7 @@
                     const float v = q[e] - x0;
                     s1 += v; s2 += v * v;
                 }
-                if (ok) img[(size_t)(c >> 3) * img_n + (size_t)blockIdx.y * T + t] =
-                    make_uint4(pack_half2(img_dtype, q[0], q[1]), pack_half2(img_dtype, q[2], q[3]), pack_half2(img_dtype, q[4], q[5]),
-                               pack_half2(img_dtype, q[6], q[7]));
+                if (ok) store_img8<SPLIT>(img, (size_t)(c >> 3) * img_n + (size_t)blockIdx.y * T + t, img_plane, img_dtype, q);
             }
         } else
         for (int c = c0; c < c0 + cw; ++c) {
@@ -147,9 +162,7 @@
             q8[e] = v;
         }
         if (img && ok)
-            img[(size_t)(c >> 3) * img_n + (size_t)blockIdx.y * T + t] =
-                make_uint4(pack_half2(img_dtype, q8[0], q8[1]), pack_half2(img_dtype, q8[2], q8[3]), pack_half2(img_dtype, q8[4], q8[5]),
-                           pack_half2(img_dtype, q8[6], q8[7]));
+            store_img8<SPLIT>(img, (size_t)(c >> 3) * img_n + (size_t)blockIdx.y * T + t, img_plane, img_dtype, q8);
     }
     for (; c < c0 + cw; ++c) {
         float v = (x[base + (size_t)c * T] - mean) * rstd * w[c] + bvec[c];
@@ -338,8 +351,8 @@
 }
 
 static int check_img(int C, const void *img, int64_t img_n, int B, int T, int dtype) {
-    MI_REQUIRE(!img || (C % 32 == 0 && img_n >= (int64_t)B * T && ((uintptr_t)img & 15) == 0 && (dtype == MI_DTYPE_BF16 || dtype == MI_DTYPE_F16)),
-               "token kernel: operand image needs C %% 32 == 0, >= B * T columns, 16-byte alignment and a half dtype");
+    MI_REQUIRE(!img || (C % 32 == 0 && img_n >= (int64_t)B * T && ((uintptr_t)img & 15) == 0 && (dtype == MI_DTYPE_BF16 || dtype == MI_DTYPE_F16 || dtype == MI_DTYPE_F32)),
+               "token kernel: operand image needs C %% 32 == 0, >= B * T columns, 16-byte alignment and a dtype (float32: the split image)");
     return MI_OK;
 }
 
@@ -347,8 +360,12 @@
                         float2 *ostat, hipStream_t st, void *img, int64_t img_n, int img_dtype) {
     MI_REQUIRE(C % 4 == 0, "layernorm: C %% 4 != 0");
     MI_TRY(check_img(C, img, img_n, B, T, img_dtype));
-    hipLaunchKernelGGL(token_tile_kernel<0>, dim3(ceil_div(T, 64), B), dim3(256), 0, st, x, C, T, w, b, pe, nullptr, 1e-5f, y, ostat,
-                       (uint4 *)img, img_n, img_dtype);
+    if (img && img_dtype == MI_DTYPE_F32)
+        hipLaunchKernelGGL((token_tile_kernel<0, true>), dim3(ceil_div(T, 64), B), dim3(256), 0, st, x, C, T, w, b, pe, nullptr, 1e-5f, y, ostat,
+                           (uint4 *)img, img_n, img_dtype);
+    else
+        hipLaunchKernelGGL(token_tile_kernel<0>, dim3(ceil_div(T, 64), B), dim3(256), 0, st, x, C, T, w, b, pe, nullptr, 1e-5f, y, ostat,
+                           (uint4 *)img, img_n, img_dtype);
     MI_CHECK_LAUNCH();
     return MI_OK;
 }
@@ -356,8 +373,12 @@
 int launch_token_stats(const float *x, int B, int C, int T, float2 *ostat, hipStream_t st, void *img, int64_t img_n, int img_dtype) {
     MI_REQUIRE(C % 4 == 0, "token_stats: C %% 4 != 0");
     MI_TRY(check_img(C, img, img_n, B, T, img_dtype));
-    hipLaunchKernelGGL(token_tile_kernel<1>, dim3(ceil_div(T, 64), B), dim3(256), 0, st, x, C, T, nullptr, nullptr, nullptr, nullptr,
-                       1e-5f, nullptr, ostat, (uint4 *)img, img_n, img_dtype);
+    if (img && img_dtype == MI_DTYPE_F32)
+        hipLaunchKernelGGL((token_tile_kernel<1, true>), dim3(ceil_div(T, 64), B), dim3(256), 0, st, x, C, T, nullptr, nullptr, nullptr, nullptr,
+                           1e-5f, nullptr, ostat, (uint4 *)img, img_n, img_dtype);
+    else
+        hipLaunchKernelGGL(token_tile_kernel<1>, dim3(ceil_div(T, 64), B), dim3(256), 0, st, x, C, T, nullptr, nullptr, nullptr, nullptr,
+                           1e-5f, nullptr, ostat, (uint4 *)img, img_n, img_dtype);
     MI_CHECK_LAUNCH();
     return MI_OK;
 }
@@ -366,10 +387,14 @@
                              float2 *ostat, hipStream_t st, void *img, int64_t img_n, int img_dtype) {
     MI_REQUIRE(C % 4 == 0, "gn_apply: C %% 4 != 0");
     MI_TRY(check_img(C, img, img_n, B, T, img_dtype));
-    hipLaunchKernelGGL(token_tile_kernel<2>, dim3(ceil_div(T, 64), B), dim3(256), 0, st, x, C, T, w, b, nullptr, gstat, 1e-5f, y, ostat,
-                       (uint4 *)img, img_n, img_dtype);
-    MI_CHECK_LAUNCH();
-    return MI_OK;
-}
-
-}
+    if (img && img_dtype == MI_DTYPE_F32)
+        hipLaunchKernelGGL((token_tile_kernel<2, true>), dim3(ceil_div(T, 64), B), dim3(256), 0, st, x, C, T, w, b, nullptr, gstat, 1e-5f, y, ostat,
+                           (uint4 *)img, img_n, img_dtype);
+    else
+        hipLaunchKernelGGL(token_tile_kernel<2>, dim3(ceil_div(T, 64), B), dim3(256), 0, st, x, C, T, w, b, nullptr, gstat, 1e-5f, y, ostat,
+                           (uint4 *)img, img_n, img_dtype);
+    MI_CHECK_LAUNCH();
+    return MI_OK;
+}
+
+}
diff --git a/include/demucs_amd.h b/include/demucs_amd.h
--- a/include/demucs_amd.h
+++ b/include/demucs_amd.h
@@ -229,6 +229,13 @@
 int mi_layernorm_cf(const float *x_dev, int32_t B, int32_t C, int32_t T, const float *w_dev, const float *b_dev,
                     const float *add_dev, float *y_dev, void *stream);
 
+int mi_token_tile(int32_t mode, const float *x_dev, int32_t B, int32_t C, int32_t T, const float *w_dev, const float *b_dev,
+                  const float *add_dev, const float *gstat_dev, float *y_dev, float *stat_dev, void *img_dev, int64_t n_img,
+                  int32_t img_dtype, void *stream);
+
+int mi_attention_split_image(const float *q_dev, const float *k_dev, const float *v_dev, void *img_dev, int64_t n_img, int32_t B,
+                             int32_t heads, int32_t Tq, int32_t Tk, int64_t q_batch_stride, int64_t kv_batch_stride, void *stream);
+
 void mi_debug_set_post_launch_hook(void (*hook)(void *stream));
 
 int mi_debug_last_conv_route(void);
```
